# SCUT-BIP-Lab/SplatCo

Measured on AMD Instinct MI355X. Metric: rasterizer fwd+bwd Msplats/s @1080p; PSNR-match vs ref, higher is better.
Workload: dtype f32; 1 GPU; cfg1: 1M synthetic Gaussians (seed 0), 1 view 1920x1080 per GPU, GaussianRasterizer forward+backward, colors_precomp + scale/rotation path; gaussians=1000000, image=1920x1080, visible=1000000, parallelism=1 view per GPU (mv sharding)

## Files before the change

### include/splatco_raster.h

```cpp
#ifndef SPLATCO_RASTER_H
#define SPLATCO_RASTER_H

#include <stddef.h>
#include <stdint.h>

#ifdef __cplusplus
extern "C" {
#endif

#define SCR_ABI_VERSION 29
#define SCR_TILE 16

typedef struct scr_settings {
    int32_t image_height;
    int32_t image_width;
    float tanfovx;
    float tanfovy;
    const float* bg;
    float scale_modifier;
    const float* viewmatrix;
    const float* projmatrix;
    int32_t sh_degree;
    const float* campos;
    int32_t prefiltered;
    int32_t debug;
} scr_settings;

int scr_abi_version(void);
const char* scr_last_error(void);

size_t scr_geom_bytes(int64_t P, int32_t image_height, int32_t image_width);
size_t scr_binning_bytes(int64_t num_rendered, int64_t max_tile_instances);
size_t scr_image_bytes(int32_t image_height, int32_t image_width);
size_t scr_backward_scratch_bytes(int64_t num_rendered);

int scr_visible_filter(int64_t P, const float* means3D, const float* scales, const float* rotations,
                       const float* cov3D_precomp, const scr_settings* settings, int32_t* radii_out,
                       void* stream);

int scr_mark_visible(int64_t P, const float* means3D, const float* viewmatrix, uint8_t* present_out,
                     void* stream);

enum { SCR_PLAN_NONFINITE_COLOUR = 1,
       SCR_PLAN_LARGE_RECTS = 2 };
int scr_forward_plan(int64_t P, int32_t M, const float* means3D, const float* scales,
                     const float* rotations, const float* cov3D_precomp, const float* opacities,
                     const float* shs, const float* colors_precomp, const scr_settings* settings,
                     void* geom_buf, int32_t* radii_out, int64_t* plan_host, void* stream);

int scr_forward_run(int64_t P, int64_t num_rendered, int64_t max_tile_instances, int64_t plan_flags,
                    const scr_settings* settings, void* geom_buf, void* binning_buf, void* image_buf, float* out_color,
                    void* stream);

int scr_forward_plan_run(int64_t P, int32_t M, const float* means3D, const float* scales, const float* rotations,
                         const float* cov3D_precomp, const float* opacities, const float* shs, const float* colors_precomp,
                         const scr_settings* settings, void* geom_buf, int32_t* radii_out, int64_t* plan_host,
                         void* binning_buf, size_t binning_capacity_bytes, void* image_buf, float* out_color, void* stream);

int scr_backward(int64_t P, int32_t M, int64_t num_rendered, int64_t plan_flags, const float* means3D, const float* scales,
                 const float* rotations, const float* cov3D_precomp, const float* shs,
                 const scr_settings* settings, const int32_t* radii, void* geom_buf,
                 const void* binning_buf, void* image_buf, const float* dL_dcolor, void* scratch,
                 float* dL_dmeans3D, float* dL_dmeans2D, float* dL_dcolors, float* dL_dsh,
                 float* dL_dopacity, float* dL_dscales, float* dL_drotations, float* dL_dcov3D,
                 void* stream);

enum {
    SCR_DBG_TILES_TOUCHED = 0,
    SCR_DBG_POINT_OFFSETS = 1,
    SCR_DBG_RANGES = 2,
    SCR_DBG_POINT_LIST = 3,
    SCR_DBG_N_CONTRIB = 4,
    SCR_DBG_FINAL_T = 5,
    SCR_DBG_SPLAT_RECORDS = 6,
    SCR_DBG_QMASK = 7,
    SCR_DBG_GM_INDEX = 8
};
int scr_debug_force_deep_lists(int mode);
int scr_debug_get(int which, int64_t P, int64_t num_rendered, int32_t image_height, int32_t image_width,
                  const void* geom_buf, const void* binning_buf, const void* image_buf, void* out,
                  void* stream);

size_t scr_tpa_scratch_bytes(int32_t R, int32_t H, int32_t W);
int scr_tpa_stats(int32_t R, int32_t H, int32_t W, const float* p0, const float* p1, const float* p2, float* avg,
                  float* mx, int32_t* arg, void* scratch, void* stream);
int scr_tpa_forward(int32_t R, int32_t H, int32_t W, const float* p0, const float* p1, const float* p2, const float* ca,
                    const float* w, float* s, uint8_t* am, float* sa, float* pair0, float* pair1, float* pair2, void* stream);
int scr_tpa_backward(int32_t R, int32_t H, int32_t W, const float* p0, const float* p1, const float* p2, const float* ca,
                     const float* w, const float* s, const uint8_t* am, const float* sa, const float* g0, const float* g1,
                     const float* g2, float* d0, float* d1, float* d2, float* dca, float* dw, void* scratch, void* stream);
int scr_tpa_backward_stats(int32_t R, int32_t H, int32_t W, const float* davg, const float* dmax, const int32_t* arg,
                           float* d0, float* d1, float* d2, void* stream);

size_t scr_expand_scratch_bytes(int64_t n_candidates);
int scr_expand_plan(int64_t n_candidates, const float* neural_opacity, void* scratch,
                    int64_t* num_selected_host, void* stream);
int scr_mask_index_plan(int64_t n, const uint8_t* mask, void* scratch, int64_t* num_set_host, void* stream);
int scr_mask_index_run(int64_t n, const uint8_t* mask, const void* scratch, int64_t* index, int64_t* inverse, void* stream);
int scr_expand_run(int64_t V, int32_t k, const float* neural_opacity, const float* color,
                   const float* scale_rot, const float* offsets, int32_t offsets_ld, const float* grid_scaling,
                   const float* anchor, const void* scratch, int32_t* out_index, uint8_t* mask_out,
                   float* xyz, float* color_out, float* opacity, float* scaling, float* rot, void* stream);
int scr_expand_backward(int64_t V, int32_t k, const float* scale_rot, const float* offsets, int32_t offsets_ld,
                        const float* grid_scaling, const int32_t* out_index, const float* g_xyz,
                        const float* g_color, const float* g_opacity, const float* g_scaling,
                        const float* g_rot, float* d_neural_opacity, float* d_color, float* d_scale_rot,
                        float* d_offsets, float* d_grid_scaling, float* d_anchor, const float* g_reg, int64_t P,
                        void* stream);

size_t scr_triplane_backward_multi_scratch_bytes(int64_t V, int32_t ngrids, const int32_t* R, const int32_t* X, const int32_t* Y,
                                                 const int32_t* Z);
int scr_triplane_backward_multi(int64_t V, const float* coords, int32_t cstride, int32_t ngrids, const int32_t* R,
                                const int32_t* X, const int32_t* Y, const int32_t* Z, const int32_t* col, const float* grad_out,
                                int32_t ld, float* const* grad_planes, void* scratch, const float* nl_coef, const float* nl_dy,
                                int32_t nl_lddy, const float* nl_x, int32_t nl_ldx, void* stream);
int scr_plane_row_pairs(int32_t R, int32_t A, int32_t B, const float* plane, float* pairs, void* stream);
int scr_triplane_forward(int64_t V, const float* coords, int32_t cstride, const float* xy, const float* xz,
                         const float* yz, int32_t R, int32_t X, int32_t Y, int32_t Z, int32_t channel_last, float* out,
                         int32_t ld, int32_t col_xy, int32_t col_xz, int32_t col_yz, void* stream);
size_t scr_plane_sample_scratch_bytes(int64_t V, int32_t A, int32_t B, int32_t channels);
size_t scr_triplane_backward_scratch_bytes(int64_t V, int32_t X, int32_t Y, int32_t Z, int32_t channels);
int scr_triplane_backward(int64_t V, const float* coords, int32_t cstride, int32_t R, int32_t X, int32_t Y, int32_t Z,
                          int32_t planes, const float* grad_out, int32_t ld, const int32_t* cols, float* const* grad_planes,
                          void* scratch, void* stream);
int scr_plane_sample_backward(int64_t V, const float* coords, int32_t cstride, int32_t cx, int32_t cy, int32_t R,
                              int32_t A, int32_t B, int32_t planes, const float* grad_out0, const float* grad_out1,
                              int32_t ld, float* grad_plane0, float* grad_plane1, void* scratch, void* stream);

size_t scr_l1_ssim_scratch_bytes(int32_t C, int32_t H, int32_t W, int32_t with_grad);
int scr_l1_ssim_forward(int32_t C, int32_t H, int32_t W, const float* img1, const float* img2, void* scratch,
                        int32_t with_grad, float* out2, void* stream);
int scr_l1_ssim_backward(int32_t C, int32_t H, int32_t W, const float* img1, const float* img2,
                         const void* scratch, const float* g_l1, const float* g_ssim, float* dimg1,
                         void* stream);

#define SCR_FLIP_MAX_RADIUS 16
size_t scr_flip_scratch_bytes(int32_t N, int32_t H, int32_t W);
int scr_flip_forward(int32_t N, int32_t H, int32_t W, const float* test, const float* ref, double pixels_per_degree,
                     int32_t quantize, void* scratch, float* mean_out, float* mse_out, float* map_out, void* stream);
int scr_flip_filters(double pixels_per_degree, double* weights, int32_t* radii, double* scalars);

size_t scr_scaling_reg_scratch_bytes(int64_t P);
int scr_scaling_reg_forward(int64_t P, const float* scaling, void* scratch, float* out, void* stream);
int scr_scaling_reg_backward(int64_t P, const float* scaling, const float* g, float* dscaling, void* stream);

size_t scr_pair_l1_scratch_bytes(int64_t n);
int scr_pair_l1_forward(int64_t n, const float* gen1, const float* gen2, const float* real1, const float* real2, void* scratch,
                        float* out, void* stream);
int scr_pair_l1_backward(int64_t n, const float* gen1, const float* gen2, const float* real1, const float* real2, const float* g,
                         float* d_gen1, float* d_gen2, void* stream);

int32_t scr_anchor_gather_stat_rows(int64_t V);
int64_t scr_anchor_gather_stat_buffer_rows(int64_t V);
int scr_anchor_gather(int64_t V, const int64_t* visible_index, const float* anchor_feat, const float* anchor,
                      const float* offset, const float* scaling, float* feat_out, float* anchor_out, float* offsets_out,
                      float* grid_scaling_out, float* g_fea_out, int32_t g_fea_ld, float* col_stats_out, void* stream);
int scr_anchor_gather_backward(int64_t N, int64_t V, const int64_t* inverse_index, const float* grid_scaling, const float* d_feat,
                               const float* d_anchor, const float* d_offsets, const float* d_grid_scaling,
                               const float* d_g_fea, int32_t g_fea_ld, float* g_anchor_feat, float* g_anchor,
                               float* g_offset, float* g_scaling, int32_t accumulate, const float* nl_coef, const float* nl_dy,
                               int32_t nl_lddy, const float* nl_x, int32_t nl_ldx, void* stream);

size_t scr_norm_linear_scratch_bytes(int64_t V);
int scr_box_coords(int64_t V, const float* xyz, const float* lo_host, const float* hi_host, float* out, void* stream);
int scr_norm_fold(int32_t L, int32_t d, const int32_t* widths_host, const int32_t* cols_host, const uint8_t* col_at_host,
                  const void* const* lin_weight_host, const void* const* lin_bias_host, const void* const* bn_weight_host,
                  const void* const* bn_bias_host, float* G, float* c, void* stream);
int scr_norm_fold_backward(int32_t L, int32_t d, const int32_t* widths_host, const int32_t* cols_host, const uint8_t* col_at_host,
                           const void* const* lin_weight_host, const void* const* bn_weight_host, const void* const* bn_bias_host,
                           const float* dG, const float* dc, void* const* d_lin_weight_host, void* const* d_lin_bias_host,
                           void* const* d_bn_weight_host, void* const* d_bn_bias_host, void* stream);
int scr_norm_running_stats(int32_t L, int32_t d, const int32_t* widths_host, const int32_t* cols_host, const uint8_t* col_at_host,
                           const float* momentum_host, void* const* running_mean_host, void* const* running_var_host,
                           void* const* num_batches_host, const float* mean, const float* var, int64_t n, void* stream);
int scr_norm_linear_forward(int64_t V, int32_t d, const float* x, int32_t ldx, const float* G, const float* c, float eps,
                            float* y, float* mean, float* var, float* inv, void* scratch, const float* col_stats,
                            int32_t col_stat_rows, void* stream);
int scr_norm_linear_dx(int64_t V, int32_t d, const float* x, int32_t ldx, const float* dy, int32_t lddy, const float* coef,
                       float* dx, int32_t lddx, void* stream);
int scr_norm_linear_backward(int64_t V, int32_t d, const float* x, int32_t ldx, const float* dy, int32_t lddy, const float* G,
                             const float* mean, const float* inv, float* dx, int32_t lddx, float* dG, float* dc,
                             void* scratch, float* coef_out, void* stream);

size_t scr_mlp_heads_hidden_bytes(int64_t V);
size_t scr_mlp_heads_partial_bytes(int64_t V);
int scr_mlp_heads_forward(int64_t V, const float* feat, int32_t feat_ld, const float* anchor, const float* campos, const float* geo_a, const float* geo_b,
                          const float* w1, const float* b1, const float* w2o, const float* b2o, const float* w2c,
                          const float* b2c, const float* w2v, const float* b2v, void* hidden_save, float* out_opacity,
                          float* out_color, float* out_cov, void* stream);
int scr_mlp_heads_backward(int64_t V, const float* feat, int32_t feat_ld, const float* anchor, const float* campos, const float* geo_a, const float* geo_b,
                           const float* w1, const float* w2o, const float* w2c, const float* w2v, const void* hidden_save,
                           const float* out_opacity, const float* out_color, const float* g_opacity, const float* g_color,
                           const float* g_cov, void* partial, float* d_feat, float* d_anchor, float* d_geo_a, float* d_geo_b, float* d_w1,
                           float* d_b1, float* d_w2o, float* d_b2o, float* d_w2c, float* d_b2c, float* d_w2v, float* d_b2v,
                           void* stream);

int scr_statis_compute(int64_t V, int32_t k, const float* neural_opacity, const int32_t* out_index,
                       const uint8_t* update_filter, const float* viewspace_grad, int32_t grad_stride,
                       float* inc_opacity, float* inc_grad, void* stream);
int scr_statis_apply(int64_t V, int32_t k, const int64_t* visible_index, const float* inc_opacity, const float* inc_grad,
                     float* opacity_accum, float* anchor_demon, float* offset_gradient_accum, float* offset_denom,
                     void* stream);

typedef struct scr_adam_tensor {
    float* param;
    const float* grad;
    float* exp_avg;
    float* exp_avg_sq;
    int64_t numel;
    double step_size, bias_correction2_sqrt;
} scr_adam_tensor;
int scr_adam_step(int32_t n_tensors, const scr_adam_tensor* tensors, double beta1, double beta2, double eps, void* stream);

typedef struct scr_tv_plane {
    const float* plane;
    float* grad;
    int32_t channels, rows, cols;
    float coef;
} scr_tv_plane;
int scr_tv_add_grad(int32_t n_planes, const scr_tv_plane* planes, void* stream);

int scr_knn(int64_t N, int32_t k, const float* grid_host, const float* sorted_pts, const int64_t* sorted_id,
            const int32_t* cell_start, int64_t* out_idx, void* stream);
int scr_knn_curvature(int64_t N, int32_t k, const float* points, const int64_t* idx, float* curvature, void* stream);

size_t scr_points_bounds_scratch_bytes(int64_t N);
int scr_points_bounds(int64_t N, const float* points, void* scratch, float* out7, void* stream);
size_t scr_voxel_unique_scratch_bytes(int64_t N);
int scr_voxel_keys(int64_t N, const float* points, float voxel_size, const int32_t* lo_host, int32_t packed, int64_t* out,
                   void* stream);
int scr_voxel_unique_plan(int64_t N, const int64_t* sorted_keys, void* scratch, int64_t* num_unique_host, void* stream);
int scr_voxel_unique_run(int64_t N, const int64_t* sorted_keys, const void* scratch, float voxel_size,
                         const int32_t* lo_host, float* out_xyz, void* stream);
int scr_knn3_cell_keys(int64_t N, const float* grid_host, const float* points, int64_t* keys, void* stream);
int scr_knn3_dist2(int64_t N, const float* grid_host, const float* sorted_pts, const int64_t* sorted_id,
                   const int32_t* cell_start, float* out, void* stream);

int scr_copy_probe(const void* src, void* dst, size_t bytes, void* stream);

enum {
    SCR_PROF_FILTER = 0, SCR_PROF_PREPROCESS = 1, SCR_PROF_PLAN_SCAN = 2, SCR_PROF_SCATTER = 3,
    SCR_PROF_TILE_SORT = 4, SCR_PROF_BLEND_FORWARD = 5, SCR_PROF_BLEND_BACKWARD = 6,
    SCR_PROF_PREPROCESS_BACKWARD = 7, SCR_PROF_EXPAND = 8, SCR_PROF_EXPAND_BACKWARD = 9, SCR_PROF_PLANE_BACKWARD = 10,
    SCR_PROF_L1_SSIM = 11, SCR_PROF_L1_SSIM_BACKWARD = 12, SCR_PROF_TRIPLANE_FORWARD = 13, SCR_PROF_MLP_HEADS = 14,
    SCR_PROF_MLP_HEADS_BACKWARD = 15, SCR_PROF_NORM_LINEAR = 16, SCR_PROF_NORM_LINEAR_BACKWARD = 17, SCR_PROF_PLANE_ATTENTION = 18,
    SCR_PROF_FLIP = 19, SCR_PROF_COUNT = 20
};
int scr_profile_enable(int mask);
int scr_profile_stride(int every);
int scr_profile_read(double* total_ms, int64_t* launches);
const char* scr_profile_kernel_name(int idx);

int scr_markers_enable(int on);
int scr_marker_push(const char* name);
int scr_marker_pop(void);

#ifdef __cplusplus
}
#endif
#endif
```

### splatco_amd/_C.py

```python
import ctypes as C
import os

import torch

_HERE = os.path.dirname(os.path.abspath(__file__))
LIB_PATH = os.environ.get("SPLATCO_RASTER_LIB", os.path.join(_HERE, "csrc", "libsplatco_raster.so"))

PLAN_NONFINITE_COLOUR, PLAN_LARGE_RECTS = 1, 2
PROF_COUNT = 20
ABI_VERSION = 29
FLIP_MAX_RADIUS = 16

(DBG_TILES_TOUCHED, DBG_POINT_OFFSETS, DBG_RANGES, DBG_POINT_LIST, DBG_N_CONTRIB, DBG_FINAL_T, DBG_SPLAT_RECORDS, DBG_QMASK,
 DBG_GM_INDEX) = range(9)

vp, cp, u8, i32, i64, f32, f64, sz = C.c_void_p, C.c_char_p, C.c_uint8, C.c_int32, C.c_int64, C.c_float, C.c_double, C.c_size_t
P = C.POINTER


class Settings(C.Structure):
    _fields_ = [
        ("image_height", i32), ("image_width", i32),
        ("tanfovx", f32), ("tanfovy", f32),
        ("bg", vp), ("scale_modifier", f32),
        ("viewmatrix", vp), ("projmatrix", vp),
        ("sh_degree", i32), ("campos", vp),
        ("prefiltered", i32), ("debug", i32),
    ]


class AdamTensor(C.Structure):
    _fields_ = [("param", vp), ("grad", vp), ("exp_avg", vp), ("exp_avg_sq", vp),
                ("numel", i64), ("step_size", f64), ("bias_correction2_sqrt", f64)]


class TvPlane(C.Structure):
    _fields_ = [("plane", vp), ("grad", vp), ("channels", i32), ("rows", i32), ("cols", i32), ("coef", f32)]


SIGNATURES = [
    ("scr_abi_version", i32),
    ("scr_last_error", cp),
    ("scr_geom_bytes", sz, i64, i32, i32),
    ("scr_binning_bytes", sz, i64, i64),
    ("scr_image_bytes", sz, i32, i32),
    ("scr_backward_scratch_bytes", sz, i64),
    ("scr_visible_filter", i32, i64, vp, vp, vp, vp, P(Settings), vp, vp),
    ("scr_mark_visible", i32, i64, vp, vp, vp, vp),
    ("scr_forward_plan", i32, i64, i32, *[vp] * 7, P(Settings), vp, vp, P(i64), vp),
    ("scr_forward_run", i32, i64, i64, i64, i64, P(Settings), *[vp] * 5),
    ("scr_forward_plan_run", i32, i64, i32, *[vp] * 7, P(Settings), vp, vp, P(i64), vp, sz, vp, vp, vp),
    ("scr_backward", i32, i64, i32, i64, i64, *[vp] * 5, P(Settings), *[vp] * 15),
    ("scr_debug_force_deep_lists", i32, i32),
    ("scr_debug_get", i32, i32, i64, i64, i32, i32, *[vp] * 5),
    ("scr_tpa_scratch_bytes", sz, i32, i32, i32),
    ("scr_tpa_stats", i32, i32, i32, i32, *[vp] * 8),
    ("scr_tpa_forward", i32, i32, i32, i32, *[vp] * 12),
    ("scr_tpa_backward", i32, i32, i32, i32, *[vp] * 18),
    ("scr_tpa_backward_stats", i32, i32, i32, i32, *[vp] * 7),
    ("scr_expand_scratch_bytes", sz, i64),
    ("scr_expand_plan", i32, i64, vp, vp, P(i64), vp),
    ("scr_mask_index_plan", i32, i64, vp, vp, P(i64), vp),
    ("scr_mask_index_run", i32, i64, *[vp] * 5),
    ("scr_expand_run", i32, i64, i32, vp, vp, vp, vp, i32, *[vp] * 11),
    ("scr_expand_backward", i32, i64, i32, vp, vp, i32, *[vp] * 14, i64, vp),
    ("scr_triplane_backward_multi_scratch_bytes", sz, i64, i32, vp, vp, vp, vp),
    ("scr_triplane_backward_multi", i32, i64, vp, i32, i32, *[vp] * 6, i32, vp, vp, vp, vp, i32, vp, i32, vp),
    ("scr_plane_row_pairs", i32, i32, i32, i32, vp, vp, vp),
    ("scr_triplane_forward", i32, i64, vp, i32, vp, vp, vp, i32, i32, i32, i32, i32, vp, i32, i32, i32, i32, vp),
    ("scr_plane_sample_scratch_bytes", sz, i64, i32, i32, i32),
    ("scr_triplane_backward_scratch_bytes", sz, i64, i32, i32, i32, i32),
    ("scr_triplane_backward", i32, i64, vp, i32, i32, i32, i32, i32, i32, vp, i32, vp, vp, vp, vp),
    ("scr_plane_sample_backward", i32, i64, vp, i32, i32, i32, i32, i32, i32, i32, vp, vp, i32, vp, vp, vp, vp),
    ("scr_l1_ssim_scratch_bytes", sz, i32, i32, i32, i32),
    ("scr_l1_ssim_forward", i32, i32, i32, i32, vp, vp, vp, i32, vp, vp),
    ("scr_l1_ssim_backward", i32, i32, i32, i32, *[vp] * 7),
    ("scr_flip_scratch_bytes", sz, i32, i32, i32),
    ("scr_flip_forward", i32, i32, i32, i32, vp, vp, f64, i32, *[vp] * 5),
    ("scr_flip_filters", i32, f64, vp, vp, vp),
    ("scr_scaling_reg_scratch_bytes", sz, i64),
    ("scr_scaling_reg_forward", i32, i64, vp, vp, vp, vp),
    ("scr_scaling_reg_backward", i32, i64, vp, vp, vp, vp),
    ("scr_pair_l1_scratch_bytes", sz, i64),
    ("scr_pair_l1_forward", i32, i64, *[vp] * 7),
    ("scr_pair_l1_backward", i32, i64, *[vp] * 8),
    ("scr_anchor_gather_stat_rows", i32, i64),
    ("scr_anchor_gather_stat_buffer_rows", i64, i64),
    ("scr_anchor_gather", i32, i64, *[vp] * 10, i32, vp, vp),
    ("scr_anchor_gather_backward", i32, i64, i64, *[vp] * 7, i32, vp, vp, vp, vp, i32, vp, vp, i32, vp, i32, vp),
    ("scr_norm_linear_scratch_bytes", sz, i64),
    ("scr_box_coords", i32, i64, *[vp] * 5),
    ("scr_norm_fold", i32, i32, i32, *[vp] * 10),
    ("scr_norm_fold_backward", i32, i32, i32, *[vp] * 13),
    ("scr_norm_running_stats", i32, i32, i32, *[vp] * 9, i64, vp),
    ("scr_norm_linear_forward", i32, i64, i32, vp, i32, vp, vp, f32, *[vp] * 6, i32, vp),
    ("scr_norm_linear_dx", i32, i64, i32, vp, i32, vp, i32, vp, vp, i32, vp),
    ("scr_norm_linear_backward", i32, i64, i32, vp, i32, vp, i32, vp, vp, vp, vp, i32, *[vp] * 5),
    ("scr_mlp_heads_hidden_bytes", sz, i64),
    ("scr_mlp_heads_partial_bytes", sz, i64),
    ("scr_mlp_heads_forward", i32, i64, vp, i32, *[vp] * 17),
    ("scr_mlp_heads_backward", i32, i64, vp, i32, *[vp] * 28),
    ("scr_statis_compute", i32, i64, i32, vp, vp, vp, vp, i32, vp, vp, vp),
    ("scr_statis_apply", i32, i64, i32, *[vp] * 8),
    ("scr_adam_step", i32, i32, P(AdamTensor), f64, f64, f64, vp),
    ("scr_tv_add_grad", i32, i32, P(TvPlane), vp),
    ("scr_knn", i32, i64, i32, P(f32), *[vp] * 5),
    ("scr_knn_curvature", i32, i64, i32, vp, vp, vp, vp),
    ("scr_points_bounds_scratch_bytes", sz, i64),
    ("scr_points_bounds", i32, i64, vp, vp, vp, vp),
    ("scr_voxel_unique_scratch_bytes", sz, i64),
    ("scr_voxel_keys", i32, i64, vp, f32, P(i32), i32, vp, vp),
    ("scr_voxel_unique_plan", i32, i64, vp, vp, P(i64), vp),
    ("scr_voxel_unique_run", i32, i64, vp, vp, f32, P(i32), vp, vp),
    ("scr_knn3_cell_keys", i32, i64, P(f32), vp, vp, vp),
    ("scr_knn3_dist2", i32, i64, P(f32), *[vp] * 5),
    ("scr_copy_probe", i32, vp, vp, sz, vp),
    ("scr_profile_enable", i32, i32),
    ("scr_profile_stride", i32, i32),
    ("scr_profile_read", i32, P(f64), P(i64)),
    ("scr_profile_kernel_name", cp, i32),
    ("scr_markers_enable", i32, i32),
    ("scr_marker_push", i32, cp),
    ("scr_marker_pop", i32),
]
SYMBOLS = [s[0] for s in SIGNATURES]


def _load():
    if not os.path.exists(LIB_PATH):
        raise ImportError(
            f"{LIB_PATH} not found: the HIP rasterizer library is not built. Run "
            "`python -c 'import __graft_entry__ as g; g.build()'` (or `make -C splatco_amd/csrc`). "
            "There is deliberately no CPU fallback.")
    lib = C.CDLL(LIB_PATH)
    for name, restype, *argtypes in SIGNATURES:
        if not hasattr(lib, name):
            raise ImportError(f"{LIB_PATH} does not export {name}")
        f = getattr(lib, name)
        f.restype, f.argtypes = restype, argtypes
    if lib.scr_abi_version() != ABI_VERSION:
        raise ImportError(f"{LIB_PATH} has ABI version {lib.scr_abi_version()}, expected {ABI_VERSION}")
    return lib


lib = _load()


def profile_enable(which, every=1):
    check(lib.scr_profile_stride(max(int(every), 1)))
    if isinstance(which, str):
        names = [lib.scr_profile_kernel_name(i).decode() for i in range(PROF_COUNT)]
        mask = 1 << names.index(which)
    else:
        mask = -1 if which is True or which == -1 else int(which)
    lib.scr_profile_enable(mask)


MARKERS = False


def markers_enable(on=True):
    global MARKERS
    check(lib.scr_markers_enable(1 if on else 0))
    MARKERS = bool(on)


class stage:
    __slots__ = ("name", "on")

    def __init__(self, name):
        self.name = name

    def __enter__(self):
        self.on = MARKERS
        if self.on:
            lib.scr_marker_push(self.name.encode())
        return self

    def __exit__(self, *exc):
        if self.on:
            if torch.cuda.is_available():
                torch.cuda.synchronize()
            lib.scr_marker_pop()
        return False


def profile_read():
    ms = (C.c_double * PROF_COUNT)()
    n = (C.c_int64 * PROF_COUNT)()
    check(lib.scr_profile_read(ms, n))
    return {lib.scr_profile_kernel_name(i).decode(): (ms[i], n[i]) for i in range(PROF_COUNT)}


def check(rc):
    if rc != 0:
        raise RuntimeError("splatco_raster: " + lib.scr_last_error().decode())


def stream(device=None):
    return torch.cuda.current_stream(device).cuda_stream


def ptr(t):
    return None if t is None or t.numel() == 0 else t.data_ptr()


def host_array(values, ctype=i32):
    values = list(values)
    return (ctype * len(values))(*values)


def ptr_array(tensors):
    return host_array([t.data_ptr() for t in tensors], vp)


def scratch_size(nbytes):
    n = max(int(nbytes), 1)
    if n < (32 << 20):
        return n
    step = 1 << (n.bit_length() - 4)
    return (n + step - 1) // step * step


def scratch(nbytes, device):
    return torch.empty(scratch_size(nbytes), dtype=torch.uint8, device=device)


if os.environ.get("SPLATCO_MARKERS", "") not in ("", "0"):
    markers_enable(True)
```

### splatco_amd/csrc/binning.hip

```cpp
#include "common.h"

namespace scr {

template <int THREADS>
__device__ __forceinline__ uint32_t block_exclusive_scan(uint32_t v, uint32_t* lds_waves ,
                                                         uint32_t& block_total) {
    const int lane = threadIdx.x & (WAVE - 1), w = threadIdx.x / WAVE;
    uint32_t inc = v;
#pragma unroll
    for (int d = 1; d < WAVE; d <<= 1) {
        uint32_t n = __shfl_up(inc, d, WAVE);
        if (lane >= d) inc += n;
    }
    if (lane == WAVE - 1) lds_waves[w] = inc;
    __syncthreads();
    uint32_t base = 0, tot = 0;
#pragma unroll
    for (int k = 0; k < THREADS / WAVE; ++k) {
        uint32_t s = lds_waves[k];
        if (k < w) base += s;
        tot += s;
    }
    block_total = tot;
    __syncthreads();
    return base + inc - v;
}

__global__ void __launch_bounds__(1024) plan_scan_kernel(uint32_t nblk, uint32_t* __restrict__ block_sums,
                                                         unsigned long long* __restrict__ total,
                                                         uint32_t tiles, const uint32_t* __restrict__ tile_count,
                                                         uint32_t* __restrict__ ranges,
                                                         uint32_t* __restrict__ cursor,
                                                         volatile unsigned long long* mailbox,
                                                         unsigned long long seq) {
    __shared__ uint32_t lds[1024 / WAVE + 1];
    __shared__ unsigned long long wide[1024 / WAVE];
    if (blockIdx.x == 0) {
        unsigned long long carry = 0, mine = 0;
        for (uint32_t base = 0; base < nblk; base += 1024) {
            uint32_t i = base + threadIdx.x;
            uint32_t v = i < nblk ? block_sums[i] : 0u, tot;
            uint32_t ex = block_exclusive_scan<1024>(v, lds, tot);
            if (i < nblk) block_sums[i] = (uint32_t)carry + ex;
            carry += tot;
            mine += v;
        }
#pragma unroll
        for (int d = WAVE / 2; d > 0; d >>= 1) mine += (unsigned long long)__shfl_down((long long)mine, d, WAVE);
        __syncthreads();
        if ((threadIdx.x & (WAVE - 1)) == 0) wide[threadIdx.x / WAVE] = mine;
        __syncthreads();
        if (threadIdx.x == 0) {
            carry = 0;
            for (int w = 0; w < 1024 / WAVE; ++w) carry += wide[w];
            total[0] = carry;
            if (mailbox) {
                mailbox[0] = carry;
                __threadfence_system();
                mailbox[1] = seq;
            }
        }
    } else {
        uint32_t carry = 0, mx = 0;
        for (uint32_t base = 0; base < tiles; base += 1024) {
            uint32_t i = base + threadIdx.x;
            uint32_t v = i < tiles ? tile_count[i] : 0u, tot;
            uint32_t ex = block_exclusive_scan<1024>(v, lds, tot);
            if (i < tiles) {
                ranges[2 * i] = carry + ex;
                ranges[2 * i + 1] = carry + ex + v;
                cursor[i] = 0;
            }
            carry += tot;
            mx = max(mx, v);
        }
#pragma unroll
        for (int d = 32; d > 0; d >>= 1) mx = max(mx, (uint32_t)__shfl_xor((int)mx, d, WAVE));
        __syncthreads();
        if ((threadIdx.x & 63) == 0) lds[threadIdx.x >> 6] = mx;
        __syncthreads();
        if (threadIdx.x == 0) {
            uint32_t m = 0;
            for (int w = 0; w < 1024 / WAVE; ++w) m = max(m, lds[w]);
            total[1] = m;
            total[2] = 0;
            if (mailbox) {
                mailbox[2] = (unsigned long long)m | (total[3] << 32);
                __threadfence_system();
                mailbox[3] = seq;
            }
        }
    }
}

template <bool LDS_HIST>
__global__ void __launch_bounds__(BIN_THREADS)
scatter_kernel(int64_t P, int gx, int tiles, const float4* __restrict__ rec, uint2* __restrict__ gm_base,
               uint32_t* __restrict__ live_bits, const uint32_t* __restrict__ tiles_touched, const uint32_t* __restrict__ block_prefix,
               uint32_t* __restrict__ point_offsets, const uint32_t* __restrict__ ranges,
               uint32_t* __restrict__ cursor, unsigned long long* __restrict__ keys,
               const unsigned long long* __restrict__ total, unsigned long long cap_instances) {
    extern __shared__ __attribute__((aligned(16))) uint32_t hist[];
    __shared__ uint32_t lds[BIN_THREADS / WAVE + 1];
    if (total[0] > cap_instances) return;
    if (LDS_HIST) {
        for (int t = threadIdx.x; t < tiles; t += BIN_THREADS) hist[t] = 0;
        __syncthreads();
    }
    uint32_t off[BIN_ROUNDS], tts[BIN_ROUNDS], rlo[BIN_ROUNDS], rhi[BIN_ROUNDS], dbits[BIN_ROUNDS];
    uint32_t carry = block_prefix[blockIdx.x];
#pragma unroll
    for (int r = 0; r < BIN_ROUNDS; ++r) {
        const int64_t i = (int64_t)blockIdx.x * BIN_GPW + r * BIN_THREADS + threadIdx.x;
        const uint32_t tt = i < P ? tiles_touched[i] : 0u;
        uint32_t tot;
        off[r] = carry + block_exclusive_scan<BIN_THREADS>(tt, lds, tot);
        carry += tot;
        tts[r] = tt;
        rlo[r] = rhi[r] = dbits[r] = 0;
        if (i < P) point_offsets[i] = off[r] + tt;
        if (tt) {
            const float4 r2 = rec[3 * i + 2];
            dbits[r] = __float_as_uint(r2.y);
            rlo[r] = __float_as_uint(r2.z);
            rhi[r] = __float_as_uint(r2.w);
            const uint32_t x0 = rlo[r] & 0xffff, y0 = rlo[r] >> 16, rw = (rhi[r] & 0xffff) - x0;
            gm_base[i] = make_uint2(off[r] - y0 * rw - x0, rw);
            if (LDS_HIST)
                for (int ty = rlo[r] >> 16; ty < (int)(rhi[r] >> 16); ++ty)
                    for (int tx = rlo[r] & 0xffff; tx < (int)(rhi[r] & 0xffff); ++tx) atomicAdd(&hist[ty * gx + tx], 1u);
        }
    }
    if (LDS_HIST) {
        __syncthreads();
        for (int t = threadIdx.x; t < tiles; t += BIN_THREADS) {
            const uint32_t c = hist[t];
            if (c) hist[t] = ranges[2 * t] + atomicAdd(&cursor[t], c);
        }
        __syncthreads();
    }
#pragma unroll
    for (int r = 0; r < BIN_ROUNDS; ++r) {
        if (!tts[r]) continue;
        const int64_t i = (int64_t)blockIdx.x * BIN_GPW + r * BIN_THREADS + threadIdx.x;
        const uint32_t klo = (uint32_t)i << 4;
        const float4 r0 = rec[3 * i], r1 = rec[3 * i + 1];
        const unsigned long long khi = (unsigned long long)dbits[r] << 32;
        uint32_t live = 0, kbit = 1;
        for (int ty = rlo[r] >> 16; ty < (int)(rhi[r] >> 16); ++ty)
            for (int tx = rlo[r] & 0xffff; tx < (int)(rhi[r] & 0xffff); ++tx) {
                const uint32_t t = (uint32_t)(ty * gx + tx);
                const uint32_t slot = LDS_HIST ? atomicAdd(&hist[t], 1u) : ranges[2 * t] + atomicAdd(&cursor[t], 1u);
                const uint32_t qm = quadrant_mask(r0, r1, tx * TILE, ty * TILE);
                keys[slot] = khi | klo | qm;
                live |= qm ? kbit : 0u;
                kbit <<= 1;
            }
        live_bits[i] = live;
    }
}

template <int D>
__device__ __forceinline__ uint32_t lane_xor(uint32_t v) {
    if constexpr (D == 1) {
        return (uint32_t)__builtin_amdgcn_mov_dpp((int)v, 0xB1, 0xf, 0xf, true);
    } else if constexpr (D == 2) {
        return (uint32_t)__builtin_amdgcn_mov_dpp((int)v, 0x4E, 0xf, 0xf, true);
    } else if constexpr (D == 4) {
        int t = __builtin_amdgcn_update_dpp((int)v, (int)v, 0x104, 0xf, 0x5, false);
        return (uint32_t)__builtin_amdgcn_update_dpp(t, (int)v, 0x114, 0xf, 0xA, false);
    } else if constexpr (D == 8) {
        int t = __builtin_amdgcn_update_dpp((int)v, (int)v, 0x108, 0xf, 0x3, false);
        return (uint32_t)__builtin_amdgcn_update_dpp(t, (int)v, 0x118, 0xf, 0xC, false);
    } else if constexpr (D == 16) {
        auto r = __builtin_amdgcn_permlane16_swap(v, v, false, false);
        return sel(0xFFFF0000FFFF0000ull, r[0], r[1]);
    } else {
        auto r = __builtin_amdgcn_permlane32_swap(v, v, false, false);
        return sel(0xFFFFFFFF00000000ull, r[0], r[1]);
    }
}

constexpr unsigned long long lanes_with_bit_clear(int bit) {
    unsigned long long m = 0;
    for (int l = 0; l < 64; ++l)
        if ((l & bit) == 0) m |= 1ull << l;
    return m;
}

template <int E, int K, int J>
__device__ __forceinline__ void bitonic_step(uint32_t (&klo)[E], uint32_t (&khi)[E], int lane) {
    if constexpr (J < E) {
#pragma unroll
        for (int e = 0; e < E; ++e) {
            if ((e & J) != 0) continue;
            const int f = e | J;
            const unsigned long long desc = K < E ? ((e & K) == 0 ? 0ull : ~0ull) : ~lanes_with_bit_clear(K / E);
            const unsigned long long a = ((unsigned long long)khi[e] << 32) | klo[e];
            const unsigned long long b = ((unsigned long long)khi[f] << 32) | klo[f];
            const unsigned long long swm = lanes(a > b) ^ desc;
            const uint32_t t0 = klo[e], t1 = khi[e];
            klo[e] = sel(swm, klo[f], t0); khi[e] = sel(swm, khi[f], t1);
            klo[f] = sel(swm, t0, klo[f]); khi[f] = sel(swm, t1, khi[f]);
        }
    } else {
        constexpr int D = J / E;
        constexpr unsigned long long keep_max = lanes_with_bit_clear(D) ^ lanes_with_bit_clear(K / E);
#pragma unroll
        for (int e = 0; e < E; ++e) {
            const uint32_t olo = lane_xor<D>(klo[e]), ohi = lane_xor<D>(khi[e]);
            const unsigned long long mine = ((unsigned long long)khi[e] << 32) | klo[e];
            const unsigned long long theirs = ((unsigned long long)ohi << 32) | olo;
            const unsigned long long take = lanes(theirs < mine) ^ keep_max;
            klo[e] = sel(take, olo, klo[e]);
            khi[e] = sel(take, ohi, khi[e]);
        }
    }
}

template <int E, int K, int J>
__device__ __forceinline__ void bitonic_stage(uint32_t (&klo)[E], uint32_t (&khi)[E], int lane) {
    bitonic_step<E, K, J>(klo, khi, lane);
    if constexpr (J > 1) bitonic_stage<E, K, J / 2>(klo, khi, lane);
}
template <int E, int K>
__device__ __forceinline__ void bitonic_network(uint32_t (&klo)[E], uint32_t (&khi)[E], int lane) {
    bitonic_stage<E, K, K / 2>(klo, khi, lane);
    if constexpr (K < 64 * E) bitonic_network<E, K * 2>(klo, khi, lane);
}

constexpr int WAVE_SORT_MAX = 1024;

struct FinalLists {
    const uint2* gm_base;
    uint32_t* point_list;
    uint32_t* gm_index;
    uint8_t* qmask;
    int tx, ty;
    __device__ __forceinline__ void write(uint32_t i, uint32_t klo) const {
        const uint32_t id = klo >> 4;
        point_list[i] = id;
        qmask[i] = (uint8_t)(klo & 15u);
        if (gm_index) {
            const uint2 b = gm_base[id];
            gm_index[i] = b.x + (uint32_t)ty * b.y + (uint32_t)tx;
        }
    }
    template <int U, typename GetK>
    __device__ __forceinline__ void write_batch(uint32_t lo, uint32_t e0, uint32_t stride, uint32_t cnt, GetK getk) const {
        uint32_t k[U];
        uint2 b[U];
#pragma unroll
        for (int u = 0; u < U; ++u) {
            const uint32_t e = e0 + (uint32_t)u * stride;
            k[u] = e < cnt ? getk(e, u) : 0u;
        }
        if (gm_index) {
#pragma unroll
            for (int u = 0; u < U; ++u) b[u] = gm_base[k[u] >> 4];
        }
        __builtin_amdgcn_sched_barrier(0);
#pragma unroll
        for (int u = 0; u < U; ++u) {
            const uint32_t e = e0 + (uint32_t)u * stride;
            if (e < cnt) {
                point_list[lo + e] = k[u] >> 4;
                qmask[lo + e] = (uint8_t)(k[u] & 15u);
                if (gm_index) gm_index[lo + e] = b[u].x + (uint32_t)ty * b[u].y + (uint32_t)tx;
            }
        }
    }
};

template <int E>
__device__ __forceinline__ void wave_sort_regs(uint32_t n, const unsigned long long* __restrict__ keys,
                                               uint32_t (&klo)[E], uint32_t (&khi)[E]) {
    const int lane = threadIdx.x & 63;
#pragma unroll
    for (int e = 0; e < E; ++e) {
        const uint32_t i = (uint32_t)e * 64 + lane;
        const unsigned long long v = i < n ? keys[i] : ~0ull;
        klo[e] = (uint32_t)v;
        khi[e] = (uint32_t)(v >> 32);
    }
    bitonic_network<E, 2>(klo, khi, lane);
}

template <int E, bool FINAL>
__device__ __forceinline__ void wave_sort(uint32_t n, unsigned long long* __restrict__ keys, uint32_t lo,
                                          const FinalLists& fl, uint32_t* __restrict__ tr) {
    const int lane = threadIdx.x & 63;
    uint32_t klo[E], khi[E];
    wave_sort_regs<E>(n, keys, klo, khi);
    auto transpose = [&](uint32_t (&w)[E]) {
        __syncthreads();
#pragma unroll
        for (int e = 0; e < E; ++e) tr[lane * (E + 1) + e] = w[e];
        __syncthreads();
#pragma unroll
        for (int e = 0; e < E; ++e) {
            const int p = e * 64 + lane;
            w[e] = tr[p + p / E];
        }
    };
    transpose(klo);
    if (!FINAL) transpose(khi);
    if (FINAL) {
        fl.template write_batch<E>(lo, (uint32_t)lane, 64u, n, [&](uint32_t, int u) { return klo[u]; });
    } else {
#pragma unroll
        for (int e = 0; e < E; ++e) {
            const uint32_t i = (uint32_t)e * 64 + lane;
            if (i < n) keys[i] = ((unsigned long long)khi[e] << 32) | klo[e];
        }
    }
}

__device__ __forceinline__ int split_slot(int p) { return p + (p >> 3); }
constexpr int SPLIT_SLOTS = WAVE_SORT_MAX + WAVE_SORT_MAX / 8;
template <int EA, int EB>
__device__ __forceinline__ void wave_sort_split(uint32_t n, const unsigned long long* __restrict__ keys, uint32_t lo,
                                                const FinalLists& fl, unsigned long long* __restrict__ mb) {
    constexpr int NA = 64 * EA, NB = 64 * EB, PER = EA + EB;
    const int lane = threadIdx.x & 63;
    {
        uint32_t klo[EA], khi[EA];
        wave_sort_regs<EA>(NA, keys, klo, khi);
#pragma unroll
        for (int e = 0; e < EA; ++e) mb[split_slot(lane * EA + e)] = ((unsigned long long)khi[e] << 32) | klo[e];
    }
    {
        uint32_t klo[EB], khi[EB];
        wave_sort_regs<EB>(n - NA, keys + NA, klo, khi);
#pragma unroll
        for (int e = 0; e < EB; ++e) mb[split_slot(NA + lane * EB + e)] = ((unsigned long long)khi[e] << 32) | klo[e];
    }
    __syncthreads();
    uint32_t outk[PER];
    {
        auto keyA = [&](uint32_t i) { return mb[split_slot((int)i)]; };
        auto keyB = [&](uint32_t j) { return mb[split_slot(NA + (int)j)]; };
        const uint32_t d0 = (uint32_t)lane * PER;
        uint32_t a = d0 > (uint32_t)NB ? d0 - NB : 0u, b = min(d0, (uint32_t)NA);
        while (a < b) {
            const uint32_t mid = (a + b) >> 1;
            if (keyA(mid) < keyB(d0 - mid - 1)) a = mid + 1;
            else b = mid;
        }
        uint32_t ia = a, ib = d0 - a;
        unsigned long long x = ia < (uint32_t)NA ? keyA(ia) : ~0ull, y = ib < (uint32_t)NB ? keyB(ib) : ~0ull;
#pragma unroll
        for (int k = 0; k < PER; ++k) {
            const bool takeA = x <= y;
            outk[k] = (uint32_t)(takeA ? x : y);
            if (takeA) {
                ++ia;
                x = ia < (uint32_t)NA ? keyA(ia) : ~0ull;
            } else {
                ++ib;
                y = ib < (uint32_t)NB ? keyB(ib) : ~0ull;
            }
        }
    }
    __syncthreads();
    uint32_t* tr = (uint32_t*)mb;
#pragma unroll
    for (int k = 0; k < PER; ++k) tr[lane * (PER + 1) + k] = outk[k];
    __syncthreads();
    fl.template write_batch<PER>(lo, (uint32_t)lane, 64u, n, [&](uint32_t i, int) { return tr[i + i / PER]; });
}

template <bool FINAL>
__device__ __forceinline__ void wave_sort_any(uint32_t n, unsigned long long* keys, uint32_t lo, const FinalLists& fl,
                                              unsigned long long* mb) {
    uint32_t* tr = (uint32_t*)mb;
    if (n <= 64) wave_sort<1, FINAL>(n, keys, lo, fl, tr);
    else if (n <= 128) wave_sort<2, FINAL>(n, keys, lo, fl, tr);
    else if (n <= 256) wave_sort<4, FINAL>(n, keys, lo, fl, tr);
    else if (FINAL && n > 256 && n <= 320) wave_sort_split<4, 1>(n, keys, lo, fl, mb);
    else if (FINAL && n > 256 && n <= 384) wave_sort_split<4, 2>(n, keys, lo, fl, mb);
    else if (n <= 512) wave_sort<8, FINAL>(n, keys, lo, fl, tr);
    else if (FINAL && n <= 576) wave_sort_split<8, 1>(n, keys, lo, fl, mb);
    else if (FINAL && n <= 640) wave_sort_split<8, 2>(n, keys, lo, fl, mb);
    else if (FINAL && n <= 768) wave_sort_split<8, 4>(n, keys, lo, fl, mb);
    else if (FINAL) wave_sort_split<8, 8>(n, keys, lo, fl, mb);
    else wave_sort<16, FINAL>(n, keys, lo, fl, tr);
}

__global__ void __launch_bounds__(64, 1)
tile_sort_wave_kernel(int tiles, int gx, const uint32_t* __restrict__ ranges, unsigned long long* __restrict__ keys,
                      const uint2* __restrict__ gm_base, uint32_t* __restrict__ point_list,
                      uint32_t* __restrict__ gm_index, uint8_t* __restrict__ qmask) {
    int t = xcd_tile(blockIdx.x, tiles);
    if (t < 0) return;
    const uint32_t lo = ranges[2 * t], n = ranges[2 * t + 1] - lo;
    if (n == 0 || n > (uint32_t)WAVE_SORT_MAX) return;
    const FinalLists fl{gm_base, point_list, gm_index, qmask, t % gx, t / gx};
    __shared__ unsigned long long mb[SPLIT_SLOTS];
    wave_sort_any<true>(n, keys + lo, lo, fl, mb);
}

constexpr int WG_SORT_THREADS = WG_SORT_MAX / 16;
__device__ __forceinline__ int wg_slot(int p) { return p + (p >> 4); }
__global__ void __launch_bounds__(WG_SORT_THREADS)
tile_sort_wg_kernel(int tiles, int gx, const uint32_t* __restrict__ ranges, unsigned long long* __restrict__ keys,
                    const uint2* __restrict__ gm_base, uint32_t* __restrict__ point_list,
                    uint32_t* __restrict__ gm_index, uint8_t* __restrict__ qmask) {
    extern __shared__ __attribute__((aligned(16))) unsigned long long buf[];
    int t = xcd_tile(blockIdx.x, tiles);
    if (t < 0) return;
    const uint32_t lo = ranges[2 * t], n = ranges[2 * t + 1] - lo;
    if (n <= (uint32_t)WAVE_SORT_MAX) return;
    const uint32_t c0 = blockIdx.y * (uint32_t)WG_SORT_MAX;
    if (c0 >= n) return;
    const uint32_t cnt = min((uint32_t)WG_SORT_MAX, n - c0);
    const int wave = threadIdx.x >> 6, lane = threadIdx.x & 63;
    unsigned long long* chunk = keys + lo + c0;
    {
        const uint32_t w0 = (uint32_t)wave * WAVE_SORT_MAX;
        const uint32_t wn = w0 < cnt ? min((uint32_t)WAVE_SORT_MAX, cnt - w0) : 0u;
        uint32_t klo[16], khi[16];
        wave_sort_regs<16>(wn, chunk + w0, klo, khi);
#pragma unroll
        for (int e = 0; e < 16; ++e)
            buf[wg_slot((int)w0 + lane * 16 + e)] = ((unsigned long long)khi[e] << 32) | klo[e];
    }
    __syncthreads();
    for (uint32_t L = WAVE_SORT_MAX; L < (uint32_t)WG_SORT_MAX && L < cnt; L <<= 1) {
        constexpr int PER = WG_SORT_MAX / WG_SORT_THREADS;
        unsigned long long outk[PER];
        const uint32_t o0 = threadIdx.x * PER, pairbase = o0 / (2u * L) * (2u * L), d0 = o0 - pairbase;
        {
            auto keyA = [&](uint32_t i) { return buf[wg_slot((int)(pairbase + i))]; };
            auto keyB = [&](uint32_t j) { return buf[wg_slot((int)(pairbase + L + j))]; };
            uint32_t a = d0 > L ? d0 - L : 0u, b = min(d0, L);
            while (a < b) {
                const uint32_t mid = (a + b) >> 1;
                if (keyA(mid) < keyB(d0 - mid - 1)) a = mid + 1;
                else b = mid;
            }
            uint32_t ia = a, ib = d0 - a;
            unsigned long long x = ia < L ? keyA(ia) : ~0ull, y = ib < L ? keyB(ib) : ~0ull;
#pragma unroll
            for (int k = 0; k < PER; ++k) {
                const bool takeA = x <= y;
                outk[k] = takeA ? x : y;
                if (takeA) {
                    ++ia;
                    x = ia < L ? keyA(ia) : ~0ull;
                } else {
                    ++ib;
                    y = ib < L ? keyB(ib) : ~0ull;
                }
            }
        }
        __syncthreads();
#pragma unroll
        for (int k = 0; k < PER; ++k) buf[wg_slot((int)(o0 + k))] = outk[k];
        __syncthreads();
    }
    const unsigned long long* src = buf;
    if (n <= (uint32_t)WG_SORT_MAX) {
        const FinalLists fl{gm_base, point_list, gm_index, qmask, t % gx, t / gx};
        for (uint32_t e = threadIdx.x; e < cnt; e += 4 * WG_SORT_THREADS)
            fl.template write_batch<4>(lo, e, (uint32_t)WG_SORT_THREADS, cnt, [&](uint32_t i, int) { return (uint32_t)src[wg_slot((int)i)]; });
    } else {
        for (uint32_t e = threadIdx.x; e < cnt; e += WG_SORT_THREADS) chunk[e] = src[wg_slot((int)e)];
    }
}

constexpr int MP_SEG = 4096;
__device__ __forceinline__ uint32_t merge_passes_needed(uint32_t n) {
    uint32_t chunks = (n + WG_SORT_MAX - 1) / WG_SORT_MAX, p = 0;
    while ((1u << p) < chunks) ++p;
    return p;
}

__device__ __forceinline__ uint32_t merge_path_cut(const unsigned long long* __restrict__ A, uint32_t la,
                                                   const unsigned long long* __restrict__ B, uint32_t lb, uint32_t s) {
    const uint32_t lane = threadIdx.x & 63;
    uint32_t lo = s > lb ? s - lb : 0u, hi = min(s, la);
    while (lo < hi) {
        const uint32_t span = hi - lo;
        const uint32_t p = span >= 65u ? lo + (uint32_t)(((unsigned long long)span * (lane + 1)) / 65u) : min(lo + lane, hi - 1);
        const bool below = A[p] < B[s - p - 1];
        const unsigned long long bal = __builtin_amdgcn_ballot_w64(below);
        const int c = __builtin_popcountll(bal);
        const uint32_t plast = __shfl(p, c > 0 ? c - 1 : 0, 64), pfirst = __shfl(p, c < 64 ? c : 63, 64);
        const uint32_t nlo = c > 0 ? plast + 1 : lo, nhi = c < 64 ? pfirst : hi;
        if (span < 65u) {
            return c < (int)min(span, 64u) ? lo + (uint32_t)c : hi;
        }
        lo = nlo;
        hi = nhi;
    }
    return lo;
}

__global__ void __launch_bounds__(256)
tile_merge_path_kernel(int tiles, int gx, uint32_t pass, const uint32_t* __restrict__ ranges,
                       const unsigned long long* __restrict__ src, unsigned long long* __restrict__ dst,
                       const uint2* __restrict__ gm_base, uint32_t* __restrict__ point_list,
                       uint32_t* __restrict__ gm_index, uint8_t* __restrict__ qmask) {
    __shared__ unsigned long long buf[MP_SEG + MP_SEG / 16];
    __shared__ uint32_t cut[2];
    int t = xcd_tile(blockIdx.x, tiles);
    if (t < 0) return;
    const uint32_t lo = ranges[2 * t], n = ranges[2 * t + 1] - lo;
    if (n <= (uint32_t)WG_SORT_MAX || pass >= merge_passes_needed(n)) return;
    const uint32_t L = (uint32_t)WG_SORT_MAX << pass;
    const uint32_t e0 = blockIdx.y * (uint32_t)MP_SEG;
    if (e0 >= n) return;
    const uint32_t pairbase = e0 / (2u * L) * (2u * L);
    const uint32_t lenA = min(L, n - pairbase);
    const uint32_t lenB = n - pairbase > L ? min(L, n - pairbase - L) : 0u;
    const uint32_t s0 = e0 - pairbase, s1 = min(s0 + (uint32_t)MP_SEG, lenA + lenB);
    const unsigned long long* A = src + lo + pairbase;
    const unsigned long long* B = A + L;
    if (threadIdx.x < 128) {
        const int w = threadIdx.x >> 6;
        const uint32_t cw = merge_path_cut(A, lenA, B, lenB, w ? s1 : s0);
        if ((threadIdx.x & 63) == 0) cut[w] = cw;
    }
    __syncthreads();
    const uint32_t i0 = cut[0], na = cut[1] - i0, j0 = s0 - i0, nb = (s1 - s0) - na;
    const uint32_t tot = na + nb;
    {
        unsigned long long v[MP_SEG / 256];
#pragma unroll
        for (int k = 0; k < MP_SEG / 256; ++k) {
            const uint32_t e = min(threadIdx.x + 256u * k, tot - 1);
            v[k] = e < na ? A[i0 + e] : B[j0 + (e - na)];
        }
#pragma unroll
        for (int k = 0; k < MP_SEG / 256; ++k) {
            const uint32_t e = threadIdx.x + 256u * k;
            if (e < tot) buf[wg_slot((int)e)] = v[k];
        }
    }
    __syncthreads();
    constexpr int PER = MP_SEG / 256;
    unsigned long long outk[PER];
    const uint32_t d0 = min((uint32_t)threadIdx.x * PER, tot);
    {
        auto keyA = [&](uint32_t i) { return buf[wg_slot((int)i)]; };
        auto keyB = [&](uint32_t j) { return buf[wg_slot((int)(na + j))]; };
        uint32_t a = d0 > nb ? d0 - nb : 0u, b = min(d0, na);
        while (a < b) {
            const uint32_t mid = (a + b) >> 1;
            if (keyA(mid) < keyB(d0 - mid - 1)) a = mid + 1;
            else b = mid;
        }
        uint32_t ia = a, ib = d0 - a;
        unsigned long long x = ia < na ? keyA(ia) : ~0ull, y = ib < nb ? keyB(ib) : ~0ull;
#pragma unroll
        for (int k = 0; k < PER; ++k) {
            const bool takeA = x < y;
            outk[k] = takeA ? x : y;
            if (takeA) {
                ++ia;
                x = ia < na ? keyA(ia) : ~0ull;
            } else {
                ++ib;
                y = ib < nb ? keyB(ib) : ~0ull;
            }
        }
    }
    __syncthreads();
#pragma unroll
    for (int k = 0; k < PER; ++k)
        if (d0 + k < tot) buf[wg_slot((int)(d0 + k))] = outk[k];
    __syncthreads();
    if (pass + 1 == merge_passes_needed(n)) {
        const FinalLists fl{gm_base, point_list, gm_index, qmask, t % gx, t / gx};
        for (uint32_t e = threadIdx.x; e < tot; e += 4 * 256)
            fl.template write_batch<4>(lo + pairbase + s0, e, 256u, tot, [&](uint32_t i, int) { return (uint32_t)buf[wg_slot((int)i)]; });
    } else {
        unsigned long long* out = dst + lo + pairbase + s0;
        for (uint32_t e = threadIdx.x; e < tot; e += 256) out[e] = buf[wg_slot((int)e)];
    }
}

void launch_plan_scans(int64_t P, const KSettings& ks, const GeomView& gv, unsigned long long* mailbox,
                       unsigned long long seq, hipStream_t st) {
    Grid g(ks.H, ks.W);
    uint32_t nb = (uint32_t)((P + BIN_GPW - 1) / BIN_GPW);
    plan_scan_kernel<<<2, 1024, 0, st>>>(nb, gv.block_sums, gv.total, (uint32_t)g.tiles, gv.tile_count,
                                         gv.ranges, gv.cursor, mailbox, seq);
}

void launch_scatter(int64_t P, const KSettings& ks, const GeomView& gv, const BinView& bv, unsigned long long cap_instances,
                    hipStream_t st) {
    if (P <= 0) return;
    Grid g(ks.H, ks.W);
    const unsigned nb = (unsigned)((P + BIN_GPW - 1) / BIN_GPW);
    allow_dynamic_lds((const void*)scatter_kernel<true>, LDS_HIST_MAX_TILES * 4);
    if (g.tiles <= LDS_HIST_MAX_TILES)
        scatter_kernel<true><<<nb, BIN_THREADS, (size_t)g.tiles * 4, st>>>(
            P, g.gx, g.tiles, gv.rec, gv.gm_base, gv.live_bits, gv.tiles_touched, gv.block_sums, gv.point_offsets, gv.ranges,
            gv.cursor, bv.keys, gv.total, cap_instances);
    else
        scatter_kernel<false><<<nb, BIN_THREADS, 0, st>>>(
            P, g.gx, g.tiles, gv.rec, gv.gm_base, gv.live_bits, gv.tiles_touched, gv.block_sums, gv.point_offsets, gv.ranges,
            gv.cursor, bv.keys, gv.total, cap_instances);
}

void launch_tile_sort(const KSettings& ks, const GeomView& gv, const BinView& bv, int64_t max_tile_instances,
                      bool with_gm_index, hipStream_t st) {
    uint32_t* const gm_index = with_gm_index ? bv.gm_index : nullptr;
    Grid g(ks.H, ks.W);
    const unsigned gt = (unsigned)xcd_grid(g.tiles);
    if (max_tile_instances <= 0) return;
    tile_sort_wave_kernel<<<gt, 64, 0, st>>>(g.tiles, g.gx, gv.ranges, bv.keys, gv.gm_base, bv.point_list, gm_index,
                                             bv.qmask);
    if (max_tile_instances <= WAVE_SORT_MAX) return;
    const unsigned chunks = (unsigned)((max_tile_instances + WG_SORT_MAX - 1) / WG_SORT_MAX);
    const size_t lds = (size_t)(WG_SORT_MAX + WG_SORT_MAX / 16) * 8;
    allow_dynamic_lds((const void*)tile_sort_wg_kernel, lds);
    tile_sort_wg_kernel<<<dim3(gt, chunks), WG_SORT_THREADS, lds, st>>>(g.tiles, g.gx, gv.ranges, bv.keys, gv.gm_base, bv.point_list,
                                                                        gm_index, bv.qmask);
    if (chunks <= 1) return;
    unsigned passes = 0;
    while ((1u << passes) < chunks) ++passes;
    const unsigned segs = (unsigned)((max_tile_instances + MP_SEG - 1) / MP_SEG);
    for (unsigned p = 0; p < passes; ++p) {
        const unsigned long long* src = (p & 1u) ? bv.keys2 : bv.keys;
        unsigned long long* dst = (p & 1u) ? bv.keys : bv.keys2;
        tile_merge_path_kernel<<<dim3(gt, segs), 256, 0, st>>>(g.tiles, g.gx, p, gv.ranges, src, dst, gv.gm_base,
                                                               bv.point_list, gm_index, bv.qmask);
    }
}

}
```

### splatco_amd/csrc/blend.hip

```cpp
#include <type_traits>

#include "common.h"

namespace scr {

typedef float v2f __attribute__((ext_vector_type(2)));

#ifdef SCR_BLEND_COUNT
__device__ __forceinline__ void count_sub_blocks(unsigned long long m, unsigned long long (&len)[4]) {
    len[0] += (m & 0x000000000f0f0f0full) != 0ull;
    len[1] += (m & 0x00000000f0f0f0f0ull) != 0ull;
    len[2] += (m & 0x0f0f0f0f00000000ull) != 0ull;
    len[3] += (m & 0xf0f0f0f000000000ull) != 0ull;
}
#define SCR_COUNT_SUB(m) (count_sub_blocks((m), sub_), count_sub_blocks((m), subc_))
#define SCR_COUNT_CHUNK_END(i)                                                                             \
    do {                                                                                                   \
        const unsigned long long a_ = subc_[0] > subc_[1] ? subc_[0] : subc_[1], b_ = subc_[2] > subc_[3] ? subc_[2] : subc_[3]; \
        cnt_[(i)] += a_ > b_ ? a_ : b_;                                                                    \
        subc_[0] = subc_[1] = subc_[2] = subc_[3] = 0;                                                     \
    } while (0)
#define SCR_COUNT_SUB_FLUSH(i_sum, i_max)                                                                  \
    do {                                                                                                   \
        cnt_[(i_sum)] += sub_[0] + sub_[1] + sub_[2] + sub_[3];                                            \
        const unsigned long long a_ = sub_[0] > sub_[1] ? sub_[0] : sub_[1], b_ = sub_[2] > sub_[3] ? sub_[2] : sub_[3]; \
        cnt_[(i_max)] += a_ > b_ ? a_ : b_;                                                                \
    } while (0)
#endif
#ifdef SCR_BLEND_COUNT
__device__ unsigned long long g_blend_counters[16];
#define SCR_COUNT(i, v) (cnt_[(i)] += (unsigned long long)(v))
#define SCR_COUNT_DECL unsigned long long cnt_[16] = {}, sub_[4] = {}, subc_[4] = {}
#define SCR_COUNT_FLUSH(lane)                                                        \
    if ((lane) == 0)                                                                 \
        for (int q_ = 0; q_ < 16; ++q_)                                              \
            if (cnt_[q_]) atomicAdd(&g_blend_counters[q_], cnt_[q_])
#else
#define SCR_COUNT(i, v) ((void)0)
#define SCR_COUNT_SUB(m) ((void)0)
#define SCR_COUNT_CHUNK_END(i) ((void)0)
#define SCR_COUNT_SUB_FLUSH(a, b) ((void)0)
#define SCR_COUNT_DECL ((void)0)
#define SCR_COUNT_FLUSH(lane) ((void)0)
#endif

__device__ __forceinline__ float fast_exp(float x) {
    const float p = x * 1.4426950408889634f;
    const float g = __builtin_amdgcn_exp2f(p);
    const float r = __builtin_fmaf(-p, 0.6931471805599453f, x);
    return __builtin_fmaf(g, r, g);
}

__device__ __forceinline__ uint32_t lanes_below(unsigned long long ballot) {
    return __builtin_amdgcn_mbcnt_hi((uint32_t)(ballot >> 32), __builtin_amdgcn_mbcnt_lo((uint32_t)ballot, 0u));
}

__global__ void __launch_bounds__(1024)
tile_order_kernel(int tiles, int gx, const uint32_t* __restrict__ ranges, uint32_t* __restrict__ order,
                  unsigned long long* __restrict__ ordered, unsigned long long* __restrict__ first) {
    __shared__ uint32_t hist[1024], start[1024], wsum[16];
    __shared__ uint32_t s_max, cnt[NUM_XCD];
    const int me = blockIdx.x;
    hist[threadIdx.x] = 0;
    if (threadIdx.x == 0) s_max = 1;
    if (threadIdx.x < NUM_XCD) cnt[threadIdx.x] = 0;
    __syncthreads();
    uint32_t mx = 0, mine[NUM_XCD] = {};
    for (int t = threadIdx.x; t < tiles; t += 1024) {
        const int x = xcd_of_tile(t, gx);
#pragma unroll
        for (int q = 0; q < NUM_XCD; ++q) mine[q] += x == q;
        if (x == me) mx = max(mx, ranges[2 * t + 1] - ranges[2 * t]);
    }
#pragma unroll
    for (int q = 0; q < NUM_XCD; ++q)
        if (mine[q]) atomicAdd(&cnt[q], mine[q]);
    if (mx) atomicMax(&s_max, mx);
    __syncthreads();
    uint32_t off = 0;
    for (int q = 0; q < me; ++q) off += cnt[q];
    const float scale = 1023.0f / (float)s_max;
    for (int t = threadIdx.x; t < tiles; t += 1024) {
        if (xcd_of_tile(t, gx) != me) continue;
        const uint32_t n = ranges[2 * t + 1] - ranges[2 * t];
        atomicAdd(&hist[1023 - min(1023u, (uint32_t)((float)n * scale))], 1u);
    }
    __syncthreads();
    {
        const int lane = threadIdx.x & 63, w = threadIdx.x >> 6;
        uint32_t v = hist[threadIdx.x], inc = v;
#pragma unroll
        for (int d = 1; d < 64; d <<= 1) {
            const uint32_t o = __shfl_up(inc, d, 64);
            if (lane >= d) inc += o;
        }
        if (lane == 63) wsum[w] = inc;
        __syncthreads();
        uint32_t base = 0;
        for (int q = 0; q < w; ++q) base += wsum[q];
        start[threadIdx.x] = base + inc - v;
    }
    __syncthreads();
    for (int t = threadIdx.x; t < tiles; t += 1024) {
        if (xcd_of_tile(t, gx) != me) continue;
        const uint32_t n = ranges[2 * t + 1] - ranges[2 * t];
        order[off + atomicAdd(&start[1023 - min(1023u, (uint32_t)((float)n * scale))], 1u)] = (uint32_t)t;
    }
    if (threadIdx.x == 0) {
        first[me] = off;
        if (me == NUM_XCD - 1) first[NUM_XCD] = off + cnt[me];
        if (me == 0) *ordered = 1;
    }
}

__device__ __forceinline__ int blend_tile(int slot, int tiles, const uint32_t* __restrict__ order,
                                          const unsigned long long* __restrict__ total) {
    const int xcd = slot % NUM_XCD, j = slot / NUM_XCD;
    if (total[2]) {
        const uint32_t f = (uint32_t)total[4 + xcd], e = (uint32_t)total[5 + xcd];
        return f + j < e ? (int)order[f + j] : -1;
    }
    const int chunk = (tiles + NUM_XCD - 1) / NUM_XCD;
    const int t = xcd * chunk + j;
    return j < chunk && t < tiles ? t : -1;
}

constexpr int FCHUNK = 64;

template <bool SAFE>
__global__ void __launch_bounds__(64)
blend_forward_kernel(int W, int H, int gx, int tiles, const uint32_t* __restrict__ order, const unsigned long long* __restrict__ total,
                     const uint32_t* __restrict__ ranges,
                     const uint32_t* __restrict__ point_list, const uint8_t* __restrict__ qmask,
                     const float4* __restrict__ rec, const float* __restrict__ bg,
                     float* __restrict__ out_color, float* __restrict__ final_T,
                     uint32_t* __restrict__ n_contrib) {
    __shared__ float4 sp[5][FCHUNK / 2];
    const int quad = (blockIdx.x / NUM_XCD) & 3;
    const int t = blend_tile((int)(blockIdx.x % NUM_XCD + (blockIdx.x / (4 * NUM_XCD)) * NUM_XCD), tiles, order, total);
    if (t < 0) return;
    const int lane = threadIdx.x;
    const int px = (t % gx) * TILE + (quad & 1) * 8 + (lane & 7);
    const int py = (t / gx) * TILE + (quad >> 1) * 8 + (lane >> 3);
    const bool inside = px < W && py < H;
    const float pxf = (float)px, pyf = (float)py;
    const uint32_t lo = ranges[2 * t], n = ranges[2 * t + 1] - lo;
    unsigned long long done = lanes(!inside);
    SCR_COUNT_DECL;
    float T = 1.0f, C0 = 0.0f, C1 = 0.0f, C2 = 0.0f;
    float c099 = 0.99f;
    asm volatile("" : "+v"(c099));
    uint32_t last = 0;

    uint32_t m_next = 0, id_next = 0;
    bool sel_cur = false;
    float4 r0 = make_float4(0, 0, 0, 0), r1 = r0;
    float r2x = 0.0f;
    auto load_mask_id = [&](uint32_t base, uint32_t& m, uint32_t& id) {
        uint32_t i = base + lane;
        bool have = i < n;
        m = have ? ((qmask[lo + i] >> quad) & 1u) : 0u;
        id = have ? point_list[lo + i] : 0u;
    };
    auto gather = [&](uint32_t m, uint32_t id) {
        sel_cur = m != 0;
        if (sel_cur) {
            r0 = rec[3 * (size_t)id];
            r1 = rec[3 * (size_t)id + 1];
            r2x = rec[3 * (size_t)id + 2].x;
        }
    };
    for (int i = lane; i < 5 * (FCHUNK / 2); i += WAVE) (&sp[0][0])[i] = make_float4(0, 0, 0, 0);
    uint32_t m0, id0;
    load_mask_id(0, m0, id0);
    gather(m0, id0);
    load_mask_id(FCHUNK, m_next, id_next);

    for (uint32_t base = 0; base < n; base += FCHUNK) {
        const unsigned long long bal = __builtin_amdgcn_ballot_w64(sel_cur);
        const int cnt = __builtin_popcountll(bal);
        if (sel_cur) {
            const uint32_t pos = lanes_below(bal), q = pos >> 1, h = pos & 1;
            float* f0 = (float*)&sp[0][q];
            float* f1 = (float*)&sp[1][q];
            float* f2 = (float*)&sp[2][q];
            float* f3 = (float*)&sp[3][q];
            float* f4 = (float*)&sp[4][q];
            f0[h] = r0.x; f0[2 + h] = r0.y;
            f1[h] = r0.z; f1[2 + h] = r0.w;
            f2[h] = r1.x; f2[2 + h] = r1.y;
            f3[h] = r1.z; f3[2 + h] = r1.w;
            f4[h] = r2x;  f4[2 + h] = __uint_as_float(base + lane + 1);
        }
        gather(m_next, id_next);
        load_mask_id(base + 2 * FCHUNK, m_next, id_next);
        __syncthreads();
        auto group = [&](const int k, auto npairs) {
            constexpr int NP = decltype(npairs)::value, NS = 2 * NP;
            v2f power[NP], al[NP];
            float4 p3[NP], p4[NP];
#pragma unroll
            for (int h = 0; h < NP; ++h) {
                const int q = (k >> 1) + h;
                const float4 p0 = sp[0][q], p1 = sp[1][q], p2 = sp[2][q];
                p3[h] = sp[3][q];
                p4[h] = sp[4][q];
                const v2f dx = v2f{p0.x, p0.y} - pxf, dy = v2f{p0.z, p0.w} - pyf;
                const v2f A = {p1.x, p1.y}, B = {p1.z, p1.w}, Cq = {p2.x, p2.y}, o = {p2.z, p2.w};
                power[h] = __builtin_elementwise_fma(dx, __builtin_elementwise_fma(A, dx, B * dy), (Cq * dy) * dy);
                al[h] = o * v2f{fast_exp(power[h].x), fast_exp(power[h].y)};
            }
            float alpha[NS], pw[NS];
#pragma unroll
            for (int h = 0; h < NP; ++h) {
                alpha[2 * h] = vmin(c099, al[h].x); alpha[2 * h + 1] = vmin(c099, al[h].y);
                pw[2 * h] = power[h].x; pw[2 * h + 1] = power[h].y;
            }
            unsigned long long hit[NS], anyh = 0ull;
#pragma unroll
            for (int u = 0; u < NS; ++u) {
                hit[u] = (k + u < cnt) ? (lanes(!(pw[u] > 0.0f)) & lanes(!(alpha[u] < 1.0f / 255.0f))) : 0ull;
                anyh |= hit[u];
            }
#ifdef SCR_BLEND_COUNT
            for (int u = 0; u < NS; ++u)
                if (k + u < cnt) {
                    SCR_COUNT(0, 1);
                    SCR_COUNT(2, __builtin_popcountll(done & lanes(inside)));
                    SCR_COUNT(3, (anyh & ~done) == 0ull);
                }
#endif
            if ((anyh & ~done) == 0ull) return;
#pragma unroll
            for (int u = 0; u < NS; ++u) {
                const int h = u >> 1;
                const float cr = (u & 1) ? p3[h].y : p3[h].x, cg = (u & 1) ? p3[h].w : p3[h].z;
                const float cb = (u & 1) ? p4[h].y : p4[h].x, cj = (u & 1) ? p4[h].w : p4[h].z;
                const unsigned long long hm = hit[u] & ~done;
                const unsigned long long stop = lanes(T * (1.0f - alpha[u]) < 0.0001f) & hm;
                done |= stop;
                const unsigned long long live = hm & ~stop;
                SCR_COUNT(1, __builtin_popcountll(live));
                SCR_COUNT_SUB(live);
                const float a = sel(live, alpha[u], 0.0f);
                const float w = a * T;
                if (SAFE) {
                    C0 = sel(live, __builtin_fmaf(cr, w, C0), C0);
                    C1 = sel(live, __builtin_fmaf(cg, w, C1), C1);
                    C2 = sel(live, __builtin_fmaf(cb, w, C2), C2);
                } else {
                    C0 = __builtin_fmaf(cr, w, C0);
                    C1 = __builtin_fmaf(cg, w, C1);
                    C2 = __builtin_fmaf(cb, w, C2);
                }
                T = T * (1.0f - a);
                last = sel(live, __float_as_uint(cj), last);
            }
        };
        int k = 0;
        for (; k + 2 < cnt; k += 4) group(k, std::integral_constant<int, 2>{});
        if (k < cnt) group(k, std::integral_constant<int, 1>{});
        SCR_COUNT_CHUNK_END(6);
        if (~done == 0ull) break;
        __syncthreads();
    }
    SCR_COUNT_SUB_FLUSH(4, 5);
    SCR_COUNT_FLUSH(lane);
    if (inside) {
        size_t pix = (size_t)py * W + px, hw = (size_t)H * W;
        out_color[pix] = __builtin_fmaf(T, bg[0], C0);
        out_color[hw + pix] = __builtin_fmaf(T, bg[1], C1);
        out_color[2 * hw + pix] = __builtin_fmaf(T, bg[2], C2);
        final_T[pix] = T;
        n_contrib[pix] = last;
    }
}

#define SCR_DPP(d, s, ctrl) "v_add_f32_dpp " d ", " s ", " s " " ctrl "\n\t"
__device__ __forceinline__ void column_fold(float& s0, float& s1, float& s2, float t0, float t1, float t2) {
    asm volatile("s_nop 1\n\t"
                 SCR_DPP("%0", "%0", "row_shl:4 row_mask:0xf bank_mask:0x5")
                 SCR_DPP("%1", "%1", "row_shl:4 row_mask:0xf bank_mask:0x5")
                 SCR_DPP("%2", "%2", "row_shl:4 row_mask:0xf bank_mask:0x5")
                 SCR_DPP("%0", "%3", "row_shr:4 row_mask:0xf bank_mask:0xa")
                 SCR_DPP("%1", "%4", "row_shr:4 row_mask:0xf bank_mask:0xa")
                 SCR_DPP("%2", "%5", "row_shr:4 row_mask:0xf bank_mask:0xa")
                 SCR_DPP("%0", "%0", "quad_perm:[2,3,0,1] row_mask:0xf bank_mask:0xf")
                 SCR_DPP("%1", "%1", "quad_perm:[2,3,0,1] row_mask:0xf bank_mask:0xf")
                 SCR_DPP("%2", "%2", "quad_perm:[2,3,0,1] row_mask:0xf bank_mask:0xf")
                 SCR_DPP("%0", "%0", "quad_perm:[1,0,3,2] row_mask:0xf bank_mask:0xf")
                 SCR_DPP("%1", "%1", "quad_perm:[1,0,3,2] row_mask:0xf bank_mask:0xf")
                 SCR_DPP("%2", "%2", "quad_perm:[1,0,3,2] row_mask:0xf bank_mask:0xf")
                 "s_nop 1"
                 : "+v"(s0), "+v"(s1), "+v"(s2)
                 : "v"(t0), "v"(t1), "v"(t2));
}
constexpr int TCS = WAVE + 4;

struct PixState {
    float T, dLp0, dLp1, dLp2;
    float behind, last_alpha, d_last;
};
template <bool SAFE>
__device__ __forceinline__ void splat_pixel_grad(PixState& s, float T, float4 b, float cb, float G, float alpha,
                                                 unsigned long long hit, float& Y, float& w) {
#pragma clang fp contract(fast)
    w = alpha * T;
    s.behind = SAFE ? s.last_alpha * s.d_last + (1.0f - s.last_alpha) * s.behind : s.last_alpha * (s.d_last - s.behind) + s.behind;
    float d = b.z * s.dLp0 + b.w * s.dLp1 + cb * s.dLp2;
    if (SAFE) d = sel(hit, d, 0.0f);
    Y = G * (T * (d - s.behind));
    if (SAFE) Y = sel(hit, Y, 0.0f);
    s.last_alpha = alpha;
    s.d_last = d;
}
__device__ __forceinline__ void group_transmittance(float& T, const float (&om)[4], float (&Tu)[4]) {
#pragma clang fp contract(off)
    const float P = ((om[0] * om[1]) * om[2]) * om[3];
    float r = __builtin_amdgcn_rcpf(P);
    r = __builtin_fmaf(__builtin_fmaf(-P, r, 1.0f), r, r);
    const float q = T * r;
    Tu[3] = __builtin_fmaf(__builtin_fmaf(-q, P, T), r, q);
    Tu[2] = Tu[3] * om[3];
    Tu[1] = Tu[2] * om[2];
    Tu[0] = Tu[1] * om[1];
    T = Tu[3];
}

typedef float f4_t __attribute__((ext_vector_type(4)));
__device__ __forceinline__ void store16_dword_aligned(void* p, float4 v) {
    const f4_t q = {v.x, v.y, v.z, v.w};
    asm volatile("global_store_dwordx4 %0, %1, off" : : "v"(p), "v"(q) : "memory");
}

constexpr int BCH = 64;
constexpr int BWD_MIN_WAVES = 4;
constexpr int ACC_BUFS = 2;

template <bool SAFE>
__global__ void __launch_bounds__(256, BWD_MIN_WAVES)
blend_backward_kernel(int W, int H, int gx, int tiles, const uint32_t* __restrict__ order, const unsigned long long* __restrict__ total,
                      const uint32_t* __restrict__ ranges,
                      const uint32_t* __restrict__ point_list, const uint32_t* __restrict__ gm_index,
                      const uint2* __restrict__ gm_base,
                      const uint8_t* __restrict__ qmask, const float4* __restrict__ rec,
                      const float* __restrict__ bg, const float* __restrict__ final_T,
                      const uint32_t* __restrict__ n_contrib, const float* __restrict__ dL_dpix,
                      GradRec* __restrict__ grad_rec, unsigned long long* __restrict__ cut_key, unsigned long long stamp,
                      uint8_t* __restrict__ has_rec) {
    __shared__ float4 st[4][3][BCH + 4];
    __shared__ float4 accA[ACC_BUFS][4][BCH], accB[ACC_BUFS][4][BCH];
    __shared__ float accC[ACC_BUFS][4][BCH];
    __shared__ __attribute__((aligned(16))) float tr[4][8 * TCS];
    __shared__ uint32_t wave_max[4];
    const int t = blend_tile((int)blockIdx.x, tiles, order, total);
    if (t < 0) return;
    const uint32_t lo = ranges[2 * t], n = ranges[2 * t + 1] - lo;
    if (n == 0) return;
    const int wave = threadIdx.x >> 6, lane = threadIdx.x & 63;
    const int qx0 = (t % gx) * TILE + (wave & 1) * 8, qy0 = (t / gx) * TILE + (wave >> 1) * 8;
    const int px = qx0 + (lane >> 3), py = qy0 + (lane & 7);
    const bool inside = px < W && py < H;
    const float pxf = (float)px, pyf = (float)py;
    const float qx0f = (float)qx0, qy0f = (float)qy0;
    const size_t pix = (size_t)py * W + px, hw = (size_t)H * W;
    const uint32_t last = inside ? n_contrib[pix] : 0u;
    PixState ps;
    ps.T = inside ? final_T[pix] : 0.0f;
    ps.dLp0 = ps.dLp1 = ps.dLp2 = 0.0f;
    if (inside) {
        ps.dLp0 = dL_dpix[pix];
        ps.dLp1 = dL_dpix[hw + pix];
        ps.dLp2 = dL_dpix[2 * hw + pix];
    }
    ps.behind = (bg[0] * ps.dLp0 + bg[1] * ps.dLp1) + bg[2] * ps.dLp2;
    ps.last_alpha = ps.d_last = 0.0f;
    float c099 = 0.99f;
    asm volatile("" : "+v"(c099));
    SCR_COUNT_DECL;
    const int rcol = lane >> 3, rx = lane & 7;
    float wgt[3][8];
#pragma unroll
    for (int y = 0; y < 8; ++y) {
        wgt[0][y] = 1.0f; wgt[1][y] = (float)y; wgt[2][y] = (float)(y * y);
        if (rcol >= 4) {
            const bool in = qx0 + rx < W && qy0 + y < H;
            const size_t q = (size_t)(qy0 + y) * W + (size_t)(qx0 + rx);
#pragma unroll
            for (int c = 0; c < 3; ++c) wgt[c][y] = in ? dL_dpix[c * hw + q] : 0.0f;
        }
    }
    const float xw = rcol < 4 ? (float)rx : 0.0f;
    float* const trw = &tr[wave][0];
    const float* const trr = trw + rcol * TCS + 8 * rx;
    const int rkind = rcol >= 4 ? 2 : (lane >> 2) & 1;
    const bool rstore = (lane & 3) == 0 && (rcol < 4 || ((lane >> 2) & 1) == 0);
    const int rcu = rcol & 3;
    const unsigned long long rcu1 = lanes(rcu == 1), rcu2 = lanes(rcu == 2), rcu3 = lanes(rcu == 3);
    char* const accA0 = (char*)&accA[0][wave][0];
    char* const accB0 = (char*)&accB[0][wave][0];
    char* const rdst0 = rkind == 0 ? accA0 : rkind == 1 ? accA0 + 4 : accB0 + 8;
    char* const rdst1 = rkind == 0 ? accA0 + 8 : rkind == 1 ? accA0 + 12 : accB0 + 12;
    char* const rdst2 = rkind == 0 ? accB0 + 4 : rkind == 1 ? accB0 : (char*)&accC[0][wave][0];
    const uint32_t rstride2 = rkind == 2 ? 4u : 16u;
    constexpr uint32_t PAR_A = sizeof(float4) * 4 * BCH, PAR_C = sizeof(float) * 4 * BCH;
    const uint32_t rpar2 = rkind == 2 ? PAR_C : PAR_A;
    uint32_t wm = last;
#pragma unroll
    for (int d = 32; d > 0; d >>= 1) wm = max(wm, (uint32_t)__shfl_xor((int)wm, d, WAVE));
    if (lane == 0) wave_max[wave] = wm;
    if (lane < 9) st[wave][lane / 3][lane % 3] = make_float4(0, 0, 0, 0);
    __syncthreads();
    const uint32_t wmax0 = wave_max[0], wmax1 = wave_max[1], wmax2 = wave_max[2], wmax3 = wave_max[3];
    const uint32_t max_last = max(max(wmax0, wmax1), max(wmax2, wmax3));
    const uint32_t wave_last = wave == 0 ? wmax0 : wave == 1 ? wmax1 : wave == 2 ? wmax2 : wmax3;
    const int nround = (int)((n + BCH - 1) / BCH);
    const int live_top = max_last ? (int)((max_last - 1) / BCH) : -1;

    constexpr int CUT_MIN_ROUNDS = 3;
    const bool cut = nround - 1 - live_top >= CUT_MIN_ROUNDS;
    if (threadIdx.x == 0) {
        unsigned long long ck = ~0ull;
        if (cut) {
            const uint32_t idc = point_list[lo + (uint32_t)(live_top + 1) * BCH];
            ck = ((unsigned long long)__float_as_uint(rec[3 * (size_t)idc + 2].y) << 32) | idc;
            cut_key[tiles] = stamp;
        }
        cut_key[t] = ck;
    }
    const uint32_t tile_x = (uint32_t)(t % gx), tile_y = (uint32_t)(t / gx);
    auto gm_of = [&](uint32_t pos, uint32_t id) -> uint32_t {
        if (gm_index) return gm_index[pos];
        const uint2 b = gm_base[id];
        return b.x + tile_y * b.y + tile_x;
    };
    if (!cut && wave < 3)
        for (int ci = nround - 1; ci > live_top; --ci) {
            const uint32_t i = (uint32_t)ci * BCH + lane;
            if (i < n && qmask[lo + i] != 0) {
                GradRec& gr = grad_rec[gm_of(lo + i, point_list[lo + i])];
                if (wave == 0) store16_dword_aligned(&gr.a, make_float4(0, 0, 0, 0));
                else if (wave == 1) store16_dword_aligned(&gr.b, make_float4(0, 0, 0, 0));
                else gr.c = 0.0f;
            }
        }

    uint32_t m_next = 0, id_next = 0, slot_next = 0;
    uint32_t m_cur = 0, slot_cur = 0, id_cur = 0;
    bool sel_cur = false;
    float4 r0 = make_float4(0, 0, 0, 0), r1 = r0;
    float r2x = 0.0f;
    auto load_meta = [&](int ci, uint32_t& m, uint32_t& id, uint32_t& slot) {
        const uint32_t i = (uint32_t)ci * BCH + lane;
        const bool have = ci >= 0 && i < n;
        m = have ? qmask[lo + i] : 0u;
        id = have ? point_list[lo + i] : 0u;
        slot = have ? gm_of(lo + i, id) : 0u;
    };
    auto gather = [&](int ci, uint32_t m, uint32_t id, uint32_t slot) {
        const uint32_t i = (uint32_t)ci * BCH + lane;
        sel_cur = ((m >> wave) & 1u) && i < wave_last;
        m_cur = m;
        slot_cur = slot;
        id_cur = id;
        if (sel_cur) {
            r0 = rec[3 * (size_t)id];
            r1 = rec[3 * (size_t)id + 1];
            r2x = rec[3 * (size_t)id + 2].x;
        }
    };
    if (live_top >= 0) {
        uint32_t m0, id0, sl0;
        load_meta(live_top, m0, id0, sl0);
        gather(live_top, m0, id0, sl0);
        load_meta(live_top - 1, m_next, id_next, slot_next);
    }
    for (int ci = live_top; ci >= 0; --ci) {
        const uint32_t base = (uint32_t)ci * BCH;
        const int last_rel = (int)last - (int)base;
        const unsigned long long bal = __builtin_amdgcn_ballot_w64(sel_cur);
        const int cnt = __builtin_popcountll(bal);
        if (sel_cur) {
            const uint32_t pos = lanes_below(bal);
            st[wave][0][pos + 3] = r0;
            st[wave][1][pos + 3] = r1;
            st[wave][2][pos + 3] = make_float4(r2x, __uint_as_float((uint32_t)lane), 0.0f, 0.0f);
        }
        const uint32_t m_this = m_cur, slot_this = slot_cur, id_this = id_cur;
        gather(ci - 1, m_next, id_next, slot_next);
        load_meta(ci - 2, m_next, id_next, slot_next);
        const int par = ci & 1;
        auto group = [&](const int k, auto tail) {
            constexpr bool TAIL = decltype(tail)::value;
            float Y[4], Wt[4];
            uint32_t jj[4] = {0u, 0u, 0u, 0u};
            unsigned long long hits[4] = {0ull, 0ull, 0ull, 0ull};
            float4 ra[4], rb[4];
            float2 rc[4];
#pragma unroll
            for (int u = 0; u < 4; ++u) {
                ra[u] = st[wave][0][k + 3 - u];
                rb[u] = st[wave][1][k + 3 - u];
                rc[u] = *(const float2*)&st[wave][2][k + 3 - u];
            }
            float Gs[4], al[4], om[4], Tu[4];
#pragma unroll
            for (int u = 0; u < 4; ++u) {
                if (TAIL && k - u < 0) {
                    Gs[u] = al[u] = 0.0f;
                    om[u] = 1.0f;
                    SCR_COUNT(13, 1);
                    continue;
                }
                const float4 a = ra[u], b = rb[u];
                const uint32_t j = __float_as_uint(rc[u].y);
                const float dx = a.x - pxf, dy = a.y - pyf;
                const float power = __builtin_fmaf(dx, __builtin_fmaf(a.z, dx, a.w * dy), (b.x * dy) * dy);
                const float ar = b.y * fast_exp(power);
                const unsigned long long hit = lanes((int)j < last_rel) & lanes(!(power > 0.0f)) & lanes(!(ar < 1.0f / 255.0f));
                SCR_COUNT(8, 1);
                SCR_COUNT(9, __builtin_popcountll(hit));
                SCR_COUNT_SUB(hit);
                SCR_COUNT(10, __builtin_popcountll(lanes(!((int)j < last_rel)) & lanes(inside)));
                SCR_COUNT(11, __builtin_popcountll(lanes(!(power > 0.0f)) & lanes(!(ar < 1.0f / 255.0f)) & lanes(inside)));
                Gs[u] = sel(hit, ar, 0.0f);
                al[u] = vmin(c099, Gs[u]);
                om[u] = 1.0f - al[u];
                if (SAFE) hits[u] = hit;
                jj[u] = j;
            }
            group_transmittance(ps.T, om, Tu);
#pragma unroll
            for (int u = 0; u < 4; ++u) {
                if (TAIL && k - u < 0) {
                    Y[u] = Wt[u] = 0.0f;
                    continue;
                }
                splat_pixel_grad<SAFE>(ps, Tu[u], rb[u], rc[u].x, Gs[u], al[u], hits[u], Y[u], Wt[u]);
            }
            float s0, s1, s2;
            {
                asm volatile("" ::: "memory");
#pragma unroll
                for (int u = 0; u < 4; ++u) {
                    trw[u * TCS + lane] = Y[u];
                    trw[(4 + u) * TCS + lane] = Wt[u];
                }
                asm volatile("" ::: "memory");
                const float4 va = *(const float4*)trr, vb = *(const float4*)(trr + 4);
                asm volatile("" ::: "memory");
                const float v[8] = {va.x, va.y, va.z, va.w, vb.x, vb.y, vb.z, vb.w};
                float e0 = wgt[0][0] * v[0], e1 = wgt[1][0] * v[0], e2 = wgt[2][0] * v[0];
                float o0 = wgt[0][1] * v[1], o1 = wgt[1][1] * v[1], o2 = wgt[2][1] * v[1];
#pragma unroll
                for (int y = 2; y < 8; y += 2) {
                    e0 = __builtin_fmaf(wgt[0][y], v[y], e0);
                    e1 = __builtin_fmaf(wgt[1][y], v[y], e1);
                    e2 = __builtin_fmaf(wgt[2][y], v[y], e2);
                    o0 = __builtin_fmaf(wgt[0][y + 1], v[y + 1], o0);
                    o1 = __builtin_fmaf(wgt[1][y + 1], v[y + 1], o1);
                    o2 = __builtin_fmaf(wgt[2][y + 1], v[y + 1], o2);
                }
                s0 = e0 + o0; s1 = e1 + o1; s2 = e2 + o2;
                const float t0 = xw * s0, t1 = xw * t0, t2 = xw * s1;
                column_fold(s0, s1, s2, t0, t1, t2);
            }
            if (rstore && (!TAIL || k - rcu >= 0)) {
                const uint32_t jw = sel(rcu3, jj[3], sel(rcu2, jj[2], sel(rcu1, jj[1], jj[0])));
                *(float*)(rdst0 + par * PAR_A + jw * 16u) = s0;
                *(float*)(rdst1 + par * PAR_A + jw * 16u) = s1;
                *(float*)(rdst2 + par * rpar2 + jw * rstride2) = s2;
            }
        };
        int k = cnt - 1;
        for (; k >= 3; k -= 4) group(k, std::false_type{});
        if (k >= 0) group(k, std::true_type{});
        SCR_COUNT_CHUNK_END(7);
        asm volatile("s_waitcnt lgkmcnt(0)" ::: "memory");
        if (lane < cnt) {
            const float4 ra = st[wave][0][lane + 3];
            const uint32_t j = __float_as_uint(st[wave][2][lane + 3].y);
            const float a = ra.x - qx0f, b = ra.y - qy0f;
            const float4 A = accA[par][wave][j], B = accB[par][wave][j];
            const float M0 = A.x, Mx = A.y, My = A.z, Mxx = A.w, Mxy = B.x, Myy = B.y;
            const float t1 = a * M0 - Mx, t2 = b * M0 - My;
            accA[par][wave][j] = make_float4(t1, t2, a * (t1 - Mx) + Mxx, (a * t2 - b * Mx) + Mxy);
            accB[par][wave][j] = make_float4(b * (t2 - My) + Myy, M0, B.z, B.w);
        }
        __syncthreads();
        if (wave < 3 && base + lane < n && m_this != 0) {
            const uint32_t i = base + lane;
            float4 r = make_float4(0, 0, 0, 0);
            auto part = [&](int w) {
                return wave == 0 ? accA[par][w][lane] : wave == 1 ? accB[par][w][lane]
                                                                  : make_float4(accC[par][w][lane], 0.0f, 0.0f, 0.0f);
            };
            if (((m_this >> 0) & 1u) && i < wmax0) { const float4 x = part(0); r.x += x.x; r.y += x.y; r.z += x.z; r.w += x.w; }
            if (((m_this >> 1) & 1u) && i < wmax1) { const float4 x = part(1); r.x += x.x; r.y += x.y; r.z += x.z; r.w += x.w; }
            if (((m_this >> 2) & 1u) && i < wmax2) { const float4 x = part(2); r.x += x.x; r.y += x.y; r.z += x.z; r.w += x.w; }
            if (((m_this >> 3) & 1u) && i < wmax3) { const float4 x = part(3); r.x += x.x; r.y += x.y; r.z += x.z; r.w += x.w; }
            GradRec& gr = grad_rec[slot_this];
            if (wave == 0) store16_dword_aligned(&gr.a, r);
            else if (wave == 1) store16_dword_aligned(&gr.b, r);
            else {
                gr.c = r.x;
                if (has_rec) has_rec[id_this] = 1;
            }
        }
    }
    SCR_COUNT_SUB_FLUSH(14, 15);
    SCR_COUNT_FLUSH(lane);
}

static int blend_slots_per_xcd(const Grid& g) {
    int cnt[NUM_XCD] = {};
    for (int t = 0; t < g.tiles; ++t) ++cnt[xcd_of_tile(t, g.gx)];
    int m = (g.tiles + NUM_XCD - 1) / NUM_XCD;
    for (int q = 0; q < NUM_XCD; ++q) m = cnt[q] > m ? cnt[q] : m;
    return m;
}

void launch_blend_forward(const KSettings& ks, const GeomView& gv, const BinView& bv, const ImgView& iv,
                          float* out_color, bool longest_first, bool safe, hipStream_t st) {
    Grid g(ks.H, ks.W);
    if (longest_first)
        tile_order_kernel<<<NUM_XCD, 1024, 0, st>>>(g.tiles, g.gx, gv.ranges, gv.tile_count, gv.total + 2, gv.total + 4);
    auto kernel = safe ? blend_forward_kernel<true> : blend_forward_kernel<false>;
    kernel<<<(unsigned)blend_slots_per_xcd(g) * NUM_XCD * 4, 64, 0, st>>>(
        ks.W, ks.H, g.gx, g.tiles, gv.tile_count, gv.total, gv.ranges, bv.point_list, bv.qmask, gv.rec, ks.bg, out_color, iv.final_T,
        iv.n_contrib);
}

void launch_blend_backward(const KSettings& ks, const GeomView& gv, const BinView& bv, const ImgView& iv,
                           const float* dL_dcolor, GradRec* grad_rec, unsigned long long stamp, bool deep, bool flags,
                           bool safe, hipStream_t st) {
    Grid g(ks.H, ks.W);
    const bool gm_from_base = deep;
    if (flags) { ZeroList z; z.add(gv.has_rec, ((size_t)gv.P + 3) / 4 * 4, st); launch_zero(z, st); }
    auto kernel = safe ? blend_backward_kernel<true> : blend_backward_kernel<false>;
    kernel<<<(unsigned)blend_slots_per_xcd(g) * NUM_XCD, 256, 0, st>>>(
        ks.W, ks.H, g.gx, g.tiles, gv.tile_count, gv.total, gv.ranges, bv.point_list, gm_from_base ? nullptr : bv.gm_index, gv.gm_base,
        bv.qmask, gv.rec, ks.bg,
        iv.final_T, iv.n_contrib, dL_dcolor, grad_rec, iv.cut_key, stamp, flags ? gv.has_rec : nullptr);
}

}

#ifdef SCR_BLEND_COUNT
extern "C" int scr_tool_blend_counters(unsigned long long* out16, int reset) {
    if (out16 && hipMemcpyFromSymbol(out16, HIP_SYMBOL(scr::g_blend_counters), 16 * 8) != hipSuccess) return 1;
    if (reset) {
        unsigned long long z[16] = {};
        if (hipMemcpyToSymbol(HIP_SYMBOL(scr::g_blend_counters), z, 16 * 8) != hipSuccess) return 1;
    }
    return 0;
}
#endif
```

### splatco_amd/csrc/capi.hip

```cpp
#include <stdarg.h>
#include <stdio.h>
#include <string.h>

#include "common.h"
#include "adam.h"
#include "tv.h"
#include <chrono>
#include <map>
#include <mutex>
#include <utility>
#include <cstring>

using namespace scr;

static thread_local char g_err[512] = "";
namespace scr {
int g_force_deep_lists = -1;

void allow_dynamic_lds(const void* kernel, size_t bytes) {
    if (bytes <= 65536) return;
    static std::mutex mu;
    static std::map<std::pair<int, const void*>, size_t> granted;
    int dev = 0;
    (void)hipGetDevice(&dev);
    std::lock_guard<std::mutex> lk(mu);
    size_t& have = granted[{dev, kernel}];
    if (bytes <= have) return;
    if (hipFuncSetAttribute(kernel, hipFuncAttributeMaxDynamicSharedMemorySize, (int)bytes) == hipSuccess) have = bytes;
    (void)hipGetLastError();
}
}

static int fail(const char* fmt, ...) {
    va_list ap;
    va_start(ap, fmt);
    vsnprintf(g_err, sizeof(g_err), fmt, ap);
    va_end(ap);
    return 1;
}

#define HIP_TRY(expr)                                                                      \
    do {                                                                                   \
        hipError_t e_ = (expr);                                                            \
        if (e_ != hipSuccess) return fail("%s failed: %s", #expr, hipGetErrorString(e_)); \
    } while (0)

#define CHECK_LAUNCH(name, debug, st)                                                      \
    do {                                                                                   \
        hipError_t e_ = hipGetLastError();                                                 \
        if (e_ != hipSuccess) return fail("launch of %s failed: %s", name, hipGetErrorString(e_)); \
        if (debug) {                                                                       \
            e_ = hipStreamSynchronize(st);                                                 \
            if (e_ != hipSuccess) return fail("%s faulted: %s", name, hipGetErrorString(e_)); \
        }                                                                                  \
    } while (0)

#include <dlfcn.h>
#include <atomic>
#include <vector>
namespace {
struct ProfRec { int idx; hipEvent_t a, b; };
unsigned g_prof_mask = 0;
unsigned g_prof_stride = 1;
unsigned g_prof_seen[32] = {};
std::vector<ProfRec> g_prof_recs;
std::vector<hipEvent_t> g_prof_pool;
hipEvent_t prof_event() {
    hipEvent_t e;
    if (!g_prof_pool.empty()) { e = g_prof_pool.back(); g_prof_pool.pop_back(); return e; }
    (void)hipEventCreate(&e);
    return e;
}
bool g_mark_on = false;
int (*g_roctx_push)(const char*) = nullptr;
int (*g_roctx_pop)() = nullptr;
struct MarkScope {
    bool on;
    explicit MarkScope(const char* name) : on(g_mark_on) { if (on) (void)g_roctx_push(name); }
    ~MarkScope() { if (on) (void)g_roctx_pop(); }
};
#define SCR_MARK_FN MarkScope mark_fn_(__func__)
extern const char* const kProfNames[SCR_PROF_COUNT];
struct ProfScope {
    bool on; hipStream_t st; ProfRec r; MarkScope mark;
    ProfScope(int idx, hipStream_t s) : on((g_prof_mask >> idx) & 1u), st(s), mark(kProfNames[idx]) {
        if (on && g_prof_stride > 1) on = (g_prof_seen[idx]++ % g_prof_stride) == 0;
        if (on) { r.idx = idx; r.a = prof_event(); r.b = prof_event(); (void)hipEventRecord(r.a, st); }
    }
    ~ProfScope() { if (on) { (void)hipEventRecord(r.b, st); g_prof_recs.push_back(r); } }
};
const char* const kProfNames[SCR_PROF_COUNT] = {
    "filter_kernel", "preprocess_kernel", "plan_scan_kernel", "scatter_kernel", "tile_sort_kernel",
    "blend_forward_kernel", "blend_backward_kernel", "preprocess_backward_kernel", "expand_kernel",
    "expand_backward_kernel", "plane_sample_backward_kernels", "l1_ssim_forward_kernel",
    "l1_ssim_backward_kernel", "triplane_forward_kernel", "mlp_heads_kernel", "mlp_heads_backward_kernel",
    "norm_linear_kernels", "norm_linear_backward_kernels", "plane_attention_kernels", "flip_kernel"};
}

typedef float copy_f4 __attribute__((ext_vector_type(4)));
__global__ void __launch_bounds__(256) copy_probe_kernel(const copy_f4* __restrict__ src, copy_f4* __restrict__ dst, size_t n) {
    const size_t base = (size_t)blockIdx.x * 1024 + threadIdx.x;
    copy_f4 v[4];
#pragma unroll
    for (int u = 0; u < 4; ++u) if (base + u * 256 < n) v[u] = __builtin_nontemporal_load(&src[base + u * 256]);
#pragma unroll
    for (int u = 0; u < 4; ++u) if (base + u * 256 < n) __builtin_nontemporal_store(v[u], &dst[base + u * 256]);
}

struct Mailbox {
    volatile unsigned long long* host = nullptr;
    unsigned long long* dev = nullptr;
    unsigned long long seq = 0;
};
static Mailbox& mailbox() {
    thread_local Mailbox mb;
    thread_local bool tried = false;
    if (!tried) {
        tried = true;
        void* h = nullptr;
        if (hipHostMalloc(&h, 64, hipHostMallocPortable | hipHostMallocMapped | hipHostMallocCoherent) == hipSuccess && h) {
            void* d = nullptr;
            if (hipHostGetDevicePointer(&d, h, 0) == hipSuccess && d) {
                memset(h, 0, 64);
                mb.host = (volatile unsigned long long*)h;
                mb.dev = (unsigned long long*)d;
            } else {
                (void)hipHostFree(h);
            }
        }
        (void)hipGetLastError();
    }
    return mb;
}

static bool mailbox_wait(Mailbox& mb, unsigned long long seq, bool two, hipStream_t st) {
    if (!mb.host) return false;
    const auto t0 = std::chrono::steady_clock::now();
    for (unsigned spins = 0;; ++spins) {
        if (__atomic_load_n(&mb.host[1], __ATOMIC_ACQUIRE) == seq && (!two || __atomic_load_n(&mb.host[3], __ATOMIC_ACQUIRE) == seq))
            return true;
#if defined(__x86_64__)
        __builtin_ia32_pause();
#endif
        if ((spins & 1023u) == 1023u) {
            if (hipStreamQuery(st) != hipErrorNotReady)
                return __atomic_load_n(&mb.host[1], __ATOMIC_ACQUIRE) == seq &&
                       (!two || __atomic_load_n(&mb.host[3], __ATOMIC_ACQUIRE) == seq);
            if (std::chrono::steady_clock::now() - t0 > std::chrono::seconds(20)) return false;
        }
    }
}

static int check_settings(const scr_settings* s) {
    if (!s) return fail("settings is NULL");
    if (s->image_height <= 0 || s->image_width <= 0) return fail("image size must be positive");
    if (s->image_width > 16 * 65535 || s->image_height > 16 * 65535) return fail("image too large for 16-bit tile coordinates");
    if (!s->bg || !s->viewmatrix || !s->projmatrix || !s->campos) return fail("bg / viewmatrix / projmatrix / campos must be device pointers");
    if (s->sh_degree < 0 || s->sh_degree > 3) return fail("sh_degree must be 0..3");
    return 0;
}

extern "C" {

int scr_abi_version(void) { return SCR_ABI_VERSION; }
const char* scr_last_error(void) { return g_err; }

size_t scr_geom_bytes(int64_t P, int32_t H, int32_t W) { return geom_view(nullptr, P, H, W).bytes; }
size_t scr_binning_bytes(int64_t I, int64_t max_tile) { return bin_view(nullptr, I, max_tile).bytes; }
size_t scr_image_bytes(int32_t H, int32_t W) { return img_view(nullptr, H, W).bytes; }
size_t scr_backward_scratch_bytes(int64_t I) { return align_up((size_t)(I > 0 ? I : 1) * sizeof(GradRec)); }

int scr_visible_filter(int64_t P, const float* means3D, const float* scales, const float* rotations,
                       const float* cov3D_precomp, const scr_settings* settings, int32_t* radii_out,
                       void* stream) {
    SCR_MARK_FN;
    if (check_settings(settings)) return 1;
    if (P < 0) return fail("P < 0");
    if (P == 0) return 0;
    if (!means3D || !radii_out) return fail("means3D / radii_out is NULL");
    if (!cov3D_precomp && !(scales && rotations)) return fail("provide (scales, rotations) or cov3D_precomp");
    hipStream_t st = (hipStream_t)stream;
    { ProfScope ps_(SCR_PROF_FILTER, st);
      launch_filter(P, means3D, scales, rotations, cov3D_precomp, ksettings(settings), radii_out, st); }
    CHECK_LAUNCH("filter_kernel", settings->debug, st);
    return 0;
}

int scr_mark_visible(int64_t P, const float* means3D, const float* viewmatrix, uint8_t* present_out,
                     void* stream) {
    SCR_MARK_FN;
    if (P < 0) return fail("P < 0");
    if (P == 0) return 0;
    if (!means3D || !viewmatrix || !present_out) return fail("NULL argument");
    hipStream_t st = (hipStream_t)stream;
    launch_mark_visible(P, means3D, viewmatrix, present_out, st);
    CHECK_LAUNCH("mark_visible_kernel", 0, st);
    return 0;
}

static int plan_enqueue(int64_t P, int32_t M, const float* means3D, const float* scales, const float* rotations,
                        const float* cov3D_precomp, const float* opacities, const float* shs, const float* colors_precomp,
                        const scr_settings* settings, void* geom_buf, int32_t* radii_out, int64_t* plan_host, hipStream_t st,
                        unsigned long long& seq_out) {
    if (check_settings(settings)) return 1;
    if (P < 0) return fail("P < 0");
    if (!plan_host) return fail("plan_host is NULL");
    plan_host[0] = plan_host[1] = plan_host[3] = 0;
    if (!geom_buf) return fail("geom_buf is NULL");
    if ((shs != nullptr) == (colors_precomp != nullptr))
        return fail("pass either shs or colors_precomp (one of them, not both, not neither)");
    if (((scales != nullptr) || (rotations != nullptr)) == (cov3D_precomp != nullptr) || ((scales != nullptr) != (rotations != nullptr)))
        if (!(cov3D_precomp && !scales && !rotations) && !(scales && rotations && !cov3D_precomp))
            return fail("pass either scales + rotations or cov3D_precomp (one form of the covariance)");
    if (P > 0 && (!means3D || !opacities || !radii_out)) return fail("means3D / opacities / radii_out is NULL");
    if (P >= (1ll << ID_BITS)) return fail("P = %lld exceeds the 2^%d Gaussians a sort key can index", (long long)P, ID_BITS);
    if (shs && (M < (settings->sh_degree + 1) * (settings->sh_degree + 1)))
        return fail("shs has %d coefficients, sh_degree %d needs %d", M, settings->sh_degree,
                    (settings->sh_degree + 1) * (settings->sh_degree + 1));
    KSettings ks = ksettings(settings);
    GeomView gv = geom_view(geom_buf, P, ks.H, ks.W);
    Grid g(ks.H, ks.W);
    { ZeroList z; z.add(gv.tile_count, (size_t)g.tiles * 4, st); z.add(gv.total + 3, 8, st); launch_zero(z, st); }
    { ProfScope ps_(SCR_PROF_PREPROCESS, st);
      launch_preprocess(P, M, means3D, scales, rotations, cov3D_precomp, opacities, shs, colors_precomp, ks, gv,
                        radii_out, st); }
    CHECK_LAUNCH("preprocess_kernel", settings->debug, st);
    Mailbox& mb = mailbox();
    seq_out = ++mb.seq;
    { ProfScope ps_(SCR_PROF_PLAN_SCAN, st); launch_plan_scans(P, ks, gv, mb.dev, seq_out, st); }
    CHECK_LAUNCH("plan_scan_kernel", settings->debug, st);
    return 0;
}

static int plan_wait(const scr_settings* settings, void* geom_buf, int64_t P, unsigned long long seq, int64_t* plan_host,
                     hipStream_t st) {
    KSettings ks = ksettings(settings);
    GeomView gv = geom_view(geom_buf, P, ks.H, ks.W);
    Mailbox& mb = mailbox();
    unsigned long long total[4] = {0, 0, 0, 0};
    const bool posted = mailbox_wait(mb, seq, true, st);
    if (posted) {
        total[0] = mb.host[0];
        total[1] = mb.host[2] & 0xffffffffull;
        total[3] = mb.host[2] >> 32;
    }
    if (!posted) {
        HIP_TRY(hipMemcpyAsync(total, gv.total, 32, hipMemcpyDeviceToHost, st));
        HIP_TRY(hipStreamSynchronize(st));
    }
    if (total[0] >= 0xFFFFFFFFull)
        return fail("num_rendered >= 2^32 - 1 (counted %llu): the (Gaussian, tile) instances do not fit 32-bit indices", total[0]);
    plan_host[0] = (int64_t)total[0];
    plan_host[1] = (int64_t)total[1];
    plan_host[3] = (int64_t)total[3];
    return 0;
}

int scr_forward_plan(int64_t P, int32_t M, const float* means3D, const float* scales,
                     const float* rotations, const float* cov3D_precomp, const float* opacities,
                     const float* shs, const float* colors_precomp, const scr_settings* settings,
                     void* geom_buf, int32_t* radii_out, int64_t* plan_host, void* stream) {
    SCR_MARK_FN;
    unsigned long long seq = 0;
    const int rc = plan_enqueue(P, M, means3D, scales, rotations, cov3D_precomp, opacities, shs, colors_precomp, settings, geom_buf,
                                radii_out, plan_host, (hipStream_t)stream, seq);
    return rc ? rc : plan_wait(settings, geom_buf, P, seq, plan_host, (hipStream_t)stream);
}

static int forward_run_impl(int64_t P, int64_t I, int64_t max_tile, int64_t plan_flags, const scr_settings* settings, void* geom_buf,
                            void* binning_buf, void* image_buf, float* out_color, void* stream, bool scatter_done);

int scr_forward_run(int64_t P, int64_t I, int64_t max_tile, int64_t plan_flags, const scr_settings* settings, void* geom_buf,
                    void* binning_buf, void* image_buf, float* out_color, void* stream) {
    SCR_MARK_FN;
    return forward_run_impl(P, I, max_tile, plan_flags, settings, geom_buf, binning_buf, image_buf, out_color, stream, false);
}

static int forward_run_impl(int64_t P, int64_t I, int64_t max_tile, int64_t plan_flags, const scr_settings* settings, void* geom_buf,
                            void* binning_buf, void* image_buf, float* out_color, void* stream, bool scatter_done) {
    if (check_settings(settings)) return 1;
    if (plan_flags & ~(int64_t)(SCR_PLAN_NONFINITE_COLOUR | SCR_PLAN_LARGE_RECTS)) return fail("plan_flags %lld: not a value scr_forward_plan returned", (long long)plan_flags);
    if (!geom_buf || !binning_buf || !image_buf || !out_color) return fail("NULL buffer");
    hipStream_t st = (hipStream_t)stream;
    KSettings ks = ksettings(settings);
    GeomView gv = geom_view(geom_buf, P, ks.H, ks.W);
    BinView bv = bin_view(binning_buf, I, max_tile);
    ImgView iv = img_view(image_buf, ks.H, ks.W);
    if (I > 0) {
        if (!scatter_done) {
            { ProfScope ps_(SCR_PROF_SCATTER, st); launch_scatter(P, ks, gv, bv, ~0ull, st); }
            CHECK_LAUNCH("scatter_kernel", settings->debug, st);
        }
        { ProfScope ps_(SCR_PROF_TILE_SORT, st); launch_tile_sort(ks, gv, bv, max_tile, !deep_lists(I, Grid(ks.H, ks.W).tiles), st); }
        CHECK_LAUNCH("tile_sort_kernel", settings->debug, st);
    }
    { ProfScope ps_(SCR_PROF_BLEND_FORWARD, st); launch_blend_forward(ks, gv, bv, iv, out_color, 2 * max_tile * (int64_t)Grid(ks.H, ks.W).tiles > 3 * I,
                                                                      (plan_flags & SCR_PLAN_NONFINITE_COLOUR) != 0, st); }
    CHECK_LAUNCH("blend_forward_kernel", settings->debug, st);
    return 0;
}

int scr_forward_plan_run(int64_t P, int32_t M, const float* means3D, const float* scales, const float* rotations,
                         const float* cov3D_precomp, const float* opacities, const float* shs, const float* colors_precomp,
                         const scr_settings* settings, void* geom_buf, int32_t* radii_out, int64_t* plan_host,
                         void* binning_buf, size_t binning_capacity_bytes, void* image_buf, float* out_color, void* stream) {
    SCR_MARK_FN;
    if (!plan_host) return fail("plan_host is NULL");
    plan_host[2] = 0;
    hipStream_t st = (hipStream_t)stream;
    unsigned long long seq = 0;
    int rc = plan_enqueue(P, M, means3D, scales, rotations, cov3D_precomp, opacities, shs, colors_precomp, settings, geom_buf,
                          radii_out, plan_host, st, seq);
    if (rc) return rc;
    const unsigned long long cap = binning_buf ? (unsigned long long)(binning_capacity_bytes / 17) : 0ull;
    const bool early = binning_buf && P > 0 && cap > 0 && image_buf && out_color;
    if (early) {
        KSettings ks = ksettings(settings);
        GeomView gv = geom_view(geom_buf, P, ks.H, ks.W);
        BinView bv = bin_view(binning_buf, 0, 0);
        { ProfScope ps_(SCR_PROF_SCATTER, st); launch_scatter(P, ks, gv, bv, cap, st); }
        CHECK_LAUNCH("scatter_kernel", settings->debug, st);
    }
    rc = plan_wait(settings, geom_buf, P, seq, plan_host, st);
    if (rc) return rc;
    const bool fits = binning_buf && scr_binning_bytes(plan_host[0], plan_host[1]) <= binning_capacity_bytes;
    const bool scattered = early && (unsigned long long)plan_host[0] <= cap;
    if (!fits) {
        if (scattered && plan_host[0] > 0) {
            KSettings ks = ksettings(settings);
            GeomView gv = geom_view(geom_buf, P, ks.H, ks.W);
            ZeroList z;
            z.add(gv.cursor, (size_t)Grid(ks.H, ks.W).tiles * 4, st);
            launch_zero(z, st);
        }
        return 0;
    }
    rc = forward_run_impl(P, plan_host[0], plan_host[1], plan_host[3], settings, geom_buf, binning_buf, image_buf, out_color, stream, scattered);
    if (rc) return rc;
    plan_host[2] = 1;
    return 0;
}

int scr_backward(int64_t P, int32_t M, int64_t I, int64_t plan_flags, const float* means3D, const float* scales,
                 const float* rotations, const float* cov3D_precomp, const float* shs,
                 const scr_settings* settings, const int32_t* radii, void* geom_buf,
                 const void* binning_buf, void* image_buf, const float* dL_dcolor, void* scratch,
                 float* dL_dmeans3D, float* dL_dmeans2D, float* dL_dcolors, float* dL_dsh,
                 float* dL_dopacity, float* dL_dscales, float* dL_drotations, float* dL_dcov3D,
                 void* stream) {
    SCR_MARK_FN;
    if (check_settings(settings)) return 1;
    if (P == 0) return 0;
    if (plan_flags & ~(int64_t)(SCR_PLAN_NONFINITE_COLOUR | SCR_PLAN_LARGE_RECTS)) return fail("plan_flags %lld: not a value scr_forward_plan returned", (long long)plan_flags);
    if (!geom_buf || !binning_buf || !image_buf || !dL_dcolor || !scratch) return fail("NULL buffer");
    if (!means3D || !radii || !dL_dmeans3D || !dL_dmeans2D || !dL_dopacity) return fail("NULL argument");
    if (shs ? !dL_dsh : !dL_dcolors) return fail("colour gradient output missing");
    if (cov3D_precomp ? !dL_dcov3D : !(dL_dscales && dL_drotations && scales && rotations))
        return fail("covariance gradient output missing");
    hipStream_t st = (hipStream_t)stream;
    KSettings ks = ksettings(settings);
    GeomView gv = geom_view(geom_buf, P, ks.H, ks.W);
    BinView bv = bin_view((void*)binning_buf, I, 0);
    ImgView iv = img_view(image_buf, ks.H, ks.W);
    static std::atomic<unsigned long long> stamp_counter{0x5ca1ab1e00000000ull};
    const unsigned long long stamp = ++stamp_counter;
    if (settings->debug) {
        unsigned long long dev_flags = 0;
        HIP_TRY(hipMemcpyAsync(&dev_flags, gv.total + 3, 8, hipMemcpyDeviceToHost, st));
        HIP_TRY(hipStreamSynchronize(st));
        if ((long long)dev_flags != (long long)plan_flags)
            return fail("plan_flags %lld passed to scr_backward, but the forward pass of this geom_buf raised %llu", (long long)plan_flags, dev_flags);
    }
    if (I > 0) {
        launch_zero_far_records(P, gv, (GradRec*)scratch, st);
        CHECK_LAUNCH("zero_far_records_kernel", settings->debug, st);
        { ProfScope ps_(SCR_PROF_BLEND_BACKWARD, st);
          launch_blend_backward(ks, gv, bv, iv, dL_dcolor, (GradRec*)scratch, stamp, deep_lists(I, Grid(ks.H, ks.W).tiles),
                                record_flags(I, Grid(ks.H, ks.W).tiles), (plan_flags & SCR_PLAN_NONFINITE_COLOUR) != 0, st); }
        CHECK_LAUNCH("blend_backward_kernel", settings->debug, st);
    }
    { ProfScope ps_(SCR_PROF_PREPROCESS_BACKWARD, st);
      launch_preprocess_backward(P, M, means3D, scales, rotations, cov3D_precomp, shs, ks, radii, gv, bv,
                                 (const GradRec*)scratch, iv.cut_key, stamp, record_flags(I, Grid(ks.H, ks.W).tiles), dL_dmeans3D, dL_dmeans2D, shs ? nullptr : dL_dcolors,
                                 shs ? dL_dsh : nullptr, dL_dopacity, cov3D_precomp ? nullptr : dL_dscales,
                                 cov3D_precomp ? nullptr : dL_drotations, cov3D_precomp ? dL_dcov3D : nullptr, st); }
    CHECK_LAUNCH("preprocess_backward_kernel", settings->debug, st);
    return 0;
}

int scr_debug_force_deep_lists(int mode) {
    if (mode < -1 || mode > 1) return fail("scr_debug_force_deep_lists: -1 (automatic), 0 or 1");
    scr::g_force_deep_lists = mode;
    return 0;
}

int scr_debug_get(int which, int64_t P, int64_t I, int32_t H, int32_t W, const void* geom_buf,
                  const void* binning_buf, const void* image_buf, void* out, void* stream) {
    SCR_MARK_FN;
    hipStream_t st = (hipStream_t)stream;
    Grid g(H, W);
    const void* src = nullptr;
    size_t bytes = 0;
    if (which <= SCR_DBG_RANGES || which == SCR_DBG_SPLAT_RECORDS) {
        if (!geom_buf) return fail("geom_buf is NULL");
        GeomView gv = geom_view((void*)geom_buf, P, H, W);
        if (which == SCR_DBG_TILES_TOUCHED) { src = gv.tiles_touched; bytes = (size_t)P * 4; }
        else if (which == SCR_DBG_POINT_OFFSETS) { src = gv.point_offsets; bytes = (size_t)P * 4; }
        else if (which == SCR_DBG_RANGES) { src = gv.ranges; bytes = (size_t)g.tiles * 8; }
        else { src = gv.rec; bytes = (size_t)P * REC_F * 4; }
    } else if (which == SCR_DBG_POINT_LIST) {
        if (!binning_buf) return fail("binning_buf is NULL");
        src = bin_view((void*)binning_buf, I, 0).point_list;
        bytes = (size_t)I * 4;
    } else if (which == SCR_DBG_QMASK || which == SCR_DBG_GM_INDEX) {
        if (!binning_buf) return fail("binning_buf is NULL");
        BinView bv = bin_view((void*)binning_buf, I, 0);
        if (which == SCR_DBG_GM_INDEX && deep_lists(I, g.tiles))
            return fail("gm_index is not materialised for deep tile lists (I > 8192 per tile on average)");
        src = which == SCR_DBG_QMASK ? (const void*)bv.qmask : (const void*)bv.gm_index;
        bytes = which == SCR_DBG_QMASK ? (size_t)I : (size_t)I * 4;
    } else if (which == SCR_DBG_N_CONTRIB || which == SCR_DBG_FINAL_T) {
        if (!image_buf) return fail("image_buf is NULL");
        ImgView iv = img_view((void*)image_buf, H, W);
        src = which == SCR_DBG_N_CONTRIB ? (const void*)iv.n_contrib : (const void*)iv.final_T;
        bytes = (size_t)H * W * 4;
    } else {
        return fail("unknown debug selector %d", which);
    }
    if (bytes) HIP_TRY(hipMemcpyAsync(out, src, bytes, hipMemcpyDeviceToDevice, st));
    return 0;
}

static inline size_t expand_nwg(int64_t n) { return (size_t)((n + 1023) / 1024); }

size_t scr_expand_scratch_bytes(int64_t n) { return align_up((expand_nwg(n) + 1) * 4) + 256; }

int scr_expand_plan(int64_t n, const float* neural_opacity, void* scratch, int64_t* num_selected_host,
                    void* stream) {
    SCR_MARK_FN;
    if (!num_selected_host) return fail("num_selected_host is NULL");
    *num_selected_host = 0;
    if (n < 0) return fail("n < 0");
    if (n == 0) return 0;
    if (!neural_opacity || !scratch) return fail("NULL argument");
    if (n >= (1ll << 31)) return fail("more than 2^31 candidates");
    hipStream_t st = (hipStream_t)stream;
    uint32_t* wg = (uint32_t*)scratch;
    unsigned long long* total = (unsigned long long*)((char*)scratch + align_up((expand_nwg(n) + 1) * 4));
    Mailbox& mb = mailbox();
    const unsigned long long seq = ++mb.seq;
    { ProfScope ps_(SCR_PROF_EXPAND, st); launch_expand_count(n, neural_opacity, wg, total, mb.dev, seq, st); }
    CHECK_LAUNCH("expand_count_kernel", 0, st);
    unsigned long long t = 0;
    if (mailbox_wait(mb, seq, false, st)) {
        t = mb.host[0];
    } else {
        HIP_TRY(hipMemcpyAsync(&t, total, 8, hipMemcpyDeviceToHost, st));
        HIP_TRY(hipStreamSynchronize(st));
    }
    *num_selected_host = (int64_t)t;
    return 0;
}

int scr_mask_index_plan(int64_t n, const uint8_t* mask, void* scratch, int64_t* num_set_host, void* stream) {
    SCR_MARK_FN;
    if (!num_set_host) return fail("num_set_host is NULL");
    *num_set_host = 0;
    if (n < 0) return fail("n < 0");
    if (n == 0) return 0;
    if (!mask || !scratch) return fail("NULL argument");
    if (n >= (1ll << 31)) return fail("more than 2^31 mask entries");
    hipStream_t st = (hipStream_t)stream;
    uint32_t* wg = (uint32_t*)scratch;
    unsigned long long* total = (unsigned long long*)((char*)scratch + align_up((expand_nwg(n) + 1) * 4));
    Mailbox& mb = mailbox();
    const unsigned long long seq = ++mb.seq;
    { ProfScope ps_(SCR_PROF_EXPAND, st); launch_mask_count(n, mask, wg, total, mb.dev, seq, st); }
    CHECK_LAUNCH("mask_count_kernel", 0, st);
    unsigned long long t = 0;
    if (mailbox_wait(mb, seq, false, st)) {
        t = mb.host[0];
    } else {
        HIP_TRY(hipMemcpyAsync(&t, total, 8, hipMemcpyDeviceToHost, st));
        HIP_TRY(hipStreamSynchronize(st));
    }
    *num_set_host = (int64_t)t;
    return 0;
}

int scr_mask_index_run(int64_t n, const uint8_t* mask, const void* scratch, int64_t* index, int64_t* inverse, void* stream) {
    SCR_MARK_FN;
    if (n <= 0) return n < 0 ? fail("n < 0") : 0;
    if (!mask || !scratch || (!index && !inverse)) return fail("NULL argument");
    hipStream_t st = (hipStream_t)stream;
    { ProfScope ps_(SCR_PROF_EXPAND, st); launch_mask_index(n, mask, (const uint32_t*)scratch, index, inverse, st); }
    CHECK_LAUNCH("mask_index_kernel", 0, st);
    return 0;
}

int scr_expand_run(int64_t V, int32_t k, const float* neural_opacity, const float* color,
                   const float* scale_rot, const float* offsets, int32_t offsets_ld, const float* grid_scaling,
                   const float* anchor, const void* scratch, int32_t* out_index, uint8_t* mask_out,
                   float* xyz, float* color_out, float* opacity, float* scaling, float* rot, void* stream) {
    SCR_MARK_FN;
    if (V < 0 || k <= 0) return fail("bad V / k");
    if (offsets_ld < 3 * k) return fail("offsets_ld %d: the offset rows of an anchor are 3 k = %d floats long", offsets_ld, 3 * k);
    if (V == 0) return 0;
    if (!neural_opacity || !color || !scale_rot || !offsets || !grid_scaling || !anchor || !scratch || !out_index)
        return fail("NULL argument");
    hipStream_t st = (hipStream_t)stream;
    { ProfScope ps_(SCR_PROF_EXPAND, st);
      launch_expand_run(V * k, k, neural_opacity, color, scale_rot, offsets, offsets_ld, grid_scaling, anchor,
                        (const uint32_t*)scratch, out_index, mask_out, xyz, color_out, opacity, scaling, rot, st); }
    CHECK_LAUNCH("expand_run_kernel", 0, st);
    return 0;
}

int scr_expand_backward(int64_t V, int32_t k, const float* scale_rot, const float* offsets, int32_t offsets_ld,
                        const float* grid_scaling, const int32_t* out_index, const float* g_xyz,
                        const float* g_color, const float* g_opacity, const float* g_scaling,
                        const float* g_rot, float* d_neural_opacity, float* d_color, float* d_scale_rot,
                        float* d_offsets, float* d_grid_scaling, float* d_anchor, const float* g_reg, int64_t P,
                        void* stream) {
    SCR_MARK_FN;
    if (V < 0 || k <= 0) return fail("bad V / k");
    if (g_reg && P <= 0) return fail("scr_expand_backward: g_reg needs P = the number of selected candidates");
    if (offsets_ld < 3 * k) return fail("offsets_ld %d: the offset rows of an anchor are 3 k = %d floats long", offsets_ld, 3 * k);
    if (V == 0) return 0;
    if (!scale_rot || !offsets || !grid_scaling || !out_index || !d_neural_opacity || !d_color || !d_scale_rot ||
        !d_offsets || !d_grid_scaling || !d_anchor)
        return fail("NULL argument");
    hipStream_t st = (hipStream_t)stream;
    { ProfScope ps_(SCR_PROF_EXPAND_BACKWARD, st);
      launch_expand_backward(V, k, scale_rot, offsets, offsets_ld, grid_scaling, out_index, g_xyz, g_color, g_opacity, g_scaling,
                             g_rot, d_neural_opacity, d_color, d_scale_rot, d_offsets, d_grid_scaling, d_anchor, g_reg, P, st); }
    CHECK_LAUNCH("expand_backward_kernel", 0, st);
    return 0;
}

size_t scr_plane_sample_scratch_bytes(int64_t V, int32_t A, int32_t B, int32_t channels) {
    return triplane_scratch_bytes(V, A, B, channels);
}

int scr_plane_sample_backward(int64_t V, const float* coords, int32_t cstride, int32_t cx, int32_t cy, int32_t R,
                              int32_t A, int32_t B, int32_t planes, const float* grad_out0, const float* grad_out1,
                              int32_t ld, float* grad_plane0, float* grad_plane1, void* scratch, void* stream) {
    SCR_MARK_FN;
    if (V < 0 || R <= 0 || A <= 1 || B <= 1) return fail("bad sizes");
    if (planes != 1 && planes != 2) return fail("planes must be 1 or 2");
    if (cstride <= 0 || cx < 0 || cy < 0 || cx >= cstride || cy >= cstride || ld < R) return fail("bad strides");
    if (!grad_plane0 || !scratch || (V > 0 && (!coords || !grad_out0))) return fail("NULL argument");
    if (planes == 2 && (!grad_plane1 || (V > 0 && !grad_out1))) return fail("NULL argument (second plane)");
    hipStream_t st = (hipStream_t)stream;
    int rc;
    { ProfScope ps_(SCR_PROF_PLANE_BACKWARD, st);
      rc = launch_plane_sample_backward(V, coords, cstride, cx, cy, R, A, B, planes, grad_out0, grad_out1, ld, grad_plane0,
                                        grad_plane1, scratch, st); }
    if (rc == 1) return fail("R = %d channels per plane exceeds the supported 16", R);
    if (rc == 2) return fail("plane %dx%d has too many 32x32 tiles for the LDS histogram", A, B);
    CHECK_LAUNCH("plane_sample_backward", 0, st);
    return 0;
}

size_t scr_triplane_backward_scratch_bytes(int64_t V, int32_t X, int32_t Y, int32_t Z, int32_t channels) {
    return triplane_backward_scratch_bytes(V, X, Y, Z, channels);
}

int scr_triplane_backward(int64_t V, const float* coords, int32_t cstride, int32_t R, int32_t X, int32_t Y, int32_t Z,
                          int32_t planes, const float* grad_out, int32_t ld, const int32_t* cols, float* const* grad_planes,
                          void* scratch, void* stream) {
    SCR_MARK_FN;
    if (V < 0 || R <= 0 || X <= 1 || Y <= 1 || Z <= 1) return fail("bad sizes");
    if (planes != 1 && planes != 2) return fail("planes must be 1 or 2");
    if (cstride < 3 || ld < R * 3 * planes) return fail("bad strides");
    if (!cols || !grad_planes || !scratch || (V > 0 && (!coords || !grad_out))) return fail("NULL argument");
    for (int q = 0; q < 3 * planes; ++q) {
        if (!grad_planes[q]) return fail("NULL plane gradient %d", q);
        if (cols[q] < 0 || cols[q] + R > ld) return fail("column block %d outside the gradient rows", q);
    }
    hipStream_t st = (hipStream_t)stream;
    int rc;
    { ProfScope ps_(SCR_PROF_PLANE_BACKWARD, st);
      rc = launch_triplane_backward(V, coords, cstride, R, X, Y, Z, planes, grad_out, ld, cols, grad_planes, scratch, st); }
    if (rc == 1) return fail("R = %d channels per plane exceeds the supported 16", R);
    if (rc == 2) return fail("a plane of %dx%dx%d has too many 32x32 tiles for the LDS histogram", X, Y, Z);
    CHECK_LAUNCH("triplane_backward", 0, st);
    return 0;
}

size_t scr_triplane_backward_multi_scratch_bytes(int64_t V, int32_t ngrids, const int32_t* R, const int32_t* X, const int32_t* Y,
                                                 const int32_t* Z) {
    if (!R || !X || !Y || !Z || ngrids < 1 || ngrids > 3) return 0;
    return triplane_multi_scratch_bytes(V, ngrids, R, X, Y, Z);
}

int scr_triplane_backward_multi(int64_t V, const float* coords, int32_t cstride, int32_t ngrids, const int32_t* R,
                                const int32_t* X, const int32_t* Y, const int32_t* Z, const int32_t* col, const float* grad_out,
                                int32_t ld, float* const* grad_planes, void* scratch, const float* nl_coef, const float* nl_dy,
                                int32_t nl_lddy, const float* nl_x, int32_t nl_ldx, void* stream) {
    SCR_MARK_FN;
    if (V < 0 || ngrids < 1 || ngrids > 3) return fail("bad sizes");
    if (!R || !X || !Y || !Z || !col || !grad_planes || !scratch || (V > 0 && (!coords || (!grad_out && !nl_coef)))) return fail("NULL argument");
    if (nl_coef && (!nl_dy || !nl_x || nl_lddy < 32 || nl_ldx < col[ngrids - 1] + 3 * R[ngrids - 1])) return fail("fused dx: dy [V,32] and x (the sampled matrix) are needed");
    for (int g = 0; g < ngrids; ++g) {
        if (R[g] < 1 || X[g] < 2 || Y[g] < 2 || Z[g] < 2 || col[g] < 0 || col[g] + 3 * R[g] > (grad_out ? ld : nl_ldx)) return fail("bad grid %d", g);
        for (int q = 0; q < 3; ++q)
            if (!grad_planes[3 * g + q]) return fail("NULL plane gradient %d", 3 * g + q);
    }
    hipStream_t st = (hipStream_t)stream;
    int rc;
    { ProfScope ps_(SCR_PROF_PLANE_BACKWARD, st);
      rc = launch_triplane_backward_multi(V, coords, cstride, ngrids, R, X, Y, Z, col, grad_out, ld, grad_planes, scratch, nl_coef, nl_dy,
                                          nl_lddy, nl_x, nl_ldx, st); }
    if (rc == 3) return 3;
    CHECK_LAUNCH("triplane_backward_multi", 0, st);
    return 0;
}

int scr_plane_row_pairs(int32_t R, int32_t A, int32_t B, const float* plane, float* pairs, void* stream) {
    SCR_MARK_FN;
    if (A < 2 || B < 2) return fail("bad sizes");
    if (!plane || !pairs) return fail("NULL argument");
    if (launch_plane_row_pairs(R, A, B, plane, pairs, (hipStream_t)stream)) return fail("R = %d channels per plane exceeds the supported 16", R);
    CHECK_LAUNCH("plane_row_pairs_kernel", 0, (hipStream_t)stream);
    return 0;
}

int scr_triplane_forward(int64_t V, const float* coords, int32_t cstride, const float* xy, const float* xz,
                         const float* yz, int32_t R, int32_t X, int32_t Y, int32_t Z, int32_t channel_last, float* out,
                         int32_t ld, int32_t col_xy, int32_t col_xz, int32_t col_yz, void* stream) {
    SCR_MARK_FN;
    if (V < 0 || R <= 0 || X <= 1 || Y <= 1 || Z <= 1) return fail("bad sizes");
    if (cstride < 3 || col_xy < 0 || col_xz < 0 || col_yz < 0 || col_xy + R > ld || col_xz + R > ld || col_yz + R > ld)
        return fail("bad strides");
    if (V > 0 && (!coords || !xy || !xz || !yz || !out)) return fail("NULL argument");
    hipStream_t st = (hipStream_t)stream;
    int rc;
    { ProfScope ps_(SCR_PROF_TRIPLANE_FORWARD, st);
      rc = launch_triplane_forward(V, coords, cstride, xy, xz, yz, R, X, Y, Z, channel_last, out, ld, col_xy, col_xz, col_yz, st); }
    if (rc == 1) return fail("R = %d channels per plane exceeds the supported 16", R);
    CHECK_LAUNCH("triplane_forward_kernel", 0, st);
    return 0;
}

size_t scr_tpa_scratch_bytes(int32_t R, int32_t H, int32_t W) { return tpa_scratch_bytes(R, H, W); }

static int tpa_bad(int32_t R, int32_t H, int32_t W) {
    if (R <= 0 || 3 * R > 24) return fail("plane attention: 3 R stacked channels must be 3..24");
    if (H <= 0 || W <= 0 || (int64_t)H * W >= (1ll << 31)) return fail("plane attention: bad plane size");
    return 0;
}

int scr_tpa_stats(int32_t R, int32_t H, int32_t W, const float* p0, const float* p1, const float* p2, float* avg,
                  float* mx, int32_t* arg, void* scratch, void* stream) {
    SCR_MARK_FN;
    if (tpa_bad(R, H, W)) return 1;
    if (!p0 || !p1 || !p2 || !avg || !mx || !arg || !scratch) return fail("NULL argument");
    hipStream_t st = (hipStream_t)stream;
    { ProfScope ps_(SCR_PROF_PLANE_ATTENTION, st); launch_tpa_stats(R, (int64_t)H * W, p0, p1, p2, avg, mx, arg, scratch, st); }
    CHECK_LAUNCH("tpa_stats_kernels", 0, st);
    return 0;
}

int scr_tpa_forward(int32_t R, int32_t H, int32_t W, const float* p0, const float* p1, const float* p2, const float* ca,
                    const float* w, float* s, uint8_t* am, float* sa, float* pair0, float* pair1, float* pair2, void* stream) {
    SCR_MARK_FN;
    if (tpa_bad(R, H, W)) return 1;
    if (!p0 || !p1 || !p2 || !ca || !w || !s || !am || !sa || !pair0 || !pair1 || !pair2) return fail("NULL argument");
    hipStream_t st = (hipStream_t)stream;
    { ProfScope ps_(SCR_PROF_PLANE_ATTENTION, st); launch_tpa_forward(R, H, W, p0, p1, p2, ca, w, s, am, sa, pair0, pair1, pair2, st); }
    CHECK_LAUNCH("tpa_apply_kernel", 0, st);
    return 0;
}

int scr_tpa_backward(int32_t R, int32_t H, int32_t W, const float* p0, const float* p1, const float* p2, const float* ca,
                     const float* w, const float* s, const uint8_t* am, const float* sa, const float* g0, const float* g1,
                     const float* g2, float* d0, float* d1, float* d2, float* dca, float* dw, void* scratch, void* stream) {
    SCR_MARK_FN;
    if (tpa_bad(R, H, W)) return 1;
    if (!p0 || !p1 || !p2 || !ca || !w || !s || !am || !sa || !g0 || !g1 || !g2 || !d0 || !d1 || !d2 || !dca || !dw || !scratch)
        return fail("NULL argument");
    hipStream_t st = (hipStream_t)stream;
    { ProfScope ps_(SCR_PROF_PLANE_ATTENTION, st);
      launch_tpa_backward(R, H, W, p0, p1, p2, ca, w, s, am, sa, g0, g1, g2, d0, d1, d2, dca, dw, scratch, st); }
    CHECK_LAUNCH("tpa_bwd_kernels", 0, st);
    return 0;
}

int scr_tpa_backward_stats(int32_t R, int32_t H, int32_t W, const float* davg, const float* dmax, const int32_t* arg,
                           float* d0, float* d1, float* d2, void* stream) {
    SCR_MARK_FN;
    if (tpa_bad(R, H, W)) return 1;
    if (!davg || !dmax || !arg || !d0 || !d1 || !d2) return fail("NULL argument");
    hipStream_t st = (hipStream_t)stream;
    { ProfScope ps_(SCR_PROF_PLANE_ATTENTION, st); launch_tpa_backward_stats(R, (int64_t)H * W, davg, dmax, arg, d0, d1, d2, st); }
    CHECK_LAUNCH("tpa_bwd_stats_kernel", 0, st);
    return 0;
}

size_t scr_l1_ssim_scratch_bytes(int32_t C, int32_t H, int32_t W, int32_t with_grad) {
    return l1_ssim_scratch_bytes(C, H, W, with_grad);
}

int scr_l1_ssim_forward(int32_t C, int32_t H, int32_t W, const float* img1, const float* img2, void* scratch,
                        int32_t with_grad, float* out2, void* stream) {
    SCR_MARK_FN;
    if (C <= 0 || H <= 0 || W <= 0) return fail("bad image size");
    if (!img1 || !img2 || !scratch || !out2) return fail("NULL argument");
    hipStream_t st = (hipStream_t)stream;
    { ProfScope ps_(SCR_PROF_L1_SSIM, st); launch_l1_ssim_forward(C, H, W, img1, img2, scratch, with_grad, out2, st); }
    CHECK_LAUNCH("l1_ssim_forward_kernel", 0, st);
    return 0;
}

int scr_l1_ssim_backward(int32_t C, int32_t H, int32_t W, const float* img1, const float* img2,
                         const void* scratch, const float* g_l1, const float* g_ssim, float* dimg1,
// ... 522 lines not shown
```

### splatco_amd/csrc/common.h

```cpp
#pragma once
#include <hip/hip_runtime.h>
#include <stdint.h>

#include "../../include/splatco_raster.h"

namespace scr {

__host__ __device__ __forceinline__ uint32_t sat_add_u32(uint32_t a, uint32_t b) {
    const uint32_t s = a + b;
    return s < a ? 0xFFFFFFFFu : s;
}


constexpr int TILE = SCR_TILE;
constexpr int TILE_PIX = TILE * TILE;
constexpr int WAVE = 64;
constexpr int NUM_XCD = 8;
constexpr int PRE_BLOCK = 256;
constexpr int BIN_THREADS = 1024;
constexpr int BIN_ROUNDS = 4;
constexpr int BIN_GPW = BIN_THREADS * BIN_ROUNDS;
constexpr int LDS_HIST_MAX_TILES = 40000;
constexpr int ID_BITS = 28;
constexpr int WG_SORT_MAX = 8192;
constexpr int REC_F = 12;
constexpr int GRAD_F = 9;

inline __host__ __device__ size_t align_up(size_t x, size_t a = 256) { return (x + a - 1) / a * a; }

struct Grid {
    int W, H, gx, gy, tiles;
    __host__ __device__ Grid(int H_, int W_)
        : W(W_), H(H_), gx((W_ + TILE - 1) / TILE), gy((H_ + TILE - 1) / TILE), tiles(gx * gy) {}
};

struct GeomView {
    float4* rec;
    uint32_t* tiles_touched;
    uint32_t* point_offsets;
    uint8_t* clamped;
    uint2* gm_base;
    uint32_t* live_bits;
    uint8_t* has_rec;
    uint32_t* block_sums;
    uint32_t* tile_count;
    uint32_t* ranges;
    uint32_t* cursor;
    int64_t P;
    unsigned long long* total;
    size_t bytes;
};

inline __host__ GeomView geom_view(void* base, int64_t P, int H, int W) {
    Grid g(H, W);
    char* p = (char*)base;
    size_t off = 0;
    GeomView v;
    auto take = [&](size_t n) { char* q = p ? p + off : nullptr; off += align_up(n); return q; };
    size_t nblk = (size_t)((P + BIN_GPW - 1) / BIN_GPW);
    v.rec = (float4*)take((size_t)P * REC_F * 4);
    v.tiles_touched = (uint32_t*)take((size_t)P * 4);
    v.point_offsets = (uint32_t*)take((size_t)P * 4);
    v.clamped = (uint8_t*)take((size_t)P);
    v.gm_base = (uint2*)take((size_t)P * 8);
    v.live_bits = (uint32_t*)take((size_t)P * 4);
    v.has_rec = (uint8_t*)take((size_t)P);
    v.block_sums = (uint32_t*)take((nblk + 1) * 4);
    v.tile_count = (uint32_t*)take((size_t)g.tiles * 4);
    v.ranges = (uint32_t*)take((size_t)g.tiles * 8);
    v.cursor = (uint32_t*)take((size_t)g.tiles * 4);
    v.total = (unsigned long long*)take(128);
    v.bytes = off;
    v.P = P;
    return v;
}

extern int g_force_deep_lists;
inline __host__ bool deep_lists(int64_t I, int tiles) {
    return g_force_deep_lists >= 0 ? g_force_deep_lists != 0 : I > (int64_t)8192 * tiles;
}

constexpr int FLAGS_MIN_MEAN = 2048;
inline __host__ bool record_flags(int64_t I, int tiles) {
    return g_force_deep_lists >= 0 ? g_force_deep_lists != 0 : I > (int64_t)FLAGS_MIN_MEAN * tiles;
}

struct BinView {
    unsigned long long* keys;
    uint32_t* point_list;
    uint32_t* gm_index;
    uint8_t* qmask;
    unsigned long long* keys2;
    size_t bytes;
};

inline __host__ BinView bin_view(void* base, int64_t I, int64_t max_tile_instances) {
    char* p = (char*)base;
    size_t off = 0;
    BinView v;
    auto take = [&](size_t n) { char* q = p ? p + off : nullptr; off += align_up(n); return q; };
    size_t n = (size_t)(I > 0 ? I : 1);
    v.keys = (unsigned long long*)take(n * 8);
    v.point_list = (uint32_t*)take(n * 4);
    v.gm_index = (uint32_t*)take(n * 4);
    v.qmask = (uint8_t*)take(n);
    const bool merge = max_tile_instances > WG_SORT_MAX;
    v.keys2 = merge ? (unsigned long long*)take(n * 8) : nullptr;
    v.bytes = off;
    return v;
}

struct __attribute__((packed, aligned(4))) GradQuad { float x, y, z, w; };
struct __attribute__((packed, aligned(4))) GradRec { GradQuad a, b; float c; };
static_assert(sizeof(GradRec) == 36, "36-byte gradient records");

struct ImgView {
    float* final_T;
    uint32_t* n_contrib;
    unsigned long long* cut_key;
    size_t bytes;
};

inline __host__ ImgView img_view(void* base, int H, int W) {
    char* p = (char*)base;
    size_t off = 0;
    ImgView v;
    auto take = [&](size_t n) { char* q = p ? p + off : nullptr; off += align_up(n); return q; };
    v.final_T = (float*)take((size_t)H * W * 4);
    v.n_contrib = (uint32_t*)take((size_t)H * W * 4);
    v.cut_key = (unsigned long long*)take((size_t)Grid(H, W).tiles * 8 + 8);
    v.bytes = off;
    return v;
}

struct KSettings {
    int H, W;
    float tanfovx, tanfovy, fx, fy;
    const float* bg;
    float scale_modifier;
    const float* view;
    const float* proj;
    int sh_degree;
    const float* campos;
};

inline __host__ KSettings ksettings(const scr_settings* s) {
    KSettings k;
    k.H = s->image_height;
    k.W = s->image_width;
    k.tanfovx = s->tanfovx;
    k.tanfovy = s->tanfovy;
    k.fx = (float)s->image_width / (2.0f * s->tanfovx);
    k.fy = (float)s->image_height / (2.0f * s->tanfovy);
    k.bg = s->bg;
    k.scale_modifier = s->scale_modifier;
    k.view = s->viewmatrix;
    k.proj = s->projmatrix;
    k.sh_degree = s->sh_degree;
    k.campos = s->campos;
    return k;
}

__device__ __forceinline__ float sel(unsigned long long mask, float t, float f) {
    float r;
    asm("v_cndmask_b32_e64 %0, %1, %2, %3" : "=v"(r) : "v"(f), "v"(t), "s"(mask));
    return r;
}
__device__ __forceinline__ uint32_t sel(unsigned long long mask, uint32_t t, uint32_t f) {
    uint32_t r;
    asm("v_cndmask_b32_e64 %0, %1, %2, %3" : "=v"(r) : "v"(f), "v"(t), "s"(mask));
    return r;
}
__device__ __forceinline__ float vmin(float a, float b) {
    float r;
    asm("v_min_f32 %0, %1, %2" : "=v"(r) : "v"(a), "v"(b));
    return r;
}
__device__ __forceinline__ unsigned long long lanes(bool p) { return __builtin_amdgcn_ballot_w64(p); }
__device__ __forceinline__ bool nonfinite3(float a, float b, float c) {
    constexpr int NAN_OR_INF = 0x1 | 0x2 | 0x4 | 0x200;
    return __builtin_amdgcn_classf(a, NAN_OR_INF) || __builtin_amdgcn_classf(b, NAN_OR_INF) || __builtin_amdgcn_classf(c, NAN_OR_INF);
}

__device__ inline int xcd_tile(int block, int tiles) {
    int chunk = (tiles + NUM_XCD - 1) / NUM_XCD;
    int t = (block % NUM_XCD) * chunk + block / NUM_XCD;
    return t < tiles ? t : -1;
}
inline __host__ int xcd_grid(int tiles) { return ((tiles + NUM_XCD - 1) / NUM_XCD) * NUM_XCD; }
__host__ __device__ inline int xcd_of_tile(int t, int gx) {
    const int tx = t % gx, ty = t / gx;
    return ((tx >> 2) + (ty >> 2) * ((gx + 3) >> 2)) % NUM_XCD;
}

struct SplatForm {
    float mx, my, a, b, c, thr;
    float vy, vx;
    bool ok;
};
__device__ inline SplatForm splat_form(float4 r0, float4 r1) {
    SplatForm f;
    f.mx = r0.x; f.my = r0.y;
    f.a = -r0.z; f.b = -r0.w; f.c = -r1.x;
    f.thr = __logf(255.0f * r1.y) + 0.01f;
    f.ok = (f.a > 0.0f && f.c > 0.0f && 4.0f * f.a * f.c - f.b * f.b > 0.0f) && (f.mx - f.mx == 0.0f) &&
           (f.my - f.my == 0.0f) && (f.thr - f.thr == 0.0f);
    f.vy = -f.b / (2.0f * f.c);
    f.vx = -f.b / (2.0f * f.a);
    return f;
}
template <int S>
__device__ inline uint32_t box_mask4(float4 r0, float4 r1, int box_x0, int box_y0) {
    const SplatForm f = splat_form(r0, r1);
    if (!f.ok) return 0xfu;
    const float x0 = (float)box_x0, y0 = (float)box_y0;
    float dxl[2], dxh[2], dyl[2], dyh[2];
    float cx[2], cy[2], qx[2], qy[2], bcx[2], bcy[2], sy[2], sx[2];
#pragma unroll
    for (int h = 0; h < 2; ++h) {
        dxh[h] = f.mx - (x0 + (float)(S * h));
        dxl[h] = f.mx - (x0 + (float)(S * h + S - 1));
        dyh[h] = f.my - (y0 + (float)(S * h));
        dyl[h] = f.my - (y0 + (float)(S * h + S - 1));
        cx[h] = __builtin_amdgcn_fmed3f(0.0f, dxl[h], dxh[h]);
        cy[h] = __builtin_amdgcn_fmed3f(0.0f, dyl[h], dyh[h]);
        qx[h] = f.a * cx[h] * cx[h];
        qy[h] = f.c * cy[h] * cy[h];
        bcx[h] = f.b * cx[h];
        bcy[h] = f.b * cy[h];
        sy[h] = f.vy * cx[h];
        sx[h] = f.vx * cy[h];
    }
    uint32_t mask = 0;
#pragma unroll
    for (int q = 0; q < 4; ++q) {
        const int hx = q & 1, hy = q >> 1;
        const float v = __builtin_amdgcn_fmed3f(sy[hx], dyl[hy], dyh[hy]);
        const float t1 = bcx[hx] * v, t2 = f.c * v * v;
        const float qv = qx[hx] + t1 + t2, magv = qx[hx] + fabsf(t1) + t2;
        const float u = __builtin_amdgcn_fmed3f(sx[hy], dxl[hx], dxh[hx]);
        const float s1 = bcy[hy] * u, s2 = f.a * u * u;
        const float qh = qy[hy] + s1 + s2, magh = qy[hy] + fabsf(s1) + s2;
        const bool far = qv > __builtin_fmaf(1.0e-5f, magv, f.thr) && qh > __builtin_fmaf(1.0e-5f, magh, f.thr);
        if (!far) mask |= 1u << q;
    }
    return mask;
}
__device__ inline uint32_t quadrant_mask(float4 r0, float4 r1, int tile_x0, int tile_y0) { return box_mask4<8>(r0, r1, tile_x0, tile_y0); }


struct ZeroList {
    static constexpr int MAX = 20;
    void* p[MAX];
    unsigned long long n[MAX];
    int count = 0;
    bool full() const { return count >= MAX; }
    void add(void* ptr, size_t bytes, hipStream_t st);
};
void launch_zero(const ZeroList& z, hipStream_t st);
void launch_zero_far_records(int64_t P, const GeomView& gv, GradRec* grad_rec, hipStream_t st);
inline void ZeroList::add(void* ptr, size_t bytes, hipStream_t st) {
    if (!ptr || !bytes) return;
    if (full()) { launch_zero(*this, st); count = 0; }
    p[count] = ptr;
    n[count] = bytes;
    ++count;
}

void allow_dynamic_lds(const void* kernel, size_t bytes);

void launch_box_coords(int64_t V, const float* xyz, const float* lo, const float* hi, float* out, hipStream_t st);
int launch_nl_fold(int L, int d, const int* dd, const int* col, const unsigned char* col_at, const float* const* W,
                   const float* const* b, const float* const* gamma, const float* const* beta, float* G, float* c,
                   hipStream_t st);
int launch_nl_fold_backward(int L, int d, const int* dd, const int* col, const unsigned char* col_at, const float* const* W,
                            const float* const* gamma, const float* const* beta, const float* dG, const float* dc,
                            float* const* dW, float* const* db, float* const* dgamma, float* const* dbeta, hipStream_t st);
int launch_nl_running_stats(int L, int d, const int* dd, const int* col, const unsigned char* col_at, const float* momentum,
                            float* const* run_mean, float* const* run_var, long long* const* batches, const float* mean,
                            const float* var, int64_t n, hipStream_t st);
void launch_filter(int64_t P, const float* means3D, const float* scales, const float* rotations,
                   const float* cov3D, const KSettings& ks, int32_t* radii, hipStream_t st);
void launch_mark_visible(int64_t P, const float* means3D, const float* view, uint8_t* out, hipStream_t st);
void launch_preprocess(int64_t P, int M, const float* means3D, const float* scales, const float* rotations,
                       const float* cov3D, const float* opacities, const float* shs, const float* colors,
                       const KSettings& ks, const GeomView& gv, int32_t* radii, hipStream_t st);
void launch_plan_scans(int64_t P, const KSettings& ks, const GeomView& gv, unsigned long long* mailbox,
                       unsigned long long seq, hipStream_t st);
void launch_scatter(int64_t P, const KSettings& ks, const GeomView& gv, const BinView& bv, unsigned long long cap_instances,
                    hipStream_t st);
void launch_tile_sort(const KSettings& ks, const GeomView& gv, const BinView& bv, int64_t max_tile_instances,
                      bool with_gm_index, hipStream_t st);
void launch_blend_forward(const KSettings& ks, const GeomView& gv, const BinView& bv, const ImgView& iv,
                          float* out_color, bool longest_first, bool safe, hipStream_t st);
void launch_blend_backward(const KSettings& ks, const GeomView& gv, const BinView& bv, const ImgView& iv,
                           const float* dL_dcolor, GradRec* grad_rec, unsigned long long stamp, bool deep, bool flags,
                           bool safe, hipStream_t st);
void launch_preprocess_backward(int64_t P, int M, const float* means3D, const float* scales,
                                const float* rotations, const float* cov3D, const float* shs,
                                const KSettings& ks, const int32_t* radii, const GeomView& gv,
                                const BinView& bv, const GradRec* grad_rec, const unsigned long long* cut_key,
                                unsigned long long stamp, bool deep, float* dL_dmeans3D,
                                float* dL_dmeans2D, float* dL_dcolors, float* dL_dsh, float* dL_dopacity,
                                float* dL_dscales, float* dL_drotations, float* dL_dcov3D, hipStream_t st);

void launch_expand_count(int64_t n, const float* neural_opacity, uint32_t* wg_count, unsigned long long* total,
                         unsigned long long* mailbox, unsigned long long seq, hipStream_t st);
void launch_mask_count(int64_t n, const uint8_t* mask, uint32_t* wg_count, unsigned long long* total,
                       unsigned long long* mailbox, unsigned long long seq, hipStream_t st);
void launch_mask_index(int64_t n, const uint8_t* mask, const uint32_t* wg_offset, int64_t* index, int64_t* inverse,
                       hipStream_t st);
void launch_expand_run(int64_t n, int k, const float* neural_opacity, const float* color, const float* scale_rot,
                       const float* offsets, int ldo, const float* grid_scaling, const float* anchor,
                       const uint32_t* wg_offset, int32_t* out_index, uint8_t* mask_out, float* xyz,
                       float* color_out, float* opacity, float* scaling, float* rot, hipStream_t st);
void launch_expand_backward(int64_t V, int k, const float* scale_rot, const float* offsets, int ldo,
                            const float* grid_scaling, const int32_t* out_index, const float* g_xyz,
                            const float* g_color, const float* g_opacity, const float* g_scaling,
                            const float* g_rot, float* d_neural_opacity, float* d_color, float* d_scale_rot,
                            float* d_offsets, float* d_grid_scaling, float* d_anchor, const float* g_reg, int64_t P,
                            hipStream_t st);

void launch_statis_compute(int64_t V, int k, const float* neural_opacity, const int32_t* out_index,
                           const uint8_t* update_filter, const float* grad, int gstride, float* inc_opacity,
                           float* inc_grad, hipStream_t st);
void launch_statis_apply(int64_t V, int k, const int64_t* visible_index, const float* inc_opacity, const float* inc_grad,
                         float* opacity_accum, float* anchor_demon, float* offset_gradient_accum, float* offset_denom,
                         hipStream_t st);

constexpr int NL_DP = 80;
int anchor_gather_stat_rows(int64_t V);
int64_t anchor_gather_stat_buffer_rows(int64_t V);
void launch_anchor_gather(int64_t V, const int64_t* idx, const float* p_feat, const float* p_anchor, const float* p_offset,
                          const float* p_scaling, float* feat, float* anchor, float* offsets, float* grid_scaling,
                          float* g_fea, int ldg, float* stats, hipStream_t st);
void launch_anchor_gather_backward(int64_t N, int64_t V, const int64_t* inv, const float* grid_scaling, const float* d_feat,
                                   const float* d_anchor, const float* d_offsets, const float* d_grid_scaling,
                                   const float* d_g_fea, int ldg, float* g_feat, float* g_anchor, float* g_offset,
                                   float* g_scaling, int accumulate, const float* nl_coef, const float* nl_dy, int nl_lddy,
                                   const float* nl_x, int nl_ldx, hipStream_t st);
void launch_knn(int64_t N, int k, const float* grid9, const float* sorted_pts, const int64_t* sorted_id,
                const int32_t* cell_start, int64_t* out_idx, hipStream_t st);
void launch_knn_curvature(int64_t N, int k, const float* pts, const int64_t* idx, float* curvature, hipStream_t st);
void launch_wg_scan(uint32_t nwg, uint32_t* wg_count, unsigned long long* total, unsigned long long* mailbox,
                    unsigned long long seq, hipStream_t st);
size_t points_bounds_nwg(int64_t N);
void launch_points_bounds(int64_t N, const float* pts, float* partial, float* out, hipStream_t st);
size_t voxel_unique_nwg(int64_t n);
void launch_voxel_keys(int64_t N, const float* pts, float v, const int32_t* lo, int packed, int64_t* out, hipStream_t st);
void launch_voxel_unique_count(int64_t n, const int64_t* keys, uint32_t* wg_count, unsigned long long* total,
                               unsigned long long* mailbox, unsigned long long seq, hipStream_t st);
void launch_voxel_unique_write(int64_t n, const int64_t* keys, const uint32_t* wg_offset, float v, const int32_t* lo,
                               float* out, hipStream_t st);
void launch_knn3_cell_keys(int64_t N, const float* grid8, const float* pts, int64_t* keys, hipStream_t st);
void launch_knn3_dist2(int64_t N, const float* grid8, const float* sorted_pts, const int64_t* sorted_id,
                       const int32_t* cell_start, float* out, hipStream_t st);
size_t norm_linear_scratch_bytes(int64_t V);
int launch_norm_linear_forward(int64_t V, int d, const float* x, int ldx, const float* G, const float* c, float eps, float* y,
                               float* mean, float* var, float* inv, void* scratch, const float* stats, int stat_rows,
                               hipStream_t st);
int launch_norm_linear_backward(int64_t V, int d, const float* x, int ldx, const float* dy, int lddy, const float* G,
                                const float* mean, const float* inv, float* dx, int lddx, float* dG, float* dc, void* scratch,
                                float* coef_out, hipStream_t st);
size_t mlp_heads_hidden_bytes(int64_t V);
size_t mlp_heads_partial_bytes(int64_t V);
void launch_mlp_heads_forward(int64_t V, const float* feat, int ldf, const float* anchor, const float* campos, const float* geo_a, const float* geo_b,
                              const float* w1, const float* b1, const float* w2o, const float* b2o, const float* w2c,
                              const float* b2c, const float* w2v, const float* b2v, void* hidden_save, float* out_o,
                              float* out_c, float* out_v, hipStream_t st);
void launch_mlp_heads_backward(int64_t V, const float* feat, int ldf, const float* anchor, const float* campos, const float* geo_a, const float* geo_b,
                               const float* w1, const float* w2o, const float* w2c, const float* w2v,
                               const void* hidden_save, const float* out_o, const float* out_c, const float* g_o,
                               const float* g_c, const float* g_v, void* partial, float* d_feat, float* d_anchor,
                               float* d_geo_a, float* d_geo_b, float* d_w1, float* d_b1, float* d_w2o, float* d_b2o, float* d_w2c,
                               float* d_b2c, float* d_w2v, float* d_b2v, hipStream_t st);

size_t tpa_scratch_bytes(int R, int H, int W);
void launch_tpa_stats(int R, int64_t HW, const float* p0, const float* p1, const float* p2, float* avg, float* mx,
                      int* arg, void* scratch, hipStream_t st);
void launch_tpa_forward(int R, int H, int W, const float* p0, const float* p1, const float* p2, const float* ca,
                        const float* w, float* s, uint8_t* am, float* sa, float* o0, float* o1, float* o2, hipStream_t st);
void launch_tpa_backward(int R, int H, int W, const float* p0, const float* p1, const float* p2, const float* ca,
                         const float* w, const float* s, const uint8_t* am, const float* sa, const float* g0,
                         const float* g1, const float* g2, float* d0, float* d1, float* d2, float* dca, float* dw,
                         void* scratch, hipStream_t st);
void launch_tpa_backward_stats(int R, int64_t HW, const float* davg, const float* dmx, const int* arg, float* d0,
                               float* d1, float* d2, hipStream_t st);

size_t l1_ssim_scratch_bytes(int C, int H, int W, int with_grad);
int flip_radii(double ppd, int* rc, int* rf);
int flip_filters(double ppd, double* w, int* radii, double* scalars);
size_t flip_scratch_bytes(int N, int H, int W);
int launch_flip_forward(int N, int H, int W, const float* test, const float* ref, double ppd, int quantize,
                        void* scratch, float* mean_out, float* mse_out, float* map_out, hipStream_t st);
size_t scaling_reg_scratch_bytes(int64_t P);
size_t pair_l1_scratch_bytes(int64_t n);
void launch_pair_l1_forward(int64_t n, const float* g1, const float* g2, const float* r1, const float* r2, void* scratch, float* out,
                            hipStream_t st);
void launch_pair_l1_backward(int64_t n, const float* g1, const float* g2, const float* r1, const float* r2, const float* g, float* d1,
                             float* d2, hipStream_t st);
void launch_scaling_reg_forward(int64_t P, const float* s, void* scratch, float* out, hipStream_t st);
void launch_scaling_reg_backward(int64_t P, const float* s, const float* g, float* ds, hipStream_t st);
void launch_l1_ssim_forward(int C, int H, int W, const float* img1, const float* img2, void* scratch,
                            int with_grad, float* out2, hipStream_t st);
void launch_l1_ssim_backward(int C, int H, int W, const float* img1, const float* img2, const void* scratch,
                             const float* g_l1, const float* g_ssim, float* dimg1, hipStream_t st);
size_t triplane_multi_scratch_bytes(int64_t V, int ngrids, const int* R, const int* X, const int* Y, const int* Z);
int launch_triplane_backward_multi(int64_t V, const float* coords, int cs, int ngrids, const int* R, const int* X, const int* Y,
                                   const int* Z, const int* col, const float* grad, int ld, float* const* grad_planes,
                                   void* scratch, const float* nl_coef, const float* nl_dy, int nl_lddy, const float* nl_x,
                                   int nl_ldx, hipStream_t st);
int launch_norm_linear_dx(int64_t V, int d, const float* x, int ldx, const float* dy, int lddy, const float* coef3, float* dx,
                          int lddx, hipStream_t st);
int launch_plane_row_pairs(int R, int A, int B, const float* plane, float* pairs, hipStream_t st);
size_t triplane_scratch_bytes(int64_t V, int A, int B, int channels);
size_t triplane_backward_scratch_bytes(int64_t V, int X, int Y, int Z, int channels);
int launch_triplane_backward(int64_t V, const float* coords, int cs, int R, int X, int Y, int Z, int planes,
                             const float* grad_out, int ld, const int* cols, float* const* grad_planes, void* scratch,
                             hipStream_t st);
int launch_plane_sample_backward(int64_t V, const float* coords, int cs, int cx, int cy, int R, int A, int B, int planes,
                                 const float* grad_out0, const float* grad_out1, int ld, float* grad_plane0,
                                 float* grad_plane1, void* scratch, hipStream_t st);
int launch_triplane_forward(int64_t V, const float* coords, int cs, const float* xy, const float* xz, const float* yz,
                             int R, int X, int Y, int Z, int channel_last, float* out, int ld, int col_xy, int col_xz,
                             int col_yz, hipStream_t st);

}
```

### splatco_amd/rasterizer.py

```python
from typing import NamedTuple

import ctypes as C
import os

import torch
import torch.nn as nn

from . import _C


class GaussianRasterizationSettings(NamedTuple):
    image_height: int
    image_width: int
    tanfovx: float
    tanfovy: float
    bg: torch.Tensor
    scale_modifier: float
    viewmatrix: torch.Tensor
    projmatrix: torch.Tensor
    sh_degree: int
    campos: torch.Tensor
    prefiltered: bool
    debug: bool


def _dev_f32(t, name):
    if t is None:
        return None
    if not t.is_cuda:
        raise RuntimeError(f"{name} must be a device tensor (the rasterizer has no CPU path)")
    if t.dtype != torch.float32 or not t.is_contiguous():
        t = t.contiguous().float()
    return t


class _CSettings:

    def __init__(self, rs: GaussianRasterizationSettings):
        self.bg = _dev_f32(rs.bg, "bg")
        self.view = _dev_f32(rs.viewmatrix, "viewmatrix")
        self.proj = _dev_f32(rs.projmatrix, "projmatrix")
        self.campos = _dev_f32(rs.campos, "campos")
        s = _C.Settings()
        s.image_height, s.image_width = int(rs.image_height), int(rs.image_width)
        s.tanfovx, s.tanfovy = float(rs.tanfovx), float(rs.tanfovy)
        s.bg, s.viewmatrix, s.projmatrix, s.campos = (self.bg.data_ptr(), self.view.data_ptr(),
                                                      self.proj.data_ptr(), self.campos.data_ptr())
        s.scale_modifier = float(rs.scale_modifier)
        s.sh_degree = int(rs.sh_degree)
        s.prefiltered, s.debug = int(bool(rs.prefiltered)), int(bool(rs.debug))
        self.c = s
        self.H, self.W = s.image_height, s.image_width

    def ref(self):
        return C.byref(self.c)


class RasterState:
    __slots__ = ("P", "M", "I", "max_tile", "flags", "cs", "geom", "binning", "image", "radii")

    def debug(self, which):
        dev = self.geom.device
        tiles = ((self.cs.W + 15) // 16) * ((self.cs.H + 15) // 16)
        shapes = {
            _C.DBG_TILES_TOUCHED: ((self.P,), torch.int32), _C.DBG_POINT_OFFSETS: ((self.P,), torch.int32),
            _C.DBG_RANGES: ((tiles, 2), torch.int32), _C.DBG_POINT_LIST: ((self.I,), torch.int32),
            _C.DBG_N_CONTRIB: ((self.cs.H, self.cs.W), torch.int32),
            _C.DBG_FINAL_T: ((self.cs.H, self.cs.W), torch.float32),
            _C.DBG_SPLAT_RECORDS: ((self.P, 12), torch.float32),
            _C.DBG_QMASK: ((self.I,), torch.uint8), _C.DBG_GM_INDEX: ((self.I,), torch.int32),
        }
        shape, dt = shapes[which]
        out = torch.empty(shape, dtype=dt, device=dev)
        if out.numel():
          with torch.cuda.device(dev):
            _C.check(_C.lib.scr_debug_get(which, self.P, self.I, self.cs.H, self.cs.W, _C.ptr(self.geom),
                                          _C.ptr(self.binning), _C.ptr(self.image), out.data_ptr(), _C.stream()))
        return out


SPECULATE = os.environ.get("SPLATCO_SPECULATIVE_BINNING", "1") != "0"
_plan_guess = {}


def rasterize_forward(cs, means3D, opacities, scales, rotations, cov3D_precomp, shs, colors_precomp):
    dev = means3D.device
    P = means3D.shape[0]
    M = 0 if shs is None else shs.shape[1]
    st = RasterState()
    st.P, st.M, st.cs = P, M, cs
    st.geom = _C.scratch(_C.lib.scr_geom_bytes(P, cs.H, cs.W), dev)
    st.image = _C.scratch(_C.lib.scr_image_bytes(cs.H, cs.W), dev)
    radii = torch.empty(P, dtype=torch.int32, device=dev)
    color = torch.empty(3, cs.H, cs.W, dtype=torch.float32, device=dev)
    plan = (C.c_int64 * 4)(0, 0, 0, 0)
    key = (dev.index, cs.H, cs.W)
    guess = _plan_guess.get(key)
    spec = None
    with torch.cuda.device(dev):
        if SPECULATE and guess is not None and guess[0] > 0 and 0.5 <= P / guess[0] <= 2.0:
            scale = 1.06 * P / guess[0]
            cap = _C.lib.scr_binning_bytes(min(int(guess[1] * scale) + 4096, (1 << 32) - 2), max(int(guess[2] * 1.25), guess[2] + 64))
            spec = _C.scratch(cap, dev)
        _C.check(_C.lib.scr_forward_plan_run(P, M, _C.ptr(means3D), _C.ptr(scales), _C.ptr(rotations), _C.ptr(cov3D_precomp),
                                             _C.ptr(opacities), _C.ptr(shs), _C.ptr(colors_precomp), cs.ref(),
                                             st.geom.data_ptr(), _C.ptr(radii), plan, None if spec is None else spec.data_ptr(),
                                             0 if spec is None else spec.numel(), st.image.data_ptr(), color.data_ptr(), _C.stream()))
        st.I, st.max_tile, st.flags = int(plan[0]), int(plan[1]), int(plan[3])
        _plan_guess[key] = (P, st.I, st.max_tile)
        if plan[2]:
            st.binning = spec
        else:
            del spec
            st.binning = _C.scratch(_C.lib.scr_binning_bytes(st.I, st.max_tile), dev)
            _C.check(_C.lib.scr_forward_run(P, st.I, st.max_tile, st.flags, cs.ref(), st.geom.data_ptr(), st.binning.data_ptr(),
                                            st.image.data_ptr(), color.data_ptr(), _C.stream()))
    st.radii = radii
    return color, radii, st


def _debug_dump(path, raster_settings, **tensors):
    try:
        blob = {"raster_settings": {k: (v.detach().cpu() if isinstance(v, torch.Tensor) else v)
                                    for k, v in raster_settings._asdict().items()}}
        blob.update({k: (None if v is None else v.detach().cpu()) for k, v in tensors.items()})
        torch.save(blob, path)
        return f" (inputs written to {path})"
    except Exception as e:
        return f" (could not write {path}: {e})"


class _RasterizeGaussians(torch.autograd.Function):
    @staticmethod
    def forward(ctx, means3D, means2D, sh, colors_precomp, opacities, scales, rotations, cov3Ds_precomp,
                raster_settings):
        cs = _CSettings(raster_settings)
        ctx.set_materialize_grads(False)
        means3D = _dev_f32(means3D, "means3D")
        none_if_empty = lambda t, n: None if t is None or t.numel() == 0 else _dev_f32(t, n)
        sh, colors_precomp = none_if_empty(sh, "shs"), none_if_empty(colors_precomp, "colors_precomp")
        scales, rotations = none_if_empty(scales, "scales"), none_if_empty(rotations, "rotations")
        cov3Ds_precomp = none_if_empty(cov3Ds_precomp, "cov3D_precomp")
        opacities = _dev_f32(opacities, "opacities")
        P = means3D.shape[0]
        if P == 0:
            color = cs.bg.reshape(3, 1, 1).expand(3, cs.H, cs.W).contiguous()
            radii = torch.zeros(0, dtype=torch.int32, device=means3D.device)
            ctx.state = None
            ctx.shapes = (means3D, means2D, sh, colors_precomp, opacities, scales, rotations, cov3Ds_precomp)
            ctx.mark_non_differentiable(radii)
            return color, radii
        try:
            color, radii, st = rasterize_forward(cs, means3D, opacities, scales, rotations, cov3Ds_precomp, sh,
                                                 colors_precomp)
        except RuntimeError as e:
            if raster_settings.debug:
                raise RuntimeError(str(e) + _debug_dump("snapshot_fw.dump", raster_settings, means3D=means3D, sh=sh,
                                                        colors_precomp=colors_precomp, opacities=opacities, scales=scales,
                                                        rotations=rotations, cov3Ds_precomp=cov3Ds_precomp)) from e
            raise
        ctx.state = st
        ctx.raster_settings = raster_settings
        ctx.save_for_backward(means3D, scales, rotations, cov3Ds_precomp, sh, colors_precomp, opacities)
        ctx.m2d_shape = tuple(means2D.shape)
        ctx.mark_non_differentiable(radii)
        return color, radii

    @staticmethod
    def backward(ctx, grad_out_color, _grad_radii):
        st = ctx.state
        if st is None:
            return tuple(None if t is None else torch.zeros_like(t) for t in ctx.shapes) + (None,)
        if grad_out_color is None:
            return (None,) * 9
        means3D, scales, rotations, cov3D, sh, colors, opacities = ctx.saved_tensors
        dev, P, cs = means3D.device, st.P, st.cs
        g = _dev_f32(grad_out_color, "grad_out_color")
        widths = [3, 3 if colors is not None else 0, 3 * st.M if sh is not None else 0, 1,
                  3 if cov3D is None else 0, 4 if cov3D is None else 0, 6 if cov3D is not None else 0]
        arena = torch.empty(P * sum(widths), dtype=torch.float32, device=dev)
        parts, off = [], 0
        for w in widths:
            parts.append(arena[off:off + P * w].view(P, w) if w else None)
            off += P * w
        g_means3D, g_col, g_sh, g_op, g_scales, g_rot, g_cov = parts
        g_means2D = torch.empty(P, 3, dtype=torch.float32, device=dev)
        if g_sh is not None:
            g_sh = g_sh.view(P, st.M, 3)
        del arena, parts
        scratch = _C.scratch(_C.lib.scr_backward_scratch_bytes(st.I), dev)
        try:
          with torch.cuda.device(dev):
            _C.check(_C.lib.scr_backward(P, st.M, st.I, st.flags, _C.ptr(means3D), _C.ptr(scales), _C.ptr(rotations), _C.ptr(cov3D),
                                         _C.ptr(sh), cs.ref(), st.radii.data_ptr(), st.geom.data_ptr(),
                                         st.binning.data_ptr(), st.image.data_ptr(), g.data_ptr(), scratch.data_ptr(),
                                         g_means3D.data_ptr(), g_means2D.data_ptr(), _C.ptr(g_col), _C.ptr(g_sh),
                                         g_op.data_ptr(), _C.ptr(g_scales), _C.ptr(g_rot), _C.ptr(g_cov), _C.stream()))
        except RuntimeError as e:
            if ctx.raster_settings.debug:
                raise RuntimeError(str(e) + _debug_dump("snapshot_bw.dump", ctx.raster_settings, means3D=means3D, sh=sh,
                                                        colors_precomp=colors, opacities=opacities, scales=scales,
                                                        rotations=rotations, cov3Ds_precomp=cov3D, radii=st.radii,
                                                        grad_out_color=g)) from e
            raise
        g_op = g_op.reshape(opacities.shape)
        if ctx.m2d_shape != (P, 3):
            g_means2D = g_means2D[:, :ctx.m2d_shape[1]].reshape(ctx.m2d_shape) if len(ctx.m2d_shape) == 2 else None
        return g_means3D, g_means2D, g_sh, g_col, g_op, g_scales, g_rot, g_cov, None


def rasterize_gaussians(means3D, means2D, sh, colors_precomp, opacities, scales, rotations, cov3Ds_precomp,
                        raster_settings):
    return _RasterizeGaussians.apply(means3D, means2D, sh, colors_precomp, opacities, scales, rotations,
                                     cov3Ds_precomp, raster_settings)


class GaussianRasterizer(nn.Module):

    def __init__(self, raster_settings):
        super().__init__()
        self.raster_settings = raster_settings

    def markVisible(self, positions):
        with torch.no_grad():
            positions = _dev_f32(positions, "positions")
            P = positions.shape[0]
            out = torch.zeros(P, dtype=torch.uint8, device=positions.device)
            view = _dev_f32(self.raster_settings.viewmatrix, "viewmatrix")
            if P:
                with torch.cuda.device(positions.device):
                    _C.check(_C.lib.scr_mark_visible(P, positions.data_ptr(), view.data_ptr(), out.data_ptr(), _C.stream()))
            return out.bool()

    def forward(self, means3D, means2D, opacities, shs=None, colors_precomp=None, scales=None, rotations=None,
                cov3D_precomp=None):
        if (shs is None and colors_precomp is None) or (shs is not None and colors_precomp is not None):
            raise ValueError('GaussianRasterizer: pass either shs or colors_precomp (one of them, not both, not neither)')
        if ((scales is None or rotations is None) and cov3D_precomp is None) or \
                ((scales is not None or rotations is not None) and cov3D_precomp is not None):
            raise ValueError('GaussianRasterizer: pass either scales + rotations or cov3D_precomp (one form of the covariance, not both, not neither)')
        empty = torch.Tensor([])
        return rasterize_gaussians(
            means3D, means2D, empty if shs is None else shs, empty if colors_precomp is None else colors_precomp,
            opacities, empty if scales is None else scales, empty if rotations is None else rotations,
            empty if cov3D_precomp is None else cov3D_precomp, self.raster_settings)

    def visible_filter(self, means3D, scales=None, rotations=None, cov3D_precomp=None):
        if ((scales is None or rotations is None) and cov3D_precomp is None) or \
                ((scales is not None or rotations is not None) and cov3D_precomp is not None):
            raise ValueError('GaussianRasterizer: pass either scales + rotations or cov3D_precomp (one form of the covariance, not both, not neither)')
        with torch.no_grad():
            cs = _CSettings(self.raster_settings)
            means3D = _dev_f32(means3D, "means3D")
            scales, rotations = _dev_f32(scales, "scales"), _dev_f32(rotations, "rotations")
            cov3D_precomp = _dev_f32(cov3D_precomp, "cov3D_precomp")
            P = means3D.shape[0]
            radii = torch.empty(P, dtype=torch.int32, device=means3D.device)
            if P:
                with torch.cuda.device(means3D.device):
                    _C.check(_C.lib.scr_visible_filter(P, means3D.data_ptr(), _C.ptr(scales), _C.ptr(rotations),
                                                       _C.ptr(cov3D_precomp), cs.ref(), radii.data_ptr(), _C.stream()))
            return radii
```

Measured before the change: 1082 Msplats/s.

## Compact per-tile live splat lists during sorting and blend only live entries

The final tile-sort stage now writes a compacted list holding only splats whose quadrant mask is nonzero, packing key and original index, along with a per-tile live count. Blend forward and backward, and the longest-first tile ordering, consume the compacted list and live counts instead of the full ranges and qmask. The aim is to cut blend iterations and metadata loads for splats that touch no quadrant of the tile. In exchange, the sort kernels pay extra ballot and scan work and an 8-byte-per-instance live buffer, which also lowers binning capacity. A per-pixel n_live array is added as well.

```diff
diff --git a/include/splatco_raster.h b/include/splatco_raster.h
--- a/include/splatco_raster.h
+++ b/include/splatco_raster.h
@@ -8,7 +8,7 @@
 extern "C" {
 #endif
 
-#define SCR_ABI_VERSION 29
+#define SCR_ABI_VERSION 30
 #define SCR_TILE 16
 
 typedef struct scr_settings {
@@ -74,7 +74,9 @@
     SCR_DBG_FINAL_T = 5,
     SCR_DBG_SPLAT_RECORDS = 6,
     SCR_DBG_QMASK = 7,
-    SCR_DBG_GM_INDEX = 8
+    SCR_DBG_GM_INDEX = 8,
+    SCR_DBG_LIVE_LIST = 9,
+    SCR_DBG_LIVE_COUNT = 10
 };
 int scr_debug_force_deep_lists(int mode);
 int scr_debug_get(int which, int64_t P, int64_t num_rendered, int32_t image_height, int32_t image_width,
diff --git a/splatco_amd/_C.py b/splatco_amd/_C.py
--- a/splatco_amd/_C.py
+++ b/splatco_amd/_C.py
@@ -8,11 +8,11 @@
 
 PLAN_NONFINITE_COLOUR, PLAN_LARGE_RECTS = 1, 2
 PROF_COUNT = 20
-ABI_VERSION = 29
+ABI_VERSION = 30
 FLIP_MAX_RADIUS = 16
 
 (DBG_TILES_TOUCHED, DBG_POINT_OFFSETS, DBG_RANGES, DBG_POINT_LIST, DBG_N_CONTRIB, DBG_FINAL_T, DBG_SPLAT_RECORDS, DBG_QMASK,
- DBG_GM_INDEX) = range(9)
+ DBG_GM_INDEX, DBG_LIVE_LIST, DBG_LIVE_COUNT) = range(11)
 
 vp, cp, u8, i32, i64, f32, f64, sz = C.c_void_p, C.c_char_p, C.c_uint8, C.c_int32, C.c_int64, C.c_float, C.c_double, C.c_size_t
 P = C.POINTER
diff --git a/splatco_amd/csrc/binning.hip b/splatco_amd/csrc/binning.hip
--- a/splatco_amd/csrc/binning.hip
+++ b/splatco_amd/csrc/binning.hip
@@ -236,37 +236,69 @@
     uint32_t* point_list;
     uint32_t* gm_index;
     uint8_t* qmask;
+    uint2* live;
     int tx, ty;
-    __device__ __forceinline__ void write(uint32_t i, uint32_t klo) const {
-        const uint32_t id = klo >> 4;
-        point_list[i] = id;
-        qmask[i] = (uint8_t)(klo & 15u);
-        if (gm_index) {
-            const uint2 b = gm_base[id];
-            gm_index[i] = b.x + (uint32_t)ty * b.y + (uint32_t)tx;
-        }
-    }
     template <int U, typename GetK>
-    __device__ __forceinline__ void write_batch(uint32_t lo, uint32_t e0, uint32_t stride, uint32_t cnt, GetK getk) const {
+    __device__ __forceinline__ uint32_t write_tile_wave(uint32_t lo, uint32_t cnt, GetK getk) const {
+        const uint32_t lane = threadIdx.x & 63;
         uint32_t k[U];
         uint2 b[U];
 #pragma unroll
         for (int u = 0; u < U; ++u) {
-            const uint32_t e = e0 + (uint32_t)u * stride;
+            const uint32_t e = (uint32_t)u * 64u + lane;
             k[u] = e < cnt ? getk(e, u) : 0u;
         }
         if (gm_index) {
 #pragma unroll
-            for (int u = 0; u < U; ++u) b[u] = gm_base[k[u] >> 4];
+            for (int u = 0; u < U; ++u)
+                if (k[u] & 15u) b[u] = gm_base[k[u] >> 4];
         }
         __builtin_amdgcn_sched_barrier(0);
+        uint32_t base = 0;
 #pragma unroll
         for (int u = 0; u < U; ++u) {
-            const uint32_t e = e0 + (uint32_t)u * stride;
+            const uint32_t e = (uint32_t)u * 64u + lane;
+            const bool lv = (k[u] & 15u) != 0u;
+            const unsigned long long bal = lanes(lv);
             if (e < cnt) {
                 point_list[lo + e] = k[u] >> 4;
                 qmask[lo + e] = (uint8_t)(k[u] & 15u);
-                if (gm_index) gm_index[lo + e] = b[u].x + (uint32_t)ty * b[u].y + (uint32_t)tx;
+            }
+            if (lv) {
+                const uint32_t r = base + lanes_below(bal);
+                live[lo + r] = make_uint2(k[u], e);
+                if (gm_index) gm_index[lo + r] = b[u].x + (uint32_t)ty * b[u].y + (uint32_t)tx;
+            }
+            base += (uint32_t)__builtin_popcountll(bal);
+        }
+        return base;
+    }
+    template <int U, bool ALL, typename GetK>
+    __device__ __forceinline__ void write_batch_ranked(uint32_t lo, uint32_t at, uint32_t e0, uint32_t stride, uint32_t cnt, GetK getk) const {
+        unsigned long long k[U];
+        uint2 b[U];
+#pragma unroll
+        for (int u = 0; u < U; ++u) {
+            const uint32_t e = e0 + (uint32_t)u * stride;
+            k[u] = e < cnt ? getk(e) : 0ull;
+        }
+        auto is_live = [&](int u) { return e0 + (uint32_t)u * stride < cnt && (ALL || ((uint32_t)k[u] & 15u) != 0u); };
+        if (gm_index) {
+#pragma unroll
+            for (int u = 0; u < U; ++u)
+                if (is_live(u)) b[u] = gm_base[(uint32_t)k[u] >> 4];
+        }
+        __builtin_amdgcn_sched_barrier(0);
+#pragma unroll
+        for (int u = 0; u < U; ++u) {
+            const uint32_t e = e0 + (uint32_t)u * stride, klo = (uint32_t)k[u], r = (uint32_t)(k[u] >> 32);
+            if (e < cnt) {
+                point_list[lo + at + e] = klo >> 4;
+                qmask[lo + at + e] = (uint8_t)(klo & 15u);
+            }
+            if (is_live(u)) {
+                live[lo + r] = make_uint2(klo, at + e);
+                if (gm_index) gm_index[lo + r] = b[u].x + (uint32_t)ty * b[u].y + (uint32_t)tx;
             }
         }
     }
@@ -287,8 +319,8 @@
 }
 
 template <int E, bool FINAL>
-__device__ __forceinline__ void wave_sort(uint32_t n, unsigned long long* __restrict__ keys, uint32_t lo,
-                                          const FinalLists& fl, uint32_t* __restrict__ tr) {
+__device__ __forceinline__ uint32_t wave_sort(uint32_t n, unsigned long long* __restrict__ keys, uint32_t lo,
+                                              const FinalLists& fl, uint32_t* __restrict__ tr) {
     const int lane = threadIdx.x & 63;
     uint32_t klo[E], khi[E];
     wave_sort_regs<E>(n, keys, klo, khi);
@@ -306,20 +338,21 @@
     transpose(klo);
     if (!FINAL) transpose(khi);
     if (FINAL) {
-        fl.template write_batch<E>(lo, (uint32_t)lane, 64u, n, [&](uint32_t, int u) { return klo[u]; });
+        return fl.template write_tile_wave<E>(lo, n, [&](uint32_t, int u) { return klo[u]; });
     } else {
 #pragma unroll
         for (int e = 0; e < E; ++e) {
             const uint32_t i = (uint32_t)e * 64 + lane;
             if (i < n) keys[i] = ((unsigned long long)khi[e] << 32) | klo[e];
         }
+        return 0u;
     }
 }
 
 __device__ __forceinline__ int split_slot(int p) { return p + (p >> 3); }
 constexpr int SPLIT_SLOTS = WAVE_SORT_MAX + WAVE_SORT_MAX / 8;
 template <int EA, int EB>
-__device__ __forceinline__ void wave_sort_split(uint32_t n, const unsigned long long* __restrict__ keys, uint32_t lo,
+__device__ __forceinline__ uint32_t wave_sort_split(uint32_t n, const unsigned long long* __restrict__ keys, uint32_t lo,
                                                 const FinalLists& fl, unsigned long long* __restrict__ mb) {
     constexpr int NA = 64 * EA, NB = 64 * EB, PER = EA + EB;
     const int lane = threadIdx.x & 63;
@@ -367,37 +400,42 @@
 #pragma unroll
     for (int k = 0; k < PER; ++k) tr[lane * (PER + 1) + k] = outk[k];
     __syncthreads();
-    fl.template write_batch<PER>(lo, (uint32_t)lane, 64u, n, [&](uint32_t i, int) { return tr[i + i / PER]; });
+    return fl.template write_tile_wave<PER>(lo, n, [&](uint32_t i, int) { return tr[i + i / PER]; });
 }
 
 template <bool FINAL>
-__device__ __forceinline__ void wave_sort_any(uint32_t n, unsigned long long* keys, uint32_t lo, const FinalLists& fl,
-                                              unsigned long long* mb) {
+__device__ __forceinline__ uint32_t wave_sort_any(uint32_t n, unsigned long long* keys, uint32_t lo, const FinalLists& fl,
+                                                  unsigned long long* mb) {
     uint32_t* tr = (uint32_t*)mb;
-    if (n <= 64) wave_sort<1, FINAL>(n, keys, lo, fl, tr);
-    else if (n <= 128) wave_sort<2, FINAL>(n, keys, lo, fl, tr);
-    else if (n <= 256) wave_sort<4, FINAL>(n, keys, lo, fl, tr);
-    else if (FINAL && n > 256 && n <= 320) wave_sort_split<4, 1>(n, keys, lo, fl, mb);
-    else if (FINAL && n > 256 && n <= 384) wave_sort_split<4, 2>(n, keys, lo, fl, mb);
-    else if (n <= 512) wave_sort<8, FINAL>(n, keys, lo, fl, tr);
-    else if (FINAL && n <= 576) wave_sort_split<8, 1>(n, keys, lo, fl, mb);
-    else if (FINAL && n <= 640) wave_sort_split<8, 2>(n, keys, lo, fl, mb);
-    else if (FINAL && n <= 768) wave_sort_split<8, 4>(n, keys, lo, fl, mb);
-    else if (FINAL) wave_sort_split<8, 8>(n, keys, lo, fl, mb);
-    else wave_sort<16, FINAL>(n, keys, lo, fl, tr);
+    if (n <= 64) return wave_sort<1, FINAL>(n, keys, lo, fl, tr);
+    else if (n <= 128) return wave_sort<2, FINAL>(n, keys, lo, fl, tr);
+    else if (n <= 256) return wave_sort<4, FINAL>(n, keys, lo, fl, tr);
+    else if (FINAL && n > 256 && n <= 320) return wave_sort_split<4, 1>(n, keys, lo, fl, mb);
+    else if (FINAL && n > 256 && n <= 384) return wave_sort_split<4, 2>(n, keys, lo, fl, mb);
+    else if (n <= 512) return wave_sort<8, FINAL>(n, keys, lo, fl, tr);
+    else if (FINAL && n <= 576) return wave_sort_split<8, 1>(n, keys, lo, fl, mb);
+    else if (FINAL && n <= 640) return wave_sort_split<8, 2>(n, keys, lo, fl, mb);
+    else if (FINAL && n <= 768) return wave_sort_split<8, 4>(n, keys, lo, fl, mb);
+    else if (FINAL) return wave_sort_split<8, 8>(n, keys, lo, fl, mb);
+    else return wave_sort<16, FINAL>(n, keys, lo, fl, tr);
 }
 
 __global__ void __launch_bounds__(64, 1)
 tile_sort_wave_kernel(int tiles, int gx, const uint32_t* __restrict__ ranges, unsigned long long* __restrict__ keys,
                       const uint2* __restrict__ gm_base, uint32_t* __restrict__ point_list,
-                      uint32_t* __restrict__ gm_index, uint8_t* __restrict__ qmask) {
+                      uint32_t* __restrict__ gm_index, uint8_t* __restrict__ qmask, uint2* __restrict__ live,
+                      uint32_t* __restrict__ live_n) {
     int t = xcd_tile(blockIdx.x, tiles);
     if (t < 0) return;
     const uint32_t lo = ranges[2 * t], n = ranges[2 * t + 1] - lo;
-    if (n == 0 || n > (uint32_t)WAVE_SORT_MAX) return;
-    const FinalLists fl{gm_base, point_list, gm_index, qmask, t % gx, t / gx};
-    __shared__ unsigned long long mb[SPLIT_SLOTS];
-    wave_sort_any<true>(n, keys + lo, lo, fl, mb);
+    if (n > (uint32_t)WAVE_SORT_MAX) return;
+    uint32_t nl = 0;
+    if (n) {
+        const FinalLists fl{gm_base, point_list, gm_index, qmask, live, t % gx, t / gx};
+        __shared__ unsigned long long mb[SPLIT_SLOTS];
+        nl = wave_sort_any<true>(n, keys + lo, lo, fl, mb);
+    }
+    if (threadIdx.x == 0) live_n[t] = nl;
 }
 
 constexpr int WG_SORT_THREADS = WG_SORT_MAX / 16;
@@ -405,8 +443,10 @@
 __global__ void __launch_bounds__(WG_SORT_THREADS)
 tile_sort_wg_kernel(int tiles, int gx, const uint32_t* __restrict__ ranges, unsigned long long* __restrict__ keys,
                     const uint2* __restrict__ gm_base, uint32_t* __restrict__ point_list,
-                    uint32_t* __restrict__ gm_index, uint8_t* __restrict__ qmask) {
+                    uint32_t* __restrict__ gm_index, uint8_t* __restrict__ qmask, uint2* __restrict__ live,
+                    uint32_t* __restrict__ live_n) {
     extern __shared__ __attribute__((aligned(16))) unsigned long long buf[];
+    __shared__ uint32_t scan_lds[WG_SORT_THREADS / WAVE + 1];
     int t = xcd_tile(blockIdx.x, tiles);
     if (t < 0) return;
     const uint32_t lo = ranges[2 * t], n = ranges[2 * t + 1] - lo;
@@ -461,10 +501,24 @@
     }
     const unsigned long long* src = buf;
     if (n <= (uint32_t)WG_SORT_MAX) {
-        const FinalLists fl{gm_base, point_list, gm_index, qmask, t % gx, t / gx};
+        constexpr int PER = WG_SORT_MAX / WG_SORT_THREADS;
+        const uint32_t o0 = threadIdx.x * PER;
+        uint32_t mine = 0, total;
+#pragma unroll
+        for (int k = 0; k < PER; ++k) mine += o0 + k < cnt && ((uint32_t)buf[wg_slot((int)(o0 + k))] & 15u) != 0u;
+        uint32_t r = block_exclusive_scan<WG_SORT_THREADS>(mine, scan_lds, total);
+#pragma unroll
+        for (int k = 0; k < PER; ++k) {
+            const uint32_t klo = (uint32_t)buf[wg_slot((int)(o0 + k))];
+            if (o0 + k < cnt && (klo & 15u) != 0u) buf[wg_slot((int)(o0 + k))] = ((unsigned long long)r++ << 32) | klo;
+        }
+        __syncthreads();
+        if (threadIdx.x == 0) live_n[t] = total;
+        const FinalLists fl{gm_base, point_list, gm_index, qmask, live, t % gx, t / gx};
         for (uint32_t e = threadIdx.x; e < cnt; e += 4 * WG_SORT_THREADS)
-            fl.template write_batch<4>(lo, e, (uint32_t)WG_SORT_THREADS, cnt, [&](uint32_t i, int) { return (uint32_t)src[wg_slot((int)i)]; });
+            fl.template write_batch_ranked<4, false>(lo, 0u, e, (uint32_t)WG_SORT_THREADS, cnt, [&](uint32_t i) { return src[wg_slot((int)i)]; });
     } else {
+        if (blockIdx.y == 0 && threadIdx.x == 0) live_n[t] = n;
         for (uint32_t e = threadIdx.x; e < cnt; e += WG_SORT_THREADS) chunk[e] = src[wg_slot((int)e)];
     }
 }
@@ -501,7 +555,7 @@
 tile_merge_path_kernel(int tiles, int gx, uint32_t pass, const uint32_t* __restrict__ ranges,
                        const unsigned long long* __restrict__ src, unsigned long long* __restrict__ dst,
                        const uint2* __restrict__ gm_base, uint32_t* __restrict__ point_list,
-                       uint32_t* __restrict__ gm_index, uint8_t* __restrict__ qmask) {
+                       uint32_t* __restrict__ gm_index, uint8_t* __restrict__ qmask, uint2* __restrict__ live) {
     __shared__ unsigned long long buf[MP_SEG + MP_SEG / 16];
     __shared__ uint32_t cut[2];
     int t = xcd_tile(blockIdx.x, tiles);
@@ -572,9 +626,12 @@
         if (d0 + k < tot) buf[wg_slot((int)(d0 + k))] = outk[k];
     __syncthreads();
     if (pass + 1 == merge_passes_needed(n)) {
-        const FinalLists fl{gm_base, point_list, gm_index, qmask, t % gx, t / gx};
+        const FinalLists fl{gm_base, point_list, gm_index, qmask, live, t % gx, t / gx};
+        const uint32_t at = pairbase + s0;
         for (uint32_t e = threadIdx.x; e < tot; e += 4 * 256)
-            fl.template write_batch<4>(lo + pairbase + s0, e, 256u, tot, [&](uint32_t i, int) { return (uint32_t)buf[wg_slot((int)i)]; });
+            fl.template write_batch_ranked<4, true>(lo, at, e, 256u, tot, [&](uint32_t i) {
+                return ((unsigned long long)(at + i) << 32) | (uint32_t)buf[wg_slot((int)i)];
+            });
     } else {
         unsigned long long* out = dst + lo + pairbase + s0;
         for (uint32_t e = threadIdx.x; e < tot; e += 256) out[e] = buf[wg_slot((int)e)];
@@ -612,13 +669,13 @@
     const unsigned gt = (unsigned)xcd_grid(g.tiles);
     if (max_tile_instances <= 0) return;
     tile_sort_wave_kernel<<<gt, 64, 0, st>>>(g.tiles, g.gx, gv.ranges, bv.keys, gv.gm_base, bv.point_list, gm_index,
-                                             bv.qmask);
+                                             bv.qmask, bv.live, gv.live_n);
     if (max_tile_instances <= WAVE_SORT_MAX) return;
     const unsigned chunks = (unsigned)((max_tile_instances + WG_SORT_MAX - 1) / WG_SORT_MAX);
     const size_t lds = (size_t)(WG_SORT_MAX + WG_SORT_MAX / 16) * 8;
     allow_dynamic_lds((const void*)tile_sort_wg_kernel, lds);
     tile_sort_wg_kernel<<<dim3(gt, chunks), WG_SORT_THREADS, lds, st>>>(g.tiles, g.gx, gv.ranges, bv.keys, gv.gm_base, bv.point_list,
-                                                                        gm_index, bv.qmask);
+                                                                        gm_index, bv.qmask, bv.live, gv.live_n);
     if (chunks <= 1) return;
     unsigned passes = 0;
     while ((1u << passes) < chunks) ++passes;
@@ -627,8 +684,8 @@
         const unsigned long long* src = (p & 1u) ? bv.keys2 : bv.keys;
         unsigned long long* dst = (p & 1u) ? bv.keys : bv.keys2;
         tile_merge_path_kernel<<<dim3(gt, segs), 256, 0, st>>>(g.tiles, g.gx, p, gv.ranges, src, dst, gv.gm_base,
-                                                               bv.point_list, gm_index, bv.qmask);
-    }
-}
-
-}
+                                                               bv.point_list, gm_index, bv.qmask, bv.live);
+    }
+}
+
+}
diff --git a/splatco_amd/csrc/blend.hip b/splatco_amd/csrc/blend.hip
--- a/splatco_amd/csrc/blend.hip
+++ b/splatco_amd/csrc/blend.hip
@@ -51,12 +51,8 @@
     return __builtin_fmaf(g, r, g);
 }
 
-__device__ __forceinline__ uint32_t lanes_below(unsigned long long ballot) {
-    return __builtin_amdgcn_mbcnt_hi((uint32_t)(ballot >> 32), __builtin_amdgcn_mbcnt_lo((uint32_t)ballot, 0u));
-}
-
 __global__ void __launch_bounds__(1024)
-tile_order_kernel(int tiles, int gx, const uint32_t* __restrict__ ranges, uint32_t* __restrict__ order,
+tile_order_kernel(int tiles, int gx, const uint32_t* __restrict__ live_n, uint32_t* __restrict__ order,
                   unsigned long long* __restrict__ ordered, unsigned long long* __restrict__ first) {
     __shared__ uint32_t hist[1024], start[1024], wsum[16];
     __shared__ uint32_t s_max, cnt[NUM_XCD];
@@ -70,7 +66,7 @@
         const int x = xcd_of_tile(t, gx);
 #pragma unroll
         for (int q = 0; q < NUM_XCD; ++q) mine[q] += x == q;
-        if (x == me) mx = max(mx, ranges[2 * t + 1] - ranges[2 * t]);
+        if (x == me) mx = max(mx, live_n[t]);
     }
 #pragma unroll
     for (int q = 0; q < NUM_XCD; ++q)
@@ -82,7 +78,7 @@
     const float scale = 1023.0f / (float)s_max;
     for (int t = threadIdx.x; t < tiles; t += 1024) {
         if (xcd_of_tile(t, gx) != me) continue;
-        const uint32_t n = ranges[2 * t + 1] - ranges[2 * t];
+        const uint32_t n = live_n[t];
         atomicAdd(&hist[1023 - min(1023u, (uint32_t)((float)n * scale))], 1u);
     }
     __syncthreads();
@@ -103,7 +99,7 @@
     __syncthreads();
     for (int t = threadIdx.x; t < tiles; t += 1024) {
         if (xcd_of_tile(t, gx) != me) continue;
-        const uint32_t n = ranges[2 * t + 1] - ranges[2 * t];
+        const uint32_t n = live_n[t];
         order[off + atomicAdd(&start[1023 - min(1023u, (uint32_t)((float)n * scale))], 1u)] = (uint32_t)t;
     }
     if (threadIdx.x == 0) {
@@ -131,10 +127,10 @@
 __global__ void __launch_bounds__(64)
 blend_forward_kernel(int W, int H, int gx, int tiles, const uint32_t* __restrict__ order, const unsigned long long* __restrict__ total,
                      const uint32_t* __restrict__ ranges,
-                     const uint32_t* __restrict__ point_list, const uint8_t* __restrict__ qmask,
+                     const uint2* __restrict__ live, const uint32_t* __restrict__ live_n,
                      const float4* __restrict__ rec, const float* __restrict__ bg,
                      float* __restrict__ out_color, float* __restrict__ final_T,
-                     uint32_t* __restrict__ n_contrib) {
+                     uint32_t* __restrict__ n_contrib, uint32_t* __restrict__ n_live) {
     __shared__ float4 sp[5][FCHUNK / 2];
     const int quad = (blockIdx.x / NUM_XCD) & 3;
     const int t = blend_tile((int)(blockIdx.x % NUM_XCD + (blockIdx.x / (4 * NUM_XCD)) * NUM_XCD), tiles, order, total);
@@ -144,7 +140,8 @@
     const int py = (t / gx) * TILE + (quad >> 1) * 8 + (lane >> 3);
     const bool inside = px < W && py < H;
     const float pxf = (float)px, pyf = (float)py;
-    const uint32_t lo = ranges[2 * t], n = ranges[2 * t + 1] - lo;
+    const uint32_t lo = ranges[2 * t];
+    const uint32_t n = ranges[2 * t + 1] > lo ? live_n[t] : 0u;
     unsigned long long done = lanes(!inside);
     SCR_COUNT_DECL;
     float T = 1.0f, C0 = 0.0f, C1 = 0.0f, C2 = 0.0f;
@@ -158,9 +155,9 @@
     float r2x = 0.0f;
     auto load_mask_id = [&](uint32_t base, uint32_t& m, uint32_t& id) {
         uint32_t i = base + lane;
-        bool have = i < n;
-        m = have ? ((qmask[lo + i] >> quad) & 1u) : 0u;
-        id = have ? point_list[lo + i] : 0u;
+        const uint32_t klo = i < n ? live[lo + i].x : 0u;
+        m = (klo >> quad) & 1u;
+        id = klo >> 4;
     };
     auto gather = [&](uint32_t m, uint32_t id) {
         sel_cur = m != 0;
@@ -272,7 +269,8 @@
         out_color[hw + pix] = __builtin_fmaf(T, bg[1], C1);
         out_color[2 * hw + pix] = __builtin_fmaf(T, bg[2], C2);
         final_T[pix] = T;
-        n_contrib[pix] = last;
+        n_live[pix] = last;
+        n_contrib[pix] = last ? live[lo + last - 1].y + 1u : 0u;
     }
 }
 
@@ -341,11 +339,10 @@
 __global__ void __launch_bounds__(256, BWD_MIN_WAVES)
 blend_backward_kernel(int W, int H, int gx, int tiles, const uint32_t* __restrict__ order, const unsigned long long* __restrict__ total,
                       const uint32_t* __restrict__ ranges,
-                      const uint32_t* __restrict__ point_list, const uint32_t* __restrict__ gm_index,
-                      const uint2* __restrict__ gm_base,
-                      const uint8_t* __restrict__ qmask, const float4* __restrict__ rec,
+                      const uint2* __restrict__ live, const uint32_t* __restrict__ live_n, const uint32_t* __restrict__ gm_index,
+                      const uint2* __restrict__ gm_base, const float4* __restrict__ rec,
                       const float* __restrict__ bg, const float* __restrict__ final_T,
-                      const uint32_t* __restrict__ n_contrib, const float* __restrict__ dL_dpix,
+                      const uint32_t* __restrict__ n_live, const float* __restrict__ dL_dpix,
                       GradRec* __restrict__ grad_rec, unsigned long long* __restrict__ cut_key, unsigned long long stamp,
                       uint8_t* __restrict__ has_rec) {
     __shared__ float4 st[4][3][BCH + 4];
@@ -355,7 +352,7 @@
     __shared__ uint32_t wave_max[4];
     const int t = blend_tile((int)blockIdx.x, tiles, order, total);
     if (t < 0) return;
-    const uint32_t lo = ranges[2 * t], n = ranges[2 * t + 1] - lo;
+    const uint32_t lo = ranges[2 * t], n = live_n[t];
     if (n == 0) return;
     const int wave = threadIdx.x >> 6, lane = threadIdx.x & 63;
     const int qx0 = (t % gx) * TILE + (wave & 1) * 8, qy0 = (t / gx) * TILE + (wave >> 1) * 8;
@@ -364,7 +361,7 @@
     const float pxf = (float)px, pyf = (float)py;
     const float qx0f = (float)qx0, qy0f = (float)qy0;
     const size_t pix = (size_t)py * W + px, hw = (size_t)H * W;
-    const uint32_t last = inside ? n_contrib[pix] : 0u;
+    const uint32_t last = inside ? n_live[pix] : 0u;
     PixState ps;
     ps.T = inside ? final_T[pix] : 0.0f;
     ps.dLp0 = ps.dLp1 = ps.dLp2 = 0.0f;
@@ -422,7 +419,7 @@
     if (threadIdx.x == 0) {
         unsigned long long ck = ~0ull;
         if (cut) {
-            const uint32_t idc = point_list[lo + (uint32_t)(live_top + 1) * BCH];
+            const uint32_t idc = live[lo + (uint32_t)(live_top + 1) * BCH].x >> 4;
             ck = ((unsigned long long)__float_as_uint(rec[3 * (size_t)idc + 2].y) << 32) | idc;
             cut_key[tiles] = stamp;
         }
@@ -437,32 +434,32 @@
     if (!cut && wave < 3)
         for (int ci = nround - 1; ci > live_top; --ci) {
             const uint32_t i = (uint32_t)ci * BCH + lane;
-            if (i < n && qmask[lo + i] != 0) {
-                GradRec& gr = grad_rec[gm_of(lo + i, point_list[lo + i])];
+            const uint32_t klo = i < n ? live[lo + i].x : 0u;
+            if ((klo & 15u) != 0u) {
+                GradRec& gr = grad_rec[gm_of(lo + i, klo >> 4)];
                 if (wave == 0) store16_dword_aligned(&gr.a, make_float4(0, 0, 0, 0));
                 else if (wave == 1) store16_dword_aligned(&gr.b, make_float4(0, 0, 0, 0));
                 else gr.c = 0.0f;
             }
         }
 
-    uint32_t m_next = 0, id_next = 0, slot_next = 0;
-    uint32_t m_cur = 0, slot_cur = 0, id_cur = 0;
+    uint32_t k_next = 0, slot_next = 0;
+    uint32_t k_cur = 0, slot_cur = 0;
     bool sel_cur = false;
     float4 r0 = make_float4(0, 0, 0, 0), r1 = r0;
     float r2x = 0.0f;
-    auto load_meta = [&](int ci, uint32_t& m, uint32_t& id, uint32_t& slot) {
+    auto load_meta = [&](int ci, uint32_t& klo, uint32_t& slot) {
         const uint32_t i = (uint32_t)ci * BCH + lane;
         const bool have = ci >= 0 && i < n;
-        m = have ? qmask[lo + i] : 0u;
-        id = have ? point_list[lo + i] : 0u;
-        slot = have ? gm_of(lo + i, id) : 0u;
+        klo = have ? live[lo + i].x : 0u;
+        slot = have ? gm_of(lo + i, klo >> 4) : 0u;
     };
-    auto gather = [&](int ci, uint32_t m, uint32_t id, uint32_t slot) {
+    auto gather = [&](int ci, uint32_t klo, uint32_t slot) {
         const uint32_t i = (uint32_t)ci * BCH + lane;
-        sel_cur = ((m >> wave) & 1u) && i < wave_last;
-        m_cur = m;
+        const uint32_t id = klo >> 4;
+        sel_cur = ((klo >> wave) & 1u) && i < wave_last;
+        k_cur = klo;
         slot_cur = slot;
-        id_cur = id;
         if (sel_cur) {
             r0 = rec[3 * (size_t)id];
             r1 = rec[3 * (size_t)id + 1];
@@ -470,10 +467,10 @@
         }
     };
     if (live_top >= 0) {
-        uint32_t m0, id0, sl0;
-        load_meta(live_top, m0, id0, sl0);
-        gather(live_top, m0, id0, sl0);
-        load_meta(live_top - 1, m_next, id_next, slot_next);
+        uint32_t k0, sl0;
+        load_meta(live_top, k0, sl0);
+        gather(live_top, k0, sl0);
+        load_meta(live_top - 1, k_next, slot_next);
     }
     for (int ci = live_top; ci >= 0; --ci) {
         const uint32_t base = (uint32_t)ci * BCH;
@@ -486,9 +483,9 @@
             st[wave][1][pos + 3] = r1;
             st[wave][2][pos + 3] = make_float4(r2x, __uint_as_float((uint32_t)lane), 0.0f, 0.0f);
         }
-        const uint32_t m_this = m_cur, slot_this = slot_cur, id_this = id_cur;
-        gather(ci - 1, m_next, id_next, slot_next);
-        load_meta(ci - 2, m_next, id_next, slot_next);
+        const uint32_t m_this = k_cur & 15u, slot_this = slot_cur, id_this = k_cur >> 4;
+        gather(ci - 1, k_next, slot_next);
+        load_meta(ci - 2, k_next, slot_next);
         const int par = ci & 1;
         auto group = [&](const int k, auto tail) {
             constexpr bool TAIL = decltype(tail)::value;
@@ -624,11 +621,11 @@
                           float* out_color, bool longest_first, bool safe, hipStream_t st) {
     Grid g(ks.H, ks.W);
     if (longest_first)
-        tile_order_kernel<<<NUM_XCD, 1024, 0, st>>>(g.tiles, g.gx, gv.ranges, gv.tile_count, gv.total + 2, gv.total + 4);
+        tile_order_kernel<<<NUM_XCD, 1024, 0, st>>>(g.tiles, g.gx, gv.live_n, gv.tile_count, gv.total + 2, gv.total + 4);
     auto kernel = safe ? blend_forward_kernel<true> : blend_forward_kernel<false>;
     kernel<<<(unsigned)blend_slots_per_xcd(g) * NUM_XCD * 4, 64, 0, st>>>(
-        ks.W, ks.H, g.gx, g.tiles, gv.tile_count, gv.total, gv.ranges, bv.point_list, bv.qmask, gv.rec, ks.bg, out_color, iv.final_T,
-        iv.n_contrib);
+        ks.W, ks.H, g.gx, g.tiles, gv.tile_count, gv.total, gv.ranges, bv.live, gv.live_n, gv.rec, ks.bg, out_color, iv.final_T,
+        iv.n_contrib, iv.n_live);
 }
 
 void launch_blend_backward(const KSettings& ks, const GeomView& gv, const BinView& bv, const ImgView& iv,
@@ -639,9 +636,9 @@
     if (flags) { ZeroList z; z.add(gv.has_rec, ((size_t)gv.P + 3) / 4 * 4, st); launch_zero(z, st); }
     auto kernel = safe ? blend_backward_kernel<true> : blend_backward_kernel<false>;
     kernel<<<(unsigned)blend_slots_per_xcd(g) * NUM_XCD, 256, 0, st>>>(
-        ks.W, ks.H, g.gx, g.tiles, gv.tile_count, gv.total, gv.ranges, bv.point_list, gm_from_base ? nullptr : bv.gm_index, gv.gm_base,
-        bv.qmask, gv.rec, ks.bg,
-        iv.final_T, iv.n_contrib, dL_dcolor, grad_rec, iv.cut_key, stamp, flags ? gv.has_rec : nullptr);
+        ks.W, ks.H, g.gx, g.tiles, gv.tile_count, gv.total, gv.ranges, bv.live, gv.live_n, gm_from_base ? nullptr : bv.gm_index, gv.gm_base,
+        gv.rec, ks.bg,
+        iv.final_T, iv.n_live, dL_dcolor, grad_rec, iv.cut_key, stamp, flags ? gv.has_rec : nullptr);
 }
 
 }
diff --git a/splatco_amd/csrc/capi.hip b/splatco_amd/csrc/capi.hip
--- a/splatco_amd/csrc/capi.hip
+++ b/splatco_amd/csrc/capi.hip
@@ -312,7 +312,7 @@
     int rc = plan_enqueue(P, M, means3D, scales, rotations, cov3D_precomp, opacities, shs, colors_precomp, settings, geom_buf,
                           radii_out, plan_host, st, seq);
     if (rc) return rc;
-    const unsigned long long cap = binning_buf ? (unsigned long long)(binning_capacity_bytes / 17) : 0ull;
+    const unsigned long long cap = binning_buf ? (unsigned long long)(binning_capacity_bytes / 25) : 0ull;
     const bool early = binning_buf && P > 0 && cap > 0 && image_buf && out_color;
     if (early) {
         KSettings ks = ksettings(settings);
@@ -401,17 +401,22 @@
     Grid g(H, W);
     const void* src = nullptr;
     size_t bytes = 0;
-    if (which <= SCR_DBG_RANGES || which == SCR_DBG_SPLAT_RECORDS) {
+    if (which <= SCR_DBG_RANGES || which == SCR_DBG_SPLAT_RECORDS || which == SCR_DBG_LIVE_COUNT) {
         if (!geom_buf) return fail("geom_buf is NULL");
         GeomView gv = geom_view((void*)geom_buf, P, H, W);
         if (which == SCR_DBG_TILES_TOUCHED) { src = gv.tiles_touched; bytes = (size_t)P * 4; }
         else if (which == SCR_DBG_POINT_OFFSETS) { src = gv.point_offsets; bytes = (size_t)P * 4; }
         else if (which == SCR_DBG_RANGES) { src = gv.ranges; bytes = (size_t)g.tiles * 8; }
+        else if (which == SCR_DBG_LIVE_COUNT) { src = gv.live_n; bytes = I > 0 ? (size_t)g.tiles * 4 : 0; }
         else { src = gv.rec; bytes = (size_t)P * REC_F * 4; }
     } else if (which == SCR_DBG_POINT_LIST) {
         if (!binning_buf) return fail("binning_buf is NULL");
         src = bin_view((void*)binning_buf, I, 0).point_list;
         bytes = (size_t)I * 4;
+    } else if (which == SCR_DBG_LIVE_LIST) {
+        if (!binning_buf) return fail("binning_buf is NULL");
+        src = bin_view((void*)binning_buf, I, 0).live;
+        bytes = (size_t)I * 8;
     } else if (which == SCR_DBG_QMASK || which == SCR_DBG_GM_INDEX) {
         if (!binning_buf) return fail("binning_buf is NULL");
         BinView bv = bin_view((void*)binning_buf, I, 0);
diff --git a/splatco_amd/csrc/common.h b/splatco_amd/csrc/common.h
--- a/splatco_amd/csrc/common.h
+++ b/splatco_amd/csrc/common.h
@@ -46,6 +46,7 @@
     uint32_t* tile_count;
     uint32_t* ranges;
     uint32_t* cursor;
+    uint32_t* live_n;
     int64_t P;
     unsigned long long* total;
     size_t bytes;
@@ -69,6 +70,7 @@
     v.tile_count = (uint32_t*)take((size_t)g.tiles * 4);
     v.ranges = (uint32_t*)take((size_t)g.tiles * 8);
     v.cursor = (uint32_t*)take((size_t)g.tiles * 4);
+    v.live_n = (uint32_t*)take((size_t)g.tiles * 4);
     v.total = (unsigned long long*)take(128);
     v.bytes = off;
     v.P = P;
@@ -90,6 +92,7 @@
     uint32_t* point_list;
     uint32_t* gm_index;
     uint8_t* qmask;
+    uint2* live;
     unsigned long long* keys2;
     size_t bytes;
 };
@@ -104,6 +107,7 @@
     v.point_list = (uint32_t*)take(n * 4);
     v.gm_index = (uint32_t*)take(n * 4);
     v.qmask = (uint8_t*)take(n);
+    v.live = (uint2*)take(n * 8);
     const bool merge = max_tile_instances > WG_SORT_MAX;
     v.keys2 = merge ? (unsigned long long*)take(n * 8) : nullptr;
     v.bytes = off;
@@ -117,6 +121,7 @@
 struct ImgView {
     float* final_T;
     uint32_t* n_contrib;
+    uint32_t* n_live;
     unsigned long long* cut_key;
     size_t bytes;
 };
@@ -128,6 +133,7 @@
     auto take = [&](size_t n) { char* q = p ? p + off : nullptr; off += align_up(n); return q; };
     v.final_T = (float*)take((size_t)H * W * 4);
     v.n_contrib = (uint32_t*)take((size_t)H * W * 4);
+    v.n_live = (uint32_t*)take((size_t)H * W * 4);
     v.cut_key = (unsigned long long*)take((size_t)Grid(H, W).tiles * 8 + 8);
     v.bytes = off;
     return v;
@@ -177,6 +183,9 @@
     return r;
 }
 __device__ __forceinline__ unsigned long long lanes(bool p) { return __builtin_amdgcn_ballot_w64(p); }
+__device__ __forceinline__ uint32_t lanes_below(unsigned long long ballot) {
+    return __builtin_amdgcn_mbcnt_hi((uint32_t)(ballot >> 32), __builtin_amdgcn_mbcnt_lo((uint32_t)ballot, 0u));
+}
 __device__ __forceinline__ bool nonfinite3(float a, float b, float c) {
     constexpr int NAN_OR_INF = 0x1 | 0x2 | 0x4 | 0x200;
     return __builtin_amdgcn_classf(a, NAN_OR_INF) || __builtin_amdgcn_classf(b, NAN_OR_INF) || __builtin_amdgcn_classf(c, NAN_OR_INF);
diff --git a/splatco_amd/rasterizer.py b/splatco_amd/rasterizer.py
--- a/splatco_amd/rasterizer.py
+++ b/splatco_amd/rasterizer.py
@@ -69,6 +69,7 @@
             _C.DBG_FINAL_T: ((self.cs.H, self.cs.W), torch.float32),
             _C.DBG_SPLAT_RECORDS: ((self.P, 12), torch.float32),
             _C.DBG_QMASK: ((self.I,), torch.uint8), _C.DBG_GM_INDEX: ((self.I,), torch.int32),
+            _C.DBG_LIVE_LIST: ((self.I, 2), torch.int32), _C.DBG_LIVE_COUNT: ((tiles if self.I else 0,), torch.int32),
         }
         shape, dt = shapes[which]
         out = torch.empty(shape, dtype=dt, device=dev)
```

New measurement: 1091 Msplats/s, median of 6. No clear change (+0.9%).
